# cggos/ptam_cg

Hardware: AMD Instinct MI355X
Metric: BA LM iterations/s (50 KF x 5k pts) [+ tracked frames/s @640x480 in 'tracking'] (higher is better)
Workload: dtype f64

## Files before the change

### __graft_entry__.py

```python
import os
import subprocess
import sys

ROOT = os.path.dirname(os.path.abspath(__file__))
if ROOT not in sys.path:
    sys.path.insert(0, ROOT)


def build():
    env = dict(os.environ)
    env.setdefault("PATH", "")
    env["PATH"] = "/opt/rocm/bin:" + env["PATH"]
    subprocess.check_call(["make", "-C", os.path.join(ROOT, "ptam_cg_amd", "csrc"), "-j4"], env=env)
    subprocess.check_call(["make", "-C", os.path.join(ROOT, "oracle")], env=env)
    import ptam_cg_amd
    from ptam_cg_amd import _abi
    import ctypes
    lib = ctypes.CDLL(os.path.join(ROOT, "ptam_cg_amd", "csrc", "libptam_hip.so"))
    missing = [n for n in _abi.DECLARED if not hasattr(lib, "ptam_" + n)]
    if missing:
        raise RuntimeError(f"libptam_hip.so lacks {missing}")


def smoke():
    import numpy as np
    from ptam_cg_amd import host, synth
    from ptam_cg_amd._lib import load
    from tests.oracle_lib import load_oracle
    from tests import util
    hip, oracle = load(), load_oracle()
    a, b = synth.make_frame_pair()
    util.assert_levels_equal(util.keyframe_levels(hip, a), util.keyframe_levels(oracle, a))
    res = []
    for lib in (hip, oracle):
        ctx = host.Context(lib=lib)
        kfa = host.KeyFrame(ctx).MakeKeyFrame_Lite(a)
        kfb = host.KeyFrame(ctx).MakeKeyFrame_Lite(b)
        q, t = synth.make_patch_queries([kfa.level(l) for l in range(4)], n=200)
        res.append(host.PatchFinder(ctx).FindPatchCoarse(kfb, q, t))
    for f in ("found", "best_ssd", "best_x", "best_y"):
        assert np.array_equal(res[0][f], res[1][f]), f
    pc = synth.make_pose_case(n=300)
    ph = host.Context(lib=hip).pose_gn(pc["world"], pc["found"], pc["sqrt_inv_noise"], pc["init_pose"])[0]
    po = host.Context(lib=oracle).pose_gn(pc["world"], pc["found"], pc["sqrt_inv_noise"], pc["init_pose"])[0]
    assert np.allclose(ph, po, atol=1e-10)
    prob = synth.make_ba_problem(8, 100, 1)
    util.assert_ba_equal(util.run_ba(hip, prob), util.run_ba(oracle, prob))
    print("smoke ok: keyframe / patch search bit-exact, pose GN and bundle within tolerance")


if __name__ == "__main__":
    build()
    if len(sys.argv) > 1 and sys.argv[1] == "smoke":
        smoke()
```

### include/ptam_hip_bench.h

```cpp
#ifndef PTAM_HIP_BENCH_H
#define PTAM_HIP_BENCH_H
#include "ptam_hip.h"
#ifdef __cplusplus
extern "C" {
#endif

int ptam_bench_track_frames(int n, ptam_tracker* const* trackers, ptam_kf* const* current, const uint8_t* const* d_frames,
                            const double pose_in[12], const ptam_trackmap_opts* opts, const int32_t* shuffle_levels,
                            const int32_t* shuffle_fine, int frames_each, double* seconds_out);
int ptam_bench_track_batch(int nb, ptam_tracker* const* trackers, ptam_kf* const* current, const uint8_t* const* d_frames,
                           const double pose_in[12], const ptam_trackmap_opts* opts, const int32_t* shuffle_levels,
                           const int32_t* shuffle_fine, int rounds, int groups, double* seconds_out);
int ptam_bench_track_sequence(ptam_tracker* t, ptam_kf* current, int n_frames, const uint8_t* const* d_frames,
                              ptam_motion_model* m, const ptam_trackmap_opts* opts, const int32_t* shuffle_levels,
                              const int32_t* shuffle_fine, int passes, const double* poses_true, double* seconds_out,
                              double* stats_out);

enum {
    PTAM_TS_PYR_PVS = 0,
    PTAM_TS_DETECT = 1,
    PTAM_TS_COMPACT_SELECT = 2,
    PTAM_TS_SEARCH_COARSE = 3,
    PTAM_TS_GATHER_COARSE = 4,
    PTAM_TS_POSE_COARSE = 5,
    PTAM_TS_SEARCH_FINE = 6,
    PTAM_TS_GATHER_FINE = 7,
    PTAM_TS_POSE_FINE = 8,
    PTAM_TS_COUNT = 9
};
int ptam_tracker_set_profiling(ptam_tracker* t, int on);
int ptam_tracker_stage_time(const ptam_tracker* t, int stage, double* total_ms, int* frames);

int ptam_ba_bench_jacobian(ptam_ba* ba, int reps, double* avg_ms, double* algorithmic_bytes);
int ptam_ba_bench_jacobian_rotating(ptam_ba** bas, int n, int reps, double* avg_ms);
int ptam_ba_schur_index_map(int variant, uint16_t* out, int cap);
enum {
    PTAM_BL_COUNTS = 0,
    PTAM_BL_ROWPTR = 1,
    PTAM_BL_M_CAM = 2,
    PTAM_BL_M_PT = 3,
    PTAM_BL_M_ORIG = 4,
    PTAM_BL_M_FIDX = 5,
    PTAM_BL_M_FOUND = 6,
    PTAM_BL_M_S = 7,
    PTAM_BL_PT_ORIG = 8,
    PTAM_BL_POINTS = 9,
    PTAM_BL_CHUNKS = 10,
    PTAM_BL_S_ENTRIES = 11,
    PTAM_BL_S_SEGS = 12,
    PTAM_BL_S_WG_SEG = 13,
    PTAM_BL_S_PAIR_BEGIN = 14,
    PTAM_BL_S_WG_HEAD = 15,
    PTAM_BL_CAM_PTR = 16,
    PTAM_BL_CAM_MEAS = 17
};
int ptam_ba_debug_lists(ptam_ba* ba, int which, void* out, size_t cap_bytes);

#ifdef __cplusplus
}
#endif
#endif
```

### ptam_cg_amd/csrc/ba_debug_host.inc

```
struct BaHostTimes {
    double t0 = 0, first = 0, loop = 0;
};
#ifdef K7_TIMING
static double ba_dbg_now_us() { return std::chrono::duration<double, std::micro>(std::chrono::steady_clock::now().time_since_epoch()).count(); }
#endif

static inline void ba_dbg_begin(ptam_ba* ba, BaHostTimes& ht) {
#ifdef K7_TIMING
    ht.t0 = ba_dbg_now_us();
    (void)hipMemsetAsync(ba->d.dbg + TL_BASE, 0, 8, ba->ctx->stream);
#endif
}
static inline void ba_dbg_first_read(BaHostTimes& ht) {
#ifdef K7_TIMING
    if (ht.first == 0) ht.first = ba_dbg_now_us();
#endif
}
static inline int ba_dbg_loop_end(ptam_ba* ba, BaHostTimes& ht) {
#ifdef K7_TIMING
    ht.loop = ba_dbg_now_us();
    const BaDev& d = ba->d;
    long long h[16];
    HIP_TRY(hipMemcpy(h, d.dbg, sizeof h, hipMemcpyDeviceToHost));
    std::printf("LDLT step2 wg0: loop %lld tail %lld | last wg (role %lld): loop %lld tail %lld\n", h[1] - h[0], h[2] - h[1], h[7],
                h[5] - h[4], h[6] - h[5]);
    long long q[8];
    HIP_TRY(hipMemcpy(q, d.dbg + 32, sizeof q, hipMemcpyDeviceToHost));
    std::printf("LDLT step2 wg0 iteration 3 (cycles): micro factor %lld | my rows %lld | next panel columns %lld | publish %lld | barrier %lld | "
                "operand reads issued %lld | off-chain updates %lld\n", q[1] - q[0], q[2] - q[1], q[3] - q[2], q[4] - q[3], q[5] - q[4], q[6] - q[5], q[7] - q[6]);
#endif
    return PTAM_OK;
}
static inline int ba_dbg_dump(ptam_ba* ba, const BaHostTimes& ht) {
#if defined(K7_TIMING) || defined(SCHUR_STAMPS)
    const BaDev& d = ba->d;
#endif
#ifdef K7_TIMING
    std::printf("HOST Compute: first trial read at %.1f us, loop end %.1f us, total %.1f us (%zu trials)\n", ht.first - ht.t0, ht.loop - ht.t0,
                ba_dbg_now_us() - ht.t0, ba->trials.size());
    {
        long long c[4];
        HIP_TRY(hipMemcpy(c, d.dbg + 5000, sizeof c, hipMemcpyDeviceToHost));
        if (c[3] > c[1])
            std::printf("K7 INSIDE Compute() (its last launch, block 100): %lld shader cycles in %.2f us = %.2f GHz\n", c[2] - c[0], (c[3] - c[1]) * 0.01,
                        (double)(c[2] - c[0]) / ((c[3] - c[1]) * 10.0));
    }
    if (getenv("PTAM_TIMELINE")) {
        std::vector<long long> tl(2 + 2 * TL_MAX);
        HIP_TRY(hipMemcpy(tl.data(), d.dbg + TL_BASE, tl.size() * 8, hipMemcpyDeviceToHost));
        const long long n_tl = std::min<long long>(tl[0], TL_MAX);
        static const char* nm[] = {"?", "purge_pass1", "select_compact", "select_final", "K7", "reduce_vinv", "vinv", "schur_tile", "schur_reduce",
                                   "ldlt_step0", "backward", "point_update", "finalize", "project_e2", "pass1_trial", "purge", "reduce_partials", "publish"};
        for (long long i = 0; i < n_tl; i++)
            std::printf("TL %4lld %-16s start %9.2f us  (+%.2f)\n", i, nm[tl[2 + 2 * i] < 18 ? tl[2 + 2 * i] : 0], (tl[3 + 2 * i] - tl[3]) * 0.01,
                        i ? (tl[3 + 2 * i] - tl[1 + 2 * i]) * 0.01 : 0.0);
    }
#endif
#ifdef SCHUR_STAMPS
    {
        std::vector<long long> wt(1024);
        HIP_TRY(hipMemcpy(wt.data(), d.dbg + 3072, wt.size() * 8, hipMemcpyDeviceToHost));
        const int nw = std::min(512, d.n_schur_wg);
        const long long M40 = (1ll << 40) - 1, M56 = (1ll << 56) - 1;
        long long e0 = wt[0] & M40, x1 = 0;
        for (int i = 0; i < nw; i++) e0 = std::min(e0, wt[2 * i] & M40), x1 = std::max(x1, wt[2 * i + 1] & M56 & M40);
        std::printf("SCHUR workgroups %d: makespan %.2f us; per workgroup (entry, exit in us from the first entry, segments, hw id):\n", nw, (x1 - e0) * 0.01);
        for (int i = 0; i < nw; i++)
            std::printf("%s[%d %.1f %.1f %d %llx]", i % 8 ? " " : "\n  ", i, ((wt[2 * i] & M40) - e0) * 0.01, ((wt[2 * i + 1] & M40) - e0) * 0.01, (int)(wt[2 * i + 1] >> 56),
                        (unsigned long long)(wt[2 * i] >> 40));
        std::printf("\n");
        std::vector<int> wseg((size_t)d.n_schur_wg + 1);
        HIP_TRY(hipMemcpy(wseg.data(), d.s_wg_seg, wseg.size() * 4, hipMemcpyDeviceToHost));
        std::vector<SchurWG> segs((size_t)wseg.back());
        HIP_TRY(hipMemcpy(segs.data(), d.s_segs, segs.size() * sizeof(SchurWG), hipMemcpyDeviceToHost));
        std::vector<SchurEntry> ents((size_t)std::max(1, d.n_schur_entries));
        HIP_TRY(hipMemcpy(ents.data(), d.s_entries, (size_t)d.n_schur_entries * sizeof(SchurEntry), hipMemcpyDeviceToHost));
        std::printf("SCHUR schedule:");
        for (int i = 0; i < nw; i++) {
            std::printf("%s{%d", i % 8 ? " " : "\n  ", i);
            for (int sg = wseg[i]; sg < wseg[i + 1]; sg++) {
                long long cost = 0;
                for (int e = segs[sg].e_begin; e < segs[sg].e_end; e++) cost += ents[(size_t)e].pad & 0xffff;
                std::printf(" %d:%d:%lld", segs[sg].pair, (segs[sg].e_end - segs[sg].e_begin + 3) / 4, cost);
            }
            std::printf("}");
        }
        std::printf("\n");
    }
    {
        std::vector<long long> st(1024);
        HIP_TRY(hipMemcpy(st.data(), d.dbg + 2048, st.size() * 8, hipMemcpyDeviceToHost));
        for (int sel = 0; sel < 2; sel++) {
            const long long* b = st.data() + sel * 512;
            long long t0 = b[0];
            for (int w = 0; w < 4; w++) if (b[w * 64] && b[w * 64] < t0) t0 = b[w * 64];
            std::printf("SCHUR stamps wg %d (groups %lld): per wave, per group: top, loads issued, data there, MFMAs issued (cycles from the first top)\n", sel ? 150 : 0, b[260]);
            for (int w = 0; w < 4; w++) {
                std::printf("  w%d:", w);
                for (int i = 0; i < 16 && b[(w * 16 + i) * 4]; i++)
                    std::printf(" [%lld %lld %lld %lld]", b[(w * 16 + i) * 4] - t0, b[(w * 16 + i) * 4 + 1] - t0, b[(w * 16 + i) * 4 + 2] - t0, b[(w * 16 + i) * 4 + 3] - t0);
                std::printf(" end %lld\n", b[256 + w] - t0);
            }
            std::printf("  kernel entry %lld, exit %lld, segments %lld; last segment's epilogue (wave 0): loop end %lld, barrier 1 %lld, 2 %lld, 3 %lld, laid out %lld, stores issued %lld\n",
                        b[264] - t0, b[265] - t0, b[266], b[268] - t0, b[269] - t0, b[270] - t0, b[271] - t0, b[272] - t0, b[273] - t0);
        }
    }
#endif
    return PTAM_OK;
}
static inline int ba_dbg_k7_stamps(ptam_ba* ba, int reps) {
#ifdef K7_TIMING
    const BaDev& d = ba->d;
    long long h[16];
    HIP_TRY(hipMemcpy(h, d.dbg, sizeof h, hipMemcpyDeviceToHost));
    {
        long long c[4];
        HIP_TRY(hipMemcpy(c, d.dbg + 5000, sizeof c, hipMemcpyDeviceToHost));
        if (c[3] > c[1])
            std::printf("K7 BACK TO BACK (last of %d launches, block 100): %lld shader cycles in %.2f us = %.2f GHz\n", reps, c[2] - c[0], (c[3] - c[1]) * 0.01,
                        (double)(c[2] - c[0]) / ((c[3] - c[1]) * 10.0));
    }
    std::printf("K7 stamps (10 ns ticks since kernel-body start):");
    for (int i = 1; i < 10; i++) std::printf(" [%d] %lld", i, h[i] - h[0]);
    std::printf("\n");
    const int nb = std::min(ba->d.grid_acc, 2000);
    std::vector<long long> w(2 * nb);
    HIP_TRY(hipMemcpy(w.data(), d.dbg + 16, w.size() * 8, hipMemcpyDeviceToHost));
    long long t0 = w[0];
    for (int b = 0; b < nb; b++) t0 = std::min(t0, w[2 * b]);
    std::vector<long long> st(nb), en(nb), du(nb);
    for (int b = 0; b < nb; b++) st[b] = w[2 * b] - t0, en[b] = w[2 * b + 1] - t0, du[b] = en[b] - st[b];
    std::sort(st.begin(), st.end());
    std::sort(en.begin(), en.end());
    std::sort(du.begin(), du.end());
    std::printf("K7 block 7: body starts %lld ticks after the block's first instruction\n", h[0] - w[14]);
    std::printf("K7 wall (10 ns ticks, %d blocks): start p0/p50/p90/p100 %lld %lld %lld %lld | end %lld %lld %lld %lld | dur %lld %lld %lld %lld\n",
                nb, st[0], st[nb / 2], st[nb * 9 / 10], st[nb - 1], en[0], en[nb / 2], en[nb * 9 / 10], en[nb - 1], du[0], du[nb / 2],
                du[nb * 9 / 10], du[nb - 1]);
#endif
    return PTAM_OK;
}
```

### ptam_cg_amd/csrc/ba_jacobian.inc

```
#ifdef K7_NOW
#define K7_WSTORE(dst, v) { const double2 v_ = v; asm volatile("" ::"v"(v_.x), "v"(v_.y)); }
#else
typedef double k7_d2 __attribute__((ext_vector_type(2)));
#define K7_WSTORE(dst, v) { const double2 v_ = v; const k7_d2 w_ = {v_.x, v_.y}; asm volatile("global_store_dwordx4 %0, %1, off sc1\n\ts_nop 1" ::"v"(&(dst)), "v"(w_) : "memory"); }
#endif
template <int THREADS, bool COPY>
__device__ __forceinline__ void jac_flush(const BaDev& d, const double* Ul, double err, int nbad) {
    __shared__ double werr[THREADS / 64];
    __shared__ int wbad[THREADS / 64];
    const int tid = threadIdx.x;
    double* up = d.Upart + (size_t)blockIdx.x * d.F * 27;
#ifdef K7_FLUSH_SC1
    {
        const int n2 = (d.F * 27) >> 1;
        const bool al = ((((size_t)blockIdx.x * d.F * 27) & 1) == 0);
        if (al) {
            for (int k = tid; k < n2; k += THREADS) K7_WSTORE(((double2*)up)[k], make_double2(Ul[2 * k], Ul[2 * k + 1]));
            if (tid == 0 && ((d.F * 27) & 1)) up[d.F * 27 - 1] = Ul[d.F * 27 - 1];
        } else {
            if (tid == 0) up[0] = Ul[0];
            const int n2b = (d.F * 27 - 1) >> 1;
            for (int k = tid; k < n2b; k += THREADS) K7_WSTORE(*(double2*)(up + 1 + 2 * k), make_double2(Ul[1 + 2 * k], Ul[2 + 2 * k]));
            if (tid == 0 && (((d.F * 27) - 1) & 1)) up[d.F * 27 - 1] = Ul[d.F * 27 - 1];
        }
// ... 81 lines not shown
jac_accum_wave_kernel(DevCam cam, BaDev d, int cur, int est_arg, int per_wave, int extra) {
    TL_MARK(d, 4)
    const int4 gf = ba_guard_load(d);
    const int tid = threadIdx.x, lane = tid & 63;
    const int n_chunks64 = (d.M + 63) >> 6;
    const int wid = __builtin_amdgcn_readfirstlane(tid >> 6);
    if (ba_guard_blocks(d, gf)) return;
    if (ba_guard_stay(d, gf)) cur ^= 1;
    const int est = EST >= 0 ? EST : est_arg;
    extern __shared__ __attribute__((aligned(16))) double smem[];
    double* Ul = BIG ? d.Upart : smem;
    double* Ps = BIG ? d.pose[cur] : smem + (DET ? 0 : (((size_t)d.F * 27 + 1) & ~(size_t)1));
    double* Wt = (BIG ? smem : Ps + (size_t)d.C * 12 + 2) + (size_t)(tid >> 6) * K7_WT_DOUBLES;
    K7_WALL(0)
    const double* __restrict__ pt = d.pt[cur];
    const size_t wp = w_plane(d);
#if defined(K7_PRIO) && K7_PRIO == 1
    if (!LOOP) __builtin_amdgcn_s_setprio(0), __builtin_amdgcn_s_setprio(0);
    if (!LOOP) {
        const int pr_ = (wid >> 2) | (((blockIdx.x >> 8) & 1) << 1);
        if (pr_ == 1) __builtin_amdgcn_s_setprio(1);
        if (pr_ == 2) __builtin_amdgcn_s_setprio(2);
        if (pr_ == 3) __builtin_amdgcn_s_setprio(3);
    }
#elif defined(K7_PRIO) && K7_PRIO == 2
    if (!LOOP) {
        const int pr_ = wid & 3;
        if (pr_ == 1) __builtin_amdgcn_s_setprio(1);
        if (pr_ == 2) __builtin_amdgcn_s_setprio(2);
        if (pr_ == 3) __builtin_amdgcn_s_setprio(3);
    }
#elif defined(K7_PRIO) && K7_PRIO == 3
    if (!LOOP) {
        const int pr_ = (wid >> 1) & 3;
        if (pr_ == 1) __builtin_amdgcn_s_setprio(1);
        if (pr_ == 2) __builtin_amdgcn_s_setprio(2);
        if (pr_ == 3) __builtin_amdgcn_s_setprio(3);
    }
#endif
    int c_begin, c_end;
    {
        constexpr int WPB = THREADS / 64;
        const int blk = blockIdx.x, grid = gridDim.x;
        const int full = extra / grid, rem = extra - full * grid;
        const int before = blk * full + min(blk, rem) + min(wid, full) + ((wid > full && blk < rem) ? 1 : 0);
        const int mine = per_wave + ((wid < full || (wid == full && blk < rem)) ? 1 : 0);
        c_begin = (blk * WPB + wid) * per_wave + before;
        c_end = min(n_chunks64, c_begin + mine);
    }
    if (!BIG && !DET)
        for (int k = tid; k < d.F * 27; k += THREADS) Ul[k] = 0;
    const double* __restrict__ pose = d.pose[cur];
    const int n_pose = d.C * 12;
    double pv[2];
#pragma unroll
    for (int i = 0; i < 2; i++) {
        const int k = tid + i * THREADS;
        pv[i] = pose[min(k, n_pose - 1)];
    }
    K7In in;
    if (PREFETCH) k7_load(d, pt, min(c_begin, n_chunks64 - 1) << 6, lane, in);
    const double sigma_sq = d.sc->sigma_sq;
    if (!BIG) {
#pragma unroll
        for (int i = 0; i < 2; i++) {
            const int k = tid + i * THREADS;
            Ps[min(k, n_pose)] = pv[i];
        }
        for (int k = tid + 2 * THREADS; k < n_pose; k += THREADS) Ps[k] = pose[k];
    }
    __syncthreads();
    K7_STAMP(0)
    const double inv_sigma_sq = 1.0 / sigma_sq;
    double err = 0;
    int nbad = 0;
    K7_STAMP(1)
#pragma unroll 1
    for (int ci = c_begin; ci < c_end; ci++) {
        const int m0 = ci << 6;
        const int m = m0 + lane;
        const bool active = m < d.M;
        if (!PREFETCH) k7_load(d, pt, m0, lane, in);
        const K7In cu = in;
        K7_STAMP(2)
        if (PREFETCH && LOOP && ci + 1 < c_end) k7_load(d, pt, (ci + 1) << 6, lane, in);
        const int st = active ? cu.st : MS_DEAD, c = cu.c, p = cu.p, fidx = active ? cu.fidx : -1;
        const int src = p - cu.pt0;
        const double Xw = __shfl(cu.px, src, 64), Yw = __shfl(cu.py, src, 64), Zw = __shfl(cu.pz, src, 64);
        int pid = active ? p : (-1 - lane);
        double v[9];
#pragma unroll
        for (int i = 0; i < 9; i++) v[i] = 0;
        double A0[6] = {0, 0, 0, 0, 0, 0}, A1[6] = {0, 0, 0, 0, 0, 0}, B0[3] = {0, 0, 0}, B1[3] = {0, 0, 0};
        bool full = false;
        BaProj pr;
        double ex = 0, ey = 0, w = 0;
        const double* T = Ps + 12 * c;
        if (st == MS_BAD) {
            err += 1.0;
            nbad++;
        } else if (st == MS_ALIVE) {
            const double Xp[3] = {Xw, Yw, Zw};
            ba_project(cam, T, Xp, pr);
            ex = cu.sn * (cu.fo.x - pr.u);
            ey = cu.sn * (cu.fo.y - pr.v);
            const double e2 = ex * ex + ey * ey;
            w = ba_sqrt_weight(est, e2, sigma_sq, inv_sigma_sq);
            if (w == 0) {
                d.m_state[m] = MS_BAD;
                err += 1.0;
                nbad++;
            } else {
                err += ba_objective(est, e2, sigma_sq, inv_sigma_sq);
                full = true;
            }
        }
        K7_STAMP(3)
        if (full) {
            ex *= w;
            ey *= w;
            double D[4];
            ba_derivs(cam, pr, D);
            const double sw = cu.sn * w;
            const double D0 = sw * D[0], D1 = sw * D[1], D2 = sw * D[2], D3 = sw * D[3];
            const double X = pr.X, Y = pr.Y, Z = pr.Z;
            const double iz = rcp_nr(Z);
            __builtin_amdgcn_sched_barrier(0);
#pragma unroll
            for (int k = 0; k < 3; k++) {
                const double g0 = T[k], g1 = T[3 + k], g2 = T[6 + k];
                const double mx = (g0 - X * g2 * iz) * iz, my = (g1 - Y * g2 * iz) * iz;
                B0[k] = D0 * mx + D1 * my;
                B1[k] = D2 * mx + D3 * my;
            }
            __builtin_amdgcn_sched_barrier(0);
            if (fidx >= 0) {
                const double zx = -X * iz * iz, zy = -Y * iz * iz;
                {
                    const double mxs[6] = {iz, 0, zx, zx * Y, iz * Z - zx * X, -iz * Y};
                    const double mys[6] = {0, iz, zy, -iz * Z + zy * Y, -zy * X, iz * X};
#pragma unroll
                    for (int k = 0; k < 6; k++) {
                        A0[k] = D0 * mxs[k] + D1 * mys[k];
                        A1[k] = D2 * mxs[k] + D3 * mys[k];
                    }
                }
                __builtin_amdgcn_sched_barrier(0);
                K7_STAMP(4)
                if (!DET) {
                    double* Uc = Ul + fidx * 27;
                    int k = 0;
#pragma unroll
                    for (int a = 0; a < 6; a++)
#pragma unroll
                        for (int b = 0; b <= a; b++) K7_UADD(&Uc[k++], A0[a] * A0[b] + A1[a] * A1[b]);
#pragma unroll
                    for (int a = 0; a < 6; a++) K7_UADD(&Uc[21 + a], A0[a] * ex + A1[a] * ey);
                }
                __builtin_amdgcn_sched_barrier(0);
                K7_STAMP(5)
            }
        }
        {
            double* wg0 = d.W + (size_t)m0 * 6;
#pragma unroll
            for (int c = 0; c < 3; c++) {
                double2* wl = (double2*)(Wt + lane * 6);
#pragma unroll
                for (int h = 0; h < 3; h++)
                    wl[h] = make_double2(A0[2 * h] * B0[c] + A1[2 * h] * B1[c], A0[2 * h + 1] * B0[c] + A1[2 * h + 1] * B1[c]);
                double2 tq[3];
#pragma unroll
                for (int j = 0; j < 3; j++) tq[j] = ((const double2*)Wt)[64 * j + lane];
#pragma unroll
                for (int j = 0; j < 3; j++) {
                    const int u = 64 * j + lane;
                    if (m0 + u / 3 < d.M) K7_WSTORE(*(double2*)(wg0 + c * wp + 2 * u), tq[j]);
                }
            }
        }
        __builtin_amdgcn_sched_barrier(0);
        if (!full) ex = ey = 0;
        if (DET && active) {
            double* ad = d.Adet + m;
#pragma unroll
            for (int k = 0; k < 6; k++) ad[(size_t)k * d.M] = A0[k], ad[(size_t)(6 + k) * d.M] = A1[k];
            ad[(size_t)12 * d.M] = ex;
            ad[(size_t)13 * d.M] = ey;
        }
        v[0] = B0[0] * B0[0] + B1[0] * B1[0];
        v[1] = B0[1] * B0[0] + B1[1] * B1[0];
        v[2] = B0[1] * B0[1] + B1[1] * B1[1];
        v[3] = B0[2] * B0[0] + B1[2] * B1[0];
        v[4] = B0[2] * B0[1] + B1[2] * B1[1];
        v[5] = B0[2] * B0[2] + B1[2] * B1[2];
        v[6] = B0[0] * ex + B1[0] * ey;
        v[7] = B0[1] * ex + B1[1] * ey;
        v[8] = B0[2] * ex + B1[2] * ey;
        K7_STAMP(6)
        const int pid1 = pid + 1;
#define SEG_STEP(GETP, GETV)                                             \
    {                                                                    \
        const int po = GETP;                                             \
        double t[9];                                                     \
        _Pragma("unroll") for (int i = 0; i < 9; i++) t[i] = GETV;       \
        if (po == pid1) {                                                \
            _Pragma("unroll") for (int i = 0; i < 9; i++) v[i] += t[i];  \
        }                                                                \
    }
#ifndef K7_NOSCAN
        SEG_STEP(dpp_row_shr0_i32<1>(pid1), dpp_row_shr_f64<1>(v[i]))
        SEG_STEP(dpp_row_shr0_i32<2>(pid1), dpp_row_shr_f64<2>(v[i]))
        SEG_STEP(dpp_row_shr0_i32<4>(pid1), dpp_row_shr_f64<4>(v[i]))
        SEG_STEP(dpp_row_shr0_i32<8>(pid1), dpp_row_shr_f64<8>(v[i]))
        SEG_STEP((dpp_bcastx_i32<0x142>(pid1) & -((lane >> 4) & 1)), dpp_bcastx_f64<0x142>(v[i]))
        SEG_STEP((dpp_bcastx_i32<0x143>(pid1) & -((lane >> 5) & 1)), dpp_bcastx_f64<0x143>(v[i]))
#endif
#undef SEG_STEP
        K7_STAMP(7)
        const int pn = __shfl_down(pid, 1, 64);
        if (active && (lane == 63 || pn != pid)) {
            const bool whole = pid != cu.p_prev && pid != cu.p_next;
            double* Vp = whole ? d.V + (size_t)pid * 6 : d.cut + (size_t)(2 * ci + (pid == cu.p_prev ? 0 : 1)) * 9;
            double* Ep = whole ? d.epsB + (size_t)pid * 3 : Vp + 6;
#pragma unroll
            for (int i = 0; i < 6; i++) Vp[i] = v[i];
            Ep[0] = v[6];
            Ep[1] = v[7];
            Ep[2] = v[8];
        }
        if (!LOOP) break;
    }
    K7_STAMP(8)
    __syncthreads();
    jac_flush<THREADS, !BIG && !DET>(d, Ul, err, nbad);
    K7_STAMP(9)
    K7_WALL(1)
}

static const void* k7_wave_fn(int threads, bool loop, int est, bool big = false, bool det = false) {
    const bool tukey = est == PTAM_EST_TUKEY;
    if (det) {
        if (big) return (const void*)jac_accum_wave_kernel<256, false, true, -1, true, true>;
        if (!loop)
            return tukey ? (const void*)jac_accum_wave_kernel<1024, true, false, PTAM_EST_TUKEY, false, true>
                         : (const void*)jac_accum_wave_kernel<1024, true, false, -1, false, true>;
        return tukey ? (const void*)jac_accum_wave_kernel<256, true, true, PTAM_EST_TUKEY, false, true>
                     : (const void*)jac_accum_wave_kernel<256, false, true, -1, false, true>;
    }
    if (big) return (const void*)jac_accum_wave_kernel<256, false, true, -1, true>;
    if (!loop && threads == 1024)
        return tukey ? (const void*)jac_accum_wave_kernel<1024, true, false, PTAM_EST_TUKEY>
                     : (const void*)jac_accum_wave_kernel<1024, true, false, -1>;
    if (!loop)
        return tukey ? (const void*)jac_accum_wave_kernel<512, true, false, PTAM_EST_TUKEY>
                     : (const void*)jac_accum_wave_kernel<512, true, false, -1>;
    if (threads == 256)
        return tukey ? (const void*)jac_accum_wave_kernel<256, true, true, PTAM_EST_TUKEY>
                     : (const void*)jac_accum_wave_kernel<256, false, true, -1>;
    if (threads == 1024)
        return tukey ? (const void*)jac_accum_wave_kernel<1024, true, true, PTAM_EST_TUKEY>
                     : (const void*)jac_accum_wave_kernel<1024, false, true, -1>;
    return tukey ? (const void*)jac_accum_wave_kernel<512, true, true, PTAM_EST_TUKEY>
                 : (const void*)jac_accum_wave_kernel<512, false, true, -1>;
}

#define DET_TILE 1024
__global__ void __launch_bounds__(256) reduce_det_kernel(BaDev d) {
    if (ba_guard_blocks(d)) return;
    extern __shared__ __attribute__((aligned(16))) double det_lds[];
    constexpr int P = DET_TILE + 1;
    const int tile = blockIdx.x, tid = threadIdx.x;
    const int m0 = tile * DET_TILE, cnt = min(DET_TILE, d.M - m0);
    const size_t M = (size_t)d.M;
#pragma unroll
    for (int k = 0; k < 14; k++)
        for (int i = tid; i < cnt; i += 256) det_lds[k * P + i] = d.Adet[k * M + m0 + i];
    __syncthreads();
    const int* tptr = d.cam_ptr + (size_t)tile * (d.F + 1);
    for (int f = tid; f < d.F; f += 256) {
        double acc[27];
#pragma unroll
        for (int k = 0; k < 27; k++) acc[k] = 0;
        for (int i = tptr[f]; i < tptr[f + 1]; i++) {
            const double* ad = det_lds + (d.cam_meas[i] - m0);
            double A0[6], A1[6];
#pragma unroll
            for (int k = 0; k < 6; k++) A0[k] = ad[k * P], A1[k] = ad[(6 + k) * P];
            const double ex = ad[12 * P], ey = ad[13 * P];
            int k = 0;
#pragma unroll
            for (int a = 0; a < 6; a++)
#pragma unroll
                for (int b = 0; b <= a; b++) acc[k++] += A0[a] * A0[b] + A1[a] * A1[b];
#pragma unroll
            for (int a = 0; a < 6; a++) acc[21 + a] += A0[a] * ex + A1[a] * ey;
        }
        double* up = d.Upart + ((size_t)tile * d.F + f) * 27;
#pragma unroll
        for (int k = 0; k < 27; k++) up[k] = acc[k];
    }
}

#define RSPLIT 16
__device__ __forceinline__ void reduce_partials_body(const BaDev& d, int grid_acc, int bx, int by) {
    __shared__ double comb[4][64];
    __shared__ double werr[4];
    __shared__ int wbad[4];
    const int total = d.F * 27;
    const int lane = threadIdx.x & 63, wid = threadIdx.x >> 6;
    const int col = bx * 64 + lane;
    const int split = by;
    const int rows_per = (d.u_rows + RSPLIT - 1) / RSPLIT;
    const int r0 = split * rows_per, r1 = min(d.u_rows, r0 + rows_per);
    double s = 0;
    if (col < total && r0 + wid < r1) {
        for (int b = r0 + wid; b < r1; b += 32) {
            double q[8];
#pragma unroll
            for (int u = 0; u < 8; u++) q[u] = d.Upart[(size_t)min(b + 4 * u, r1 - 1) * total + col];
#pragma unroll
            for (int u = 0; u < 8; u++) s += b + 4 * u < r1 ? q[u] : 0.0;
        }
    }
    comb[wid][lane] = s;
    __syncthreads();
    if (wid == 0 && col < total) d.Usplit[(size_t)split * total + col] = ((comb[0][lane] + comb[1][lane]) + comb[2][lane]) + comb[3][lane];
    if (bx == 0 && by == 0) {
        double e = 0;
        int nb = 0;
        for (int b = threadIdx.x; b < grid_acc; b += 256) {
            e += d.err_part[2 * b];
            nb += d.bad_part[b];
        }
        e = wave_sum_f64(e);
        nb = wave_sum_i32(nb);
        if (lane == 0) {
            werr[wid] = e;
            wbad[wid] = nb;
        }
        __syncthreads();
        if (threadIdx.x == 0) {
            d.sc->cur_err = ((werr[0] + werr[1]) + werr[2]) + werr[3];
            d.sc->n_bad = wbad[0] + wbad[1] + wbad[2] + wbad[3];
        }
    }
}

__global__ void __launch_bounds__(256) reduce_partials_kernel(BaDev d, int grid_acc) {
    TL_MARK(d, 16)
    if (ba_guard_blocks(d)) return;
    reduce_partials_body(d, grid_acc, blockIdx.x, blockIdx.y);
}
```

### ptam_cg_amd/csrc/ba_schur.inc

```
__device__ __forceinline__ void vinv_body(const BaDev& d, double lambda, int bx) {
    const int p = bx * 256 + threadIdx.x;
    if (p >= d.P) return;
    double v[6];
    const int r0 = d.rowptr[p], r1 = d.rowptr[p + 1];
    const int c0 = r0 >> 6, c1 = (r1 - 1) >> 6;
    if (d.cut != nullptr && r1 > r0 && c0 != c1) {
        const double* q = d.cut + (size_t)(2 * c0 + 1) * 9;
        double e[3] = {q[6], q[7], q[8]};
#pragma unroll
        for (int i = 0; i < 6; i++) v[i] = q[i];
        for (int c = c0 + 1; c <= c1; c++) {
            q = d.cut + (size_t)(2 * c) * 9;
#pragma unroll
            for (int i = 0; i < 6; i++) v[i] += q[i];
#pragma unroll
            for (int i = 0; i < 3; i++) e[i] += q[6 + i];
        }
#pragma unroll
        for (int i = 0; i < 3; i++) d.epsB[(size_t)p * 3 + i] = e[i];
    } else {
#pragma unroll
        for (int i = 0; i < 6; i++) v[i] = d.V[(size_t)p * 6 + i];
    }
    double A[9] = {v[0], v[1], v[3], v[1], v[2], v[4], v[3], v[4], v[5]};
    double* out = d.Vinv + (size_t)p * 9;
    if (A[0] * A[4] * A[8] == 0) {
#pragma unroll
        for (int i = 0; i < 9; i++) out[i] = 0;
        return;
    }
    A[0] *= (1.0 + lambda);
    A[4] *= (1.0 + lambda);
    A[8] *= (1.0 + lambda);
    for (int col = 0; col < 3; col++) {
        double inv_diag = 1;
        for (int row = col; row < 3; row++) {
            double val = A[row * 3 + col];
            for (int c2 = 0; c2 < col; c2++) val -= A[c2 * 3 + col] * A[row * 3 + c2];
            if (row == col) {
                A[row * 3 + col] = val;
                inv_diag = 1 / val;
            } else {
                A[col * 3 + row] = val;
                A[row * 3 + col] = val * inv_diag;
            }
        }
    }
    for (int c = 0; c < 3; c++) {
        double y[3], x[3];
        for (int i = 0; i < 3; i++) {
            double val = (i == c) ? 1.0 : 0.0;
            for (int j = 0; j < i; j++) val -= A[i * 3 + j] * y[j];
            y[i] = val;
        }
        for (int i = 0; i < 3; i++) y[i] /= A[i * 3 + i];
        for (int i = 2; i >= 0; i--) {
            double val = y[i];
            for (int j = i + 1; j < 3; j++) val -= A[j * 3 + i] * x[j];
            x[i] = val;
        }
        for (int r = 0; r < 3; r++) out[r * 3 + c] = x[r];
    }
}

__global__ void __launch_bounds__(256) vinv_kernel(BaDev d, double lambda) {
    TL_MARK(d, 6)
    if (ba_guard_blocks(d)) return;
    vinv_body(d, lambda, blockIdx.x);
}
__global__ void __launch_bounds__(256) reduce_vinv_kernel(BaDev d, int grid_acc, int nx, double lambda, double lambda_stay) {
    TL_MARK(d, 5)
    const int4 gf = ba_guard_load(d);
    if (ba_guard_blocks(d, gf)) return;
    if (ba_guard_stay(d, gf)) lambda = lambda_stay;
    const int b = blockIdx.x, nr = nx * RSPLIT;
    if (b < nr)
        reduce_partials_body(d, grid_acc, b % nx, b / nx);
    else
        vinv_body(d, lambda, b - nr);
}

#define SCHUR_TILE_ELEMS (SCHUR_TC * SCHUR_TC * 36 + SCHUR_TC * 6)
#ifndef SCHUR_RING
#define SCHUR_RING 2
#endif
#ifndef SCHUR_NW
#define SCHUR_NW 4
#endif
#define SCHUR_WG_PER_CU (8 / SCHUR_NW)
#define SCHUR_RED_BYTES ((SCHUR_NW / 2) * 40 * 64 * 8)
#define SCHUR_N_VARIANTS 6
#define SCHUR_MAP_WPT 8

struct SchurGrp {
    double wa[3][3];
    double wb[3][3];
    double vi[9];
    double eb[3];
    unsigned pm;
};
typedef double v4f64 __attribute__((ext_vector_type(4)));
typedef double schur_d2 __attribute__((ext_vector_type(2), aligned(8)));

template <int MODE>
__host__ __device__ __forceinline__ int schur_row(int t, int rid) {
    if (MODE == 1) return rid;
    if (t < 2) return 6 * (rid / 3) + 2 * (rid % 3) + t;
    const int q = 16 + (rid >> 1);
    return 6 * (q / 3) + 2 * (q % 3) + (rid & 1);
}
struct SchurLane {
    int hi4, sh4, hi2, sh2;
    unsigned o4, o2;
};
template <int MODE>
__device__ __forceinline__ SchurLane schur_lane(int l15) {
    SchurLane L;
    const int r0 = schur_row<MODE>(0, l15), r2 = MODE == 3 ? schur_row<3>(2, l15) : 0;
    const int s0 = r0 / 6, s2 = r2 / 6;
    L.hi4 = s0 >> 2, L.sh4 = 8 * (s0 & 3), L.o4 = 8u * (unsigned)(r0 - 6 * s0);
    L.hi2 = s2 >> 2, L.sh2 = 8 * (s2 & 3), L.o2 = 8u * (unsigned)(r2 - 6 * s2);
    return L;
}

__device__ __forceinline__ unsigned schur_slot_off(unsigned o0, unsigned o1, int first, int hi, int sh, int M, bool& present) {
    const unsigned o = ((hi ? o1 : o0) >> sh) & 0xffu;
    present = o != 0xffu;
    return (present ? (unsigned)first + o : (unsigned)M) * 48u;
}

template <int MODE>
__device__ __forceinline__ void schur_fetch_role(const char* __restrict__ W0, const char* __restrict__ W1, const char* __restrict__ W2,
                                                 unsigned o0, unsigned o1, int first, const SchurLane& L, int M, double w[3][3],
                                                 bool& pres01, bool& pres2) {
    pres2 = false;
    const unsigned off4 = schur_slot_off(o0, o1, first, L.hi4, L.sh4, M, pres01) + L.o4;
#ifdef SCHUR_NOLOAD
    for (int t = 0; t < 3; t++) w[t][0] = w[t][1] = w[t][2] = (double)off4;
    return;
#endif
    if (MODE == 1) {
        w[0][0] = *(const double*)(W0 + off4);
        w[0][1] = *(const double*)(W1 + off4);
        w[0][2] = *(const double*)(W2 + off4);
        return;
    }
    const double2 p0 = *(const double2*)(W0 + off4), p1 = *(const double2*)(W1 + off4), p2 = *(const double2*)(W2 + off4);
    w[0][0] = p0.x, w[1][0] = p0.y;
    w[0][1] = p1.x, w[1][1] = p1.y;
    w[0][2] = p2.x, w[1][2] = p2.y;
    if (MODE == 3) {
        const unsigned off2 = schur_slot_off(o0, o1, first, L.hi2, L.sh2, M, pres2) + L.o2;
#ifdef SCHUR_NOFRAG2
        w[2][0] = w[2][1] = w[2][2] = (double)off2;
        return;
#endif
        w[2][0] = *(const double*)(W0 + off2);
        w[2][1] = *(const double*)(W1 + off2);
        w[2][2] = *(const double*)(W2 + off2);
    }
}

template <bool DIAG, int MA, int MB>
__device__ __forceinline__ void schur_fetch(const BaDev& d, const char* __restrict__ W0, const char* __restrict__ W1,
                                            const char* __restrict__ W2, const SchurEntry& e, const SchurLane& La, const SchurLane& Lb,
                                            SchurGrp& g) {
    const double* __restrict__ vp = d.Vinv + (size_t)e.pt * 9;
#ifdef SCHUR_NOVINV
    for (int q = 0; q < 9; q++) g.vi[q] = (double)e.pt;
    if (false)
#endif
#pragma unroll
    for (int q = 0; q < 4; q++) {
        const schur_d2 t = *(const schur_d2*)(vp + 2 * q);
        g.vi[2 * q] = t.x;
        g.vi[2 * q + 1] = t.y;
    }
#ifndef SCHUR_NOVINV
    g.vi[8] = vp[8];
#endif
    if (DIAG) {
        const double* __restrict__ ep = d.epsB + (size_t)e.pt * 3;
#pragma unroll
        for (int q = 0; q < 3; q++) g.eb[q] = ep[q];
    }
    bool a01, a2, b01 = false, b2 = false;
    schur_fetch_role<MA>(W0, W1, W2, e.offa[0], e.offa[1], e.ma, La, d.M, g.wa, a01, a2);
    if (!DIAG) schur_fetch_role<MB>(W0, W1, W2, e.offb[0], e.offb[1], e.mb, Lb, d.M, g.wb, b01, b2);
    g.pm = (__ballot(a01) ? 1u : 0u) | (__ballot(a2) ? 2u : 0u) | (__ballot(b01) ? 4u : 0u) | (__ballot(b2) ? 8u : 0u);
}

template <bool DIAG, int MA, int MB, int PM = -1>
__device__ __forceinline__ void schur_mult(const SchurGrp& g, v4f64 acc[3][3], double accE[3]
#ifdef SCHUR_DOUBLE_MFMA
                                           , v4f64 acc2[3][3]
#endif
) {
    const unsigned pm = PM >= 0 ? (unsigned)PM : g.pm;
    const bool A01 = pm & 1u, A2 = MA == 3 && (pm & 2u), B01 = DIAG ? A01 : (pm & 4u) != 0, B2 = DIAG ? A2 : (MB == 3 && (pm & 8u));
    double y[3][3];
#pragma unroll
    for (int t = 0; t < 3; t++)
#pragma unroll
        for (int c = 0; c < 3; c++) y[t][c] = 0.0;
    if (A01) {
#pragma unroll
        for (int t = 0; t < (MA < 2 ? MA : 2); t++)
#pragma unroll
            for (int c = 0; c < 3; c++) y[t][c] = g.wa[t][0] * g.vi[c] + g.wa[t][1] * g.vi[3 + c] + g.wa[t][2] * g.vi[6 + c];
    }
    if (A2) {
#pragma unroll
        for (int c = 0; c < 3; c++) y[2][c] = g.wa[2][0] * g.vi[c] + g.wa[2][1] * g.vi[3 + c] + g.wa[2][2] * g.vi[6 + c];
    }
#ifdef SCHUR_NOMFMA
#define SCH_MFMA(ti, tj, c) asm volatile("" ::"v"(y[ti][c]), "v"(DIAG ? g.wa[tj][c] : g.wb[tj][c]));
#elif defined(SCHUR_DOUBLE_MFMA)
#define SCH_MFMA(ti, tj, c)                                                                                                          \
    {                                                                                                                                \
        acc[ti][tj] = __builtin_amdgcn_mfma_f64_16x16x4f64(y[ti][c], DIAG ? g.wa[tj][c] : g.wb[tj][c], acc[ti][tj], 0, 0, 0);   \
        acc2[ti][tj] = __builtin_amdgcn_mfma_f64_16x16x4f64(y[ti][c], DIAG ? g.wa[tj][c] : g.wb[tj][c], acc2[ti][tj], 0, 0, 0); \
    }
#else
#define SCH_MFMA(ti, tj, c) acc[ti][tj] = __builtin_amdgcn_mfma_f64_16x16x4f64(y[ti][c], DIAG ? g.wa[tj][c] : g.wb[tj][c], acc[ti][tj], 0, 0, 0);
#endif
    if (A01 && B01) {
#pragma unroll
        for (int c = 0; c < 3; c++)
#pragma unroll
            for (int ti = 0; ti < (MA < 2 ? MA : 2); ti++)
#pragma unroll
                for (int tj = 0; tj < (MB < 2 ? MB : 2); tj++) SCH_MFMA(ti, tj, c)
    }
    if (!DIAG && A01 && B2) {
#pragma unroll
        for (int c = 0; c < 3; c++)
#pragma unroll
            for (int ti = 0; ti < (MA < 2 ? MA : 2); ti++) SCH_MFMA(ti, 2, c)
    }
    if (A2 && B01) {
#pragma unroll
        for (int c = 0; c < 3; c++)
#pragma unroll
            for (int tj = 0; tj < (MB < 2 ? MB : 2); tj++) SCH_MFMA(2, tj, c)
    }
    if (A2 && B2) {
#pragma unroll
        for (int c = 0; c < 3; c++) SCH_MFMA(2, 2, c)
    }
#undef SCH_MFMA
    if (DIAG) {
#pragma unroll
        for (int c = 0; c < 3; c++)
#pragma unroll
            for (int t = 0; t < MA; t++) accE[t] = fma(y[t][c], g.eb[c], accE[t]);
    }
}

template <bool DIAG, int MA, int MB>
__device__ __forceinline__ void schur_tile_body(const BaDev& d, const SchurWG wg, double* red) {
    const int tid = threadIdx.x, wid = tid >> 6;
    int lane = tid & 63;
    asm volatile("" : "+v"(lane));
    const int l15 = lane & 15, l4 = lane >> 4;
    const SchurLane La = schur_lane<MA>(l15), Lb = schur_lane<MB>(l15);
    const size_t wp8 = w_plane(d) * 8;
    const char* __restrict__ W0 = (const char*)d.W;
    const char* __restrict__ W1 = W0 + wp8;
    const char* __restrict__ W2 = W1 + wp8;
    v4f64 acc[3][3];
    double accE[3] = {0, 0, 0};
#pragma unroll
    for (int i = 0; i < 3; i++)
#pragma unroll
        for (int j = 0; j < 3; j++) acc[i][j] = (v4f64){0, 0, 0, 0};
#ifdef SCHUR_DOUBLE_MFMA
    v4f64 acc2[3][3];
#pragma unroll
    for (int i = 0; i < 3; i++)
#pragma unroll
        for (int j = 0; j < 3; j++) acc2[i][j] = (v4f64){0, 0, 0, 0};
#endif
    const int n_ent = wg.e_end - wg.e_begin;
    const int n_grp = (n_ent + 3) >> 2;
    auto entry_at = [&](int gi) {
        const int e = wg.e_begin + 4 * gi + l4;
        const bool have = gi < n_grp && e < wg.e_end;
        SchurEntry en = d.s_entries[have ? e : wg.e_begin];
        if (!have) en.offa[0] = en.offa[1] = en.offb[0] = en.offb[1] = 0xffffffffu;
        return en;
    };
    constexpr int R = SCHUR_RING;
    SchurGrp g[R];
    constexpr int NW = SCHUR_NW;
#pragma unroll
    for (int u = 0; u < R - 1; u++) schur_fetch<DIAG, MA, MB>(d, W0, W1, W2, entry_at(wid + NW * u), La, Lb, g[u]);
    SchurEntry ent_next = entry_at(wid + NW * (R - 1));
#ifdef SCHUR_STAMPS
    __shared__ long long stp[SCHUR_NW][16][4];
    int st_n = 0;
    if (lane == 0) stp[wid][0][0] = -1;
#define SCH_ST(k) if (st_n < 16 && lane == 0) stp[wid][st_n][k] = (long long)__builtin_amdgcn_s_memtime();
#else
#define SCH_ST(k)
#endif
    for (int gi = wid; gi < n_grp; gi += NW * R) {
#pragma unroll
        for (int u = 0; u < R; u++) {
            if (gi + NW * u >= n_grp) break;
            SCH_ST(0)
#ifndef SCHUR_NO_INTERLEAVE
            {
                bool done = false;
                auto step = [&](auto pm_c) {
                    constexpr int PM = decltype(pm_c)::value;
                    constexpr int pa = PM & 3, pb = PM >> 2;
                    if constexpr (pa != 0 && (MA == 3 || pa == 1) && (DIAG ? pb == 0 : (pb != 0 && (MB == 3 || pb == 1)))) {
                        const SchurEntry ent_after = entry_at(gi + NW * (u + R));
                        schur_fetch<DIAG, MA, MB>(d, W0, W1, W2, ent_next, La, Lb, g[(u + R - 1) % R]);
                        ent_next = ent_after;
                        schur_mult<DIAG, MA, MB, PM>(g[u], acc, accE);
                        __builtin_amdgcn_sched_group_barrier(0x020, 2, 0);
#pragma unroll
                        for (int q = 0; q < 20; q++) {
                            __builtin_amdgcn_sched_group_barrier(0x008, 1, 0);
                            __builtin_amdgcn_sched_group_barrier(0x020, 1, 0);
                        }
                        done = true;
#ifdef SCHUR_STAMPS
                        SCH_ST(3)
                        if (st_n < 16 && lane == 0) stp[wid][st_n][1] = stp[wid][st_n][2] = stp[wid][st_n][0];
                        st_n++;
#endif
                    }
                };
                constexpr int full_pm = 1 | (MA == 3 ? 2 : 0) | (DIAG ? 0 : (4 | (MB == 3 ? 8 : 0)));
                if (g[u].pm == (unsigned)full_pm)
                    step(std::integral_constant<int, full_pm>{});
                else {
                    unsigned pmv = g[u].pm;
                    asm volatile("" : "+v"(pmv));
                    switch (pmv) {
#define SCH_CASE(k) case k: if constexpr (k != full_pm) step(std::integral_constant<int, k>{}); break;
                        SCH_CASE(1) SCH_CASE(2) SCH_CASE(3) SCH_CASE(5) SCH_CASE(6) SCH_CASE(7) SCH_CASE(9) SCH_CASE(10) SCH_CASE(11)
                        SCH_CASE(13) SCH_CASE(14) SCH_CASE(15)
#undef SCH_CASE
                        default: break;
                    }
                }
                if (done) continue;
            }
#endif
            schur_fetch<DIAG, MA, MB>(d, W0, W1, W2, ent_next, La, Lb, g[(u + R - 1) % R]);
            ent_next = entry_at(gi + NW * (u + R));
            SCH_ST(1)
#ifdef SCHUR_STAMPS
            asm volatile("" ::"v"(g[u].wa[0][0]), "v"(g[u].wa[1][1]), "v"(g[u].wa[2][2]), "v"(g[u].vi[8]), "v"(g[u].vi[0]),
                         "v"(DIAG ? g[u].eb[2] : g[u].wb[2][2]), "v"(DIAG ? g[u].eb[0] : g[u].wb[0][0]));
#endif
            SCH_ST(2)
#ifdef SCHUR_DOUBLE_MFMA
            schur_mult<DIAG, MA, MB>(g[u], acc, accE, acc2);
#else
            schur_mult<DIAG, MA, MB>(g[u], acc, accE);
#endif
            SCH_ST(3)
#ifdef SCHUR_STAMPS
            st_n++;
#endif
        }
    }
#ifdef SCHUR_STAMPS
    {
        const long long t_end = (long long)__builtin_amdgcn_s_memtime();
        __syncthreads();
        const int sel = blockIdx.x == 0 ? 0 : (blockIdx.x == 150 ? 1 : -1);
        if (sel >= 0 && lane < 16 && wid < 4) {
            long long* o = d.dbg + 2048 + sel * 512 + (wid * 16 + lane) * 4;
            for (int k = 0; k < 4; k++) o[k] = lane < st_n ? stp[wid][lane][k] : 0;
            if (lane == 0) d.dbg[2048 + sel * 512 + 256 + wid] = t_end, d.dbg[2048 + sel * 512 + 260 + wid] = n_grp;
        }
        __syncthreads();
    }
#endif
#ifdef SCHUR_STAMPS
    const int st_sel = blockIdx.x == 0 ? 0 : (blockIdx.x == 150 ? 1 : -1);
#define SCH_EP(k) if (st_sel >= 0 && tid == 0) d.dbg[2048 + st_sel * 512 + 268 + (k)] = (long long)__builtin_amdgcn_s_memtime();
#else
#define SCH_EP(k)
#endif
    SCH_EP(0)
#pragma unroll
    for (int t = 0; t < 3; t++) {
        accE[t] += __shfl_xor(accE[t], 16, 64);
        accE[t] += __shfl_xor(accE[t], 32, 64);
    }
    double flat[39];
#pragma unroll
    for (int ti = 0; ti < 3; ti++)
#pragma unroll
        for (int tj = 0; tj < 3; tj++)
#pragma unroll
            for (int v = 0; v < 4; v++) flat[(ti * 3 + tj) * 4 + v] = acc[ti][tj][v]
#ifdef SCHUR_DOUBLE_MFMA
                                                                      + 0.0 * acc2[ti][tj][v]
#endif
                ;
#pragma unroll
    for (int t = 0; t < 3; t++) flat[36 + t] = DIAG ? accE[t] : 0.0;
    constexpr int H = NW / 2;
    if (wid >= H) {
        double* rw = red + (wid - H) * (40 * 64);
#pragma unroll
        for (int i = 0; i < 39; i++) rw[i * 64 + lane] = flat[i];
    }
    __syncthreads();
    SCH_EP(1)
    if (wid < H) {
        double* rw = red + wid * (40 * 64);
#pragma unroll
        for (int i = 0; i < 39; i++) rw[i * 64 + lane] += flat[i];
    }
    __syncthreads();
    SCH_EP(2)
    {
        static_assert(NW == 4 && SCHUR_MAP_WPT == 8 && (SCHUR_TILE_ELEMS / 2 + 255) / 256 <= 5, "five words per thread of a 256-thread workgroup");
        constexpr int variant = DIAG ? 3 - MA : 6 - MA;
        const unsigned* __restrict__ mp = d.s_map + ((size_t)variant * 64 * NW + tid) * SCHUR_MAP_WPT;
        const uint4 m4 = *(const uint4*)mp;
        const unsigned m5 = mp[4];
        const unsigned mw[5] = {m4.x, m4.y, m4.z, m4.w, m5};
        double2* out2 = (double2*)(d.s_part + (size_t)wg.slot * SCHUR_TILE_ELEMS);
        auto at = [&](unsigned m) {
            if (m == 0xffffu) return 0.0;
            if (H == 4) return (red[m] + red[2 * 2560 + m]) + (red[2560 + m] + red[3 * 2560 + m]);
            if (H == 2) return red[m] + red[2560 + m];
            return red[m];
        };
#pragma unroll
        for (int i = 0; i < 5; i++)
            if (mw[i] != 0xffffffffu) out2[tid + 64 * NW * i] = make_double2(at(mw[i] & 0xffffu), at(mw[i] >> 16));
    }
    SCH_EP(5)
}

static std::vector<unsigned short> schur_index_map() {
    std::vector<unsigned short> map((size_t)SCHUR_N_VARIANTS * SCHUR_TILE_ELEMS, 0xffffu);
    auto inv = [](int mode, int row, int& t, int& rid) {
        for (t = 0; t < mode; t++)
            for (rid = 0; rid < 16; rid++) {
                const int r = mode == 1 ? schur_row<1>(t, rid) : (mode == 2 ? schur_row<2>(t, rid) : schur_row<3>(t, rid));
                if (r == row) return true;
            }
        return false;
    };
    for (int variant = 0; variant < SCHUR_N_VARIANTS; variant++) {
        const bool diag = variant < 3;
        const int ma = diag ? 3 - variant : 6 - variant, mb = diag ? ma : 3;
        unsigned short* m = map.data() + (size_t)variant * SCHUR_TILE_ELEMS;
        for (int e = 0; e < SCHUR_TC * SCHUR_TC * 36; e++) {
            const int jk = e / 36, rc = e - jk * 36, j = jk / SCHUR_TC, k = jk - j * SCHUR_TC, r = rc / 6, c = rc - r * 6;
            int ti, rr, tj, rcol;
            if (!inv(ma, 6 * j + r, ti, rr) || !inv(mb, 6 * k + c, tj, rcol)) continue;
            m[e] = (unsigned short)(((ti * 3 + tj) * 4 + (rr >> 2)) * 64 + rcol + 16 * (rr & 3));
        }
        if (diag)
            for (int row = 0; row < SCHUR_TC * 6; row++) {
                int t, rid;
                if (inv(ma, row, t, rid)) m[SCHUR_TC * SCHUR_TC * 36 + row] = (unsigned short)((36 + t) * 64 + rid);
            }
    }
    return map;
}

static std::vector<unsigned> schur_index_map_device() {
    const std::vector<unsigned short> m = schur_index_map();
    constexpr int NT = 64 * SCHUR_NW, NE2 = SCHUR_TILE_ELEMS / 2;
    std::vector<unsigned> dev((size_t)SCHUR_N_VARIANTS * NT * SCHUR_MAP_WPT, 0xffffffffu);
    for (int v = 0; v < SCHUR_N_VARIANTS; v++)
        for (int t = 0; t < NT; t++)
            for (int i = 0; i < SCHUR_MAP_WPT && t + NT * i < NE2; i++) {
                const int e = t + NT * i;
                dev[((size_t)v * NT + t) * SCHUR_MAP_WPT + i] = (unsigned)m[(size_t)v * SCHUR_TILE_ELEMS + 2 * e] | ((unsigned)m[(size_t)v * SCHUR_TILE_ELEMS + 2 * e + 1] << 16);
            }
    return dev;
}

__global__ void __launch_bounds__(64 * SCHUR_NW) __attribute__((amdgpu_waves_per_eu(2, 2))) schur_tile_mfma_kernel(BaDev d) {
    TL_MARK(d, 7)
    extern __shared__ __attribute__((aligned(16))) double red[];
#ifdef SCHUR_STAMPS
    const long long t_entry = (long long)__builtin_amdgcn_s_memtime();
    if (threadIdx.x == 0 && blockIdx.x < 512) {
        unsigned hw, xcc;
        asm volatile("s_getreg_b32 %0, hwreg(HW_REG_HW_ID)" : "=s"(hw));
        asm volatile("s_getreg_b32 %0, hwreg(HW_REG_XCC_ID)" : "=s"(xcc));
        d.dbg[3072 + 2 * blockIdx.x] = ((long long)__builtin_amdgcn_s_memrealtime() & ((1ll << 40) - 1)) | ((long long)((xcc & 0xf) << 16 | (hw & 0xffff)) << 40);
    }
#endif
#ifdef SCHUR_NO_HEAD
    const int sg0 = d.s_wg_seg[blockIdx.x], sg1 = d.s_wg_seg[blockIdx.x + 1];
#else
    const int4 h0 = ((const int4*)d.s_wg_head)[2 * blockIdx.x], h1 = ((const int4*)d.s_wg_head)[2 * blockIdx.x + 1];
    const int sg0 = h0.x, sg1 = h0.y;
#endif
    for (int sg = sg0; sg < sg1; sg++) {
#ifdef SCHUR_NO_HEAD
        const SchurWG wg = d.s_segs[sg];
#else
        const SchurWG wg = sg == sg0 ? SchurWG{h0.z, h0.w, h1.x, h1.y} : d.s_segs[sg];
#endif
        int a = (int)((sqrt(8.0 * wg.pair + 1.0) - 1.0) * 0.5);
        while ((a + 1) * (a + 2) / 2 <= wg.pair) a++;
        while (a * (a + 1) / 2 > wg.pair) a--;
        const int b = wg.pair - a * (a + 1) / 2;
        const int ncam = min(SCHUR_TC, d.F - a * SCHUR_TC);
        const int ma = ncam <= 2 ? 1 : (ncam <= 5 ? 2 : 3);
        if (a == b) {
            if (ma == 3) schur_tile_body<true, 3, 3>(d, wg, red);
            else if (ma == 2) schur_tile_body<true, 2, 2>(d, wg, red);
            else schur_tile_body<true, 1, 1>(d, wg, red);
        } else {
            if (ma == 3) schur_tile_body<false, 3, 3>(d, wg, red);
            else if (ma == 2) schur_tile_body<false, 2, 3>(d, wg, red);
            else schur_tile_body<false, 1, 3>(d, wg, red);
        }
        __syncthreads();
    }
#ifdef SCHUR_STAMPS
    if (threadIdx.x == 0 && blockIdx.x < 512) d.dbg[3072 + 2 * blockIdx.x + 1] = (long long)__builtin_amdgcn_s_memrealtime() | ((long long)(sg1 - sg0) << 56);
    if ((blockIdx.x == 0 || blockIdx.x == 150) && threadIdx.x == 0) {
        long long* o = d.dbg + 2048 + (blockIdx.x ? 512 : 0) + 264;
        o[0] = t_entry, o[1] = (long long)__builtin_amdgcn_s_memtime(), o[2] = sg1 - sg0;
    }
#endif
}

#define SRED_SLICES 10
__device__ __forceinline__ double schur_sum_partials(const double* __restrict__ elem, int w0, int w1) {
#ifdef SRED_NOLOAD
    return (double)(w1 - w0);
#endif
    double s0 = 0, s1 = 0, s2 = 0, s3 = 0;
    for (int w = w0; w < w1; w += 32) {
        double q[32];
#pragma unroll
        for (int i = 0; i < 32; i++) {
            const double v = elem[(size_t)min(w + i, w1 - 1) * SCHUR_TILE_ELEMS];
            q[i] = w + i < w1 ? v : 0.0;
        }
#pragma unroll
        for (int i = 0; i < 32; i += 4) {
            s0 += q[i];
            s1 += q[i + 1];
            s2 += q[i + 2];
            s3 += q[i + 3];
        }
    }
    return (s0 + s1) + (s2 + s3);
}
__global__ void __launch_bounds__(256) schur_reduce_kernel(BaDev d, double lambda, int pad_identity) {
    TL_MARK(d, 8)
    const int pair = blockIdx.x, slice = blockIdx.y;
    int a = (int)((sqrt(8.0 * pair + 1.0) - 1.0) * 0.5);
    while ((a + 1) * (a + 2) / 2 <= pair) a++;
    while (a * (a + 1) / 2 > pair) a--;
    const int b = pair - a * (a + 1) / 2;
    const int wg0 = d.s_pair_wg_begin[pair], wg1 = d.s_pair_wg_begin[pair + 1];
    double* S = d.SE;
    double* E = se_E(d);
    const int band = se_band(d);
    const size_t FS = (size_t)d.F * 27;
    if (slice < 9) {
        const int idx = slice * 256 + threadIdx.x;
        const int jk = idx / 36, rc = idx - jk * 36;
        const int j = jk >> 3, k = jk & 7, r = rc / 6, c = rc - r * 6;
        const int fa = a * SCHUR_TC + j, fb = b * SCHUR_TC + k;
        if (fa >= d.F || fb >= d.F) return;
        if (a == b && j < k) return;
        const int Rr = 6 * fa + r, Cc = 6 * fb + c, Rb = Rr / SOLVE_NB, Cb = Cc / SOLVE_NB;
        if (Cb > Rb || Rb - Cb > band) return;
        const bool dg = a == b && j == k;
        const int rr = r >= c ? r : c, cc = r >= c ? c : r;
        double uq[RSPLIT];
#pragma unroll
        for (int sp = 0; sp < RSPLIT; sp++) uq[sp] = dg ? d.Usplit[sp * FS + fa * 27 + rr * (rr + 1) / 2 + cc] : 0.0;
        const double tsum = schur_sum_partials(d.s_part + idx, wg0, wg1);
        double val = -tsum;
        if (dg) {
            double u = 0;
#pragma unroll
            for (int sp = 0; sp < RSPLIT; sp++) u += uq[sp];
            if (r == c) u *= (1.0 + lambda);
            val += u;
        }
        S[se_blk(Rb, Cb, band) + (size_t)(Rr % SOLVE_NB) * SOLVE_NB + (Cc % SOLVE_NB)] = val;
        return;
    }
    if (a == b && threadIdx.x < SCHUR_TC * 6) {
        const int idx = threadIdx.x;
        const int j = idx / 6, r = idx - j * 6;
        const int fa = a * SCHUR_TC + j;
        if (fa < d.F) {
            const double s = schur_sum_partials(d.s_part + SCHUR_TC * SCHUR_TC * 36 + idx, wg0, wg1);
            double ea = 0;
#pragma unroll
            for (int sp = 0; sp < RSPLIT; sp++) ea += d.Usplit[sp * FS + fa * 27 + 21 + r];
            E[6 * fa + r] = ea - s;
        }
    }
    {
        const int np = d.npad - d.n, total = np * d.npad;
        for (int idx = pair * 256 + threadIdx.x; idx < total; idx += 256 * (int)gridDim.x) {
            const int q = idx / d.npad;
            const int r = d.n + q, c = idx - q * d.npad;
            const int Rb = r / SOLVE_NB, Cb = c / SOLVE_NB;
            if (c <= r && Rb - Cb <= band)
                S[se_blk(Rb, Cb, band) + (size_t)(r % SOLVE_NB) * SOLVE_NB + (c % SOLVE_NB)] = (r == c && pad_identity) ? 1.0 : 0.0;
        }
    }
    if (pair == 0) {
        const int np = d.npad - d.n;
        for (int idx = threadIdx.x; idx < np; idx += 256) E[d.n + idx] = 0.0;
    }
}
```

### ptam_cg_amd/csrc/bundle.h

```cpp
#pragma once
#include <cstddef>

#include "common.h"

enum { MS_ALIVE = 0, MS_BAD = 1, MS_DEAD = 2 };

#define BA_CHUNK 256
#define SCHUR_TC 8
#define SOLVE_NB 32
#define HIST_BINS 4096

struct BaChunk {
    int pt_begin, pt_end, m_begin, m_end;
};

struct SchurEntry {
    int pt;
    int ma;
    int mb;
    int pad;
    unsigned offa[2];
    unsigned offb[2];
};
struct SchurWG {
    int pair;
    int e_begin, e_end;
    int slot;
};

struct BaScalars {
    double sigma_sq;
    double cur_err;
    double new_err;
    double sumsq_cam;
    double sumsq_pt;
    double median;
    long long n_valid;
    int n_bad;
    int n_outliers;
    int sel_bin;
    int sel_k;
    int n_cand;
    int sel_bin2;
    int sel_k2;
    int select_overflow;
    int n_outliers_pub;
    int pad_;
    int end_step;
    int spec_go;
    int spec_stay;
    int spec_seq;
    int abort_any;
    int solve_fault;
};
static_assert(offsetof(BaScalars, end_step) % 16 == 0 && sizeof(BaScalars) % 8 == 0, "BaScalars: the decision words are read as one 16-byte load");

struct BaDev {
    int C, F, P, M;
    int guard;
    int guard_seq;
    int n, npad;
    int band;
    int n_chunks, grid_acc;
    int u_rows;
    int n_wchunks;
    int n_tiles, n_pairs, n_schur_wg, n_schur_entries;
    double* pose[2];
    int* cam_free;
    double* pt[2];
    double* V;
    double* epsB;
    double* Vinv;
    double* cut;
    int* rowptr;
    int* m_cam;
    int* m_pt;
    double2* m_found;
    double* m_s;
    int* m_orig;
    int* m_fidx;
    uint8_t* m_state;
    double* m_e2;
    double* m_e2t;
    uint8_t* m_zbad_t;
    double* W;
    double* Usplit;
    double* Upart;
    double* Adet;
    int* cam_ptr;
    int* cam_meas;
    double* err_part;
    int* bad_part;
    BaChunk* chunks;
    BaChunk* wchunks;
    unsigned* hist;
    double* cand;
    SchurEntry* s_entries;
    SchurWG* s_segs;
    int* s_wg_seg;
    int* s_pair_wg_begin;
    int* s_wg_head;
    double* s_part;
    unsigned* s_map;
    double* SE;
    double* L;
    double* Dg;
    double* y;
    double* da;
    double *SE2, *L2, *Dg2, *y2;
    unsigned* sflags2;
    unsigned* sflags;
    unsigned solve_seq;
    int chain_off;
    int chain_xcd;
    int spin_limit;
    double* bw_scratch;
    double* sumsq2;
    int* outliers;
    BaScalars* sc;
    long long* dbg;
};

__host__ __device__ __forceinline__ size_t w_plane(const BaDev& d) { return (size_t)(d.M + 1) * 6; }

__host__ __device__ __forceinline__ size_t se_blocks_before_row(int bi, int band) {
    return bi <= band ? (size_t)bi * (bi + 1) / 2 : (size_t)(band + 1) * (band + 2) / 2 + (size_t)(bi - band - 1) * (band + 1);
}
__host__ __device__ __forceinline__ size_t se_blk(int bi, int bj, int band) {
    const int j0 = bi - band > 0 ? bi - band : 0;
    return (se_blocks_before_row(bi, band) + (size_t)(bj - j0)) * (SOLVE_NB * SOLVE_NB);
}
__host__ __device__ __forceinline__ size_t se_size(int nblk, int band) { return se_blocks_before_row(nblk, band) * (SOLVE_NB * SOLVE_NB); }
__host__ __device__ __forceinline__ int se_band(const BaDev& d) {
    const int nblk = d.npad / SOLVE_NB;
    return d.band < nblk - 1 ? d.band : (nblk > 0 ? nblk - 1 : 0);
}
__host__ __device__ __forceinline__ double* se_E(const BaDev& d) { return d.SE + se_size(d.npad / SOLVE_NB, se_band(d)); }

#define MS_LOG 15
#define MS_CH (1 << MS_LOG)
#define MS_CH_BYTES ((size_t)MS_CH * 32)
template <class B>
__host__ __device__ __forceinline__ B* ms_chunk(B* base, size_t i) { return base + (i >> MS_LOG) * MS_CH_BYTES; }
__host__ __device__ __forceinline__ const int& ms_cam(const char* base, size_t i) { return ((const int*)ms_chunk(base, i))[i & (MS_CH - 1)]; }
__host__ __device__ __forceinline__ const int& ms_pt(const char* base, size_t i) { return ((const int*)(ms_chunk(base, i) + (size_t)MS_CH * 4))[i & (MS_CH - 1)]; }
__host__ __device__ __forceinline__ const double2& ms_found(const char* base, size_t i) { return ((const double2*)(ms_chunk(base, i) + (size_t)MS_CH * 8))[i & (MS_CH - 1)]; }
__host__ __device__ __forceinline__ const double& ms_sig(const char* base, size_t i) { return ((const double*)(ms_chunk(base, i) + (size_t)MS_CH * 24))[i & (MS_CH - 1)]; }

struct Carver {
    size_t off = 0;
    size_t take(size_t bytes) {
        const size_t o = off;
        off += (bytes + 255) & ~(size_t)255;
        return o;
    }
};

int ba_dev_meas_chunks(ptam_ba* ba, size_t n_max, char** d_chunks);
int ba_dev_ingest(ptam_ba* ba, int C, const double* poses12, const uint8_t* fixed, int P, const double* d_pts, int M);
struct BaDevResult {
    const double* pose;
    const double* pt;
    const int* pt_orig;
    int C, P_live;
    const int* outliers;
    int n_out;
    const int* step_end;
    int n_steps;
};
int ba_dev_result(const ptam_ba* ba, BaDevResult* r);

int ba_solve(ptam_ctx* ctx, BaDev& d, int cur);
#define CH_SPIN_DEFAULT (1 << 18)
size_t ba_solve_flag_bytes(int nblk);
int ba_solve_init();

#ifdef K7_TIMING
#define TL_BASE 4096
#define TL_MAX 1900
#define TL_MARK(d, kid)                                                                                   \
    if (blockIdx.x == 0 && blockIdx.y == 0 && threadIdx.x == 0) {                                         \
        const unsigned long long q_ = atomicAdd((unsigned long long*)&(d).dbg[TL_BASE], 1ull);            \
        if (q_ < TL_MAX) {                                                                                \
            (d).dbg[TL_BASE + 2 + 2 * q_] = (kid);                                                        \
            (d).dbg[TL_BASE + 3 + 2 * q_] = (long long)__builtin_amdgcn_s_memrealtime();                  \
        }                                                                                                 \
    }
#else
#define TL_MARK(d, kid)
#endif
```

### ptam_cg_amd/csrc/bundle.hip

```cpp
#include <algorithm>
#include <array>
#include <chrono>
#include <climits>
#include <atomic>
#include <numeric>
#include <utility>

#include "bundle.h"
#include "../../include/ptam_hip_bench.h"

#include "ba_math.inc"
#include "ba_pass1.inc"
#include "ba_select.inc"
#include "ba_jacobian.inc"
#include "ba_schur.inc"
#include "ba_update.inc"
#include "ba_prepare.inc"

template <class T>
struct PinVec {
    ptam_ctx* ctx = nullptr;
    T* p = nullptr;
    size_t n = 0, cap = 0, cap_bytes = 0;
    size_t size() const { return n; }
// ... 707 lines not shown
            ba->sblock_cap = ba->sblock_bytes;
        }
        HIP_TRY(hipMemsetAsync(ba->sblock, 0, sclear, ctx->stream));
        char* sb = (char*)ba->sblock;
        d.s_entries = (SchurEntry*)(sb + o_sent);
        d.s_segs = (SchurWG*)(sb + o_swg);
        d.s_wg_seg = (int*)(sb + o_swgseg);
        d.s_pair_wg_begin = (int*)(sb + o_spw);
        d.s_wg_head = (int*)(sb + o_swghead);
        d.s_part = (double*)(sb + o_spart);
        q.cap_pl = cap_pl, q.cap_cut = cap_cut;
        q.cpx = (int*)(sb + o_cpx);
        q.run_cnt = (int*)(sb + o_runcnt);
        q.run_cost = (int*)(sb + o_runcost);
        q.pl_pair = (int*)(sb + o_plpair);
        q.pl_n = (int*)(sb + o_pln);
        q.pl_run0 = (int*)(sb + o_plrun0);
        q.pl_e0 = (int*)(sb + o_ple0);
        q.pl_e = (int*)(sb + o_ple);
        q.pl_h = (long long*)(sb + o_plh);
        q.cut_pair = (int*)(sb + o_cutpair);
        q.cut_e0 = (int*)(sb + o_cute0);
        q.cut_e1 = (int*)(sb + o_cute1);
        q.cut_wg = (int*)(sb + o_cutwg);
        q.wg_first = (int*)(sb + o_wgfirst);
        q.pair_first = (int*)(sb + o_pairfirst);
        q.wseg_tmp = (int*)(sb + o_wsegtmp);
        q.rec = with_rec ? (int4*)(sb + o_rec) : nullptr;
        hipLaunchKernelGGL(prep_split_kernel, dim3(8), dim3(512), 0, ctx->stream, q, cfg);
        hipLaunchKernelGGL(prep_entries_kernel, dim3(n_pairs, 8), dim3(256), 0, ctx->stream, q, d, cfg.cost_model);
        hipLaunchKernelGGL(prep_finish_kernel, dim3(1), dim3(1024), 0, ctx->stream, q, d, cfg.slots);
    } else if (F > 0) {
        Carver sv;
        const size_t o_spw = sv.take((size_t)(n_pairs + 1) * 4), o_spart = sv.take(SCHUR_TILE_ELEMS * 8), o_one = sv.take(256);
        ba->sblock_bytes = sv.off;
        if (!ctx_cache_take(ctx->dev_cache, CTX_NCACHE(ctx->dev_cache), ba->sblock_bytes, &ba->sblock, &ba->sblock_cap)) {
            HIP_TRY(hipMalloc(&ba->sblock, ba->sblock_bytes));
            ba->sblock_cap = ba->sblock_bytes;
        }
        HIP_TRY(hipMemsetAsync(ba->sblock, 0, ba->sblock_bytes, ctx->stream));
        char* sb = (char*)ba->sblock;
        d.s_pair_wg_begin = (int*)(sb + o_spw);
        d.s_part = (double*)(sb + o_spart);
        d.s_entries = (SchurEntry*)(sb + o_one);
        d.s_segs = (SchurWG*)(sb + o_one);
        d.s_wg_seg = (int*)(sb + o_one);
        d.s_wg_head = (int*)(sb + o_one);
    }
    if (ba->det) {
        int* tile_free = (int*)(base + o_tilefree);
        hipLaunchKernelGGL(prep_det_count_kernel, dim3(n_dtiles), dim3(256), 0, ctx->stream, d, tile_free);
        hipLaunchKernelGGL(prep_det_scan_kernel, dim3(1), dim3(1024), 0, ctx->stream, tile_free, n_dtiles);
        hipLaunchKernelGGL(prep_det_lists_kernel, dim3(n_dtiles), dim3(256), 0, ctx->stream, d, (const int*)tile_free);
    }
#undef UP
    seq = ++ctx->pose_seq;
    *stamp = 0;
    hipLaunchKernelGGL(prep_publish_kernel, dim3(1), dim3(64), 0, ctx->stream, q, (volatile unsigned long long*)dp, seq);
    HIP_TRY(hipGetLastError());
    lap("phase 2 enqueued");
    if (int rc = ba_wait_stamp(ctx, stamp, seq, "the second phase of the bundle's prepare")) return rc;
    lap("phase 2 wait");
    ps = *ps_host;
    if (ps.bad) {
        ptam_set_error("bundle prepare: a Schur work list outgrew its bound (%d; workgroups per list %d %d %d %d %d %d %d %d, budgets %lld %lld, segments %d %d)", ps.bad,
                       ps.n_wgs[0], ps.n_wgs[1], ps.n_wgs[2], ps.n_wgs[3], ps.n_wgs[4], ps.n_wgs[5], ps.n_wgs[6], ps.n_wgs[7], ps.t_cut[0], ps.t_cut[1],
                       ps.n_cuts[0], ps.n_cuts[1]);
        return PTAM_E_STATE;
    }
    d.n_schur_wg = ps.n_schur_wg;
    ba->n_schur_segs = ps.n_segs;
#ifdef PREP_STAMPS
    for (int x = 0; x < 8; x++) {
        std::fprintf(stderr, "[ptam] split kernel, list %d (us from its start): lists built %.1f | in LDS %.1f | round 1 done %.1f | search done %.1f | cut written %.1f\n", x,
                     (ps.stamp[x][1] - ps.stamp[x][0]) * 0.01, (ps.stamp[x][2] - ps.stamp[x][0]) * 0.01, (ps.stamp[x][3] - ps.stamp[x][0]) * 0.01,
                     (ps.stamp[x][4] - ps.stamp[x][0]) * 0.01, (ps.stamp[x][5] - ps.stamp[x][0]) * 0.01);
        std::fprintf(stderr, "[ptam]    the search: %lld shader cycles in %.1f us = %.2f GHz\n", ps.stamp[x][7] - ps.stamp[x][6], (ps.stamp[x][4] - ps.stamp[x][2]) * 0.01,
                     (double)(ps.stamp[x][7] - ps.stamp[x][6]) / ((ps.stamp[x][4] - ps.stamp[x][2]) * 10.0));
    }
#endif
    if (getenv("PTAM_DEBUG_SCHUR")) {
        std::fprintf(stderr, "[ptam] schur: %d segments, %d workgroups; %lld entries in %d (XCD, pair) lists, budgets", ps.n_segs, ps.n_schur_wg,
                     ps.n_entries, ps.n_xp);
        for (int x = 0; x < 8; x++) std::fprintf(stderr, " %lld", ps.t_cut[x]);
        std::fprintf(stderr, "; workgroups per XCD");
        for (int x = 0; x < 8; x++) std::fprintf(stderr, " %d", ps.n_wgs[x]);
        std::fprintf(stderr, "\n");
    }
    {
        const int rc_s = ba_solve_init();
        if (rc_s) return rc_s;
    }
    ba->cur = 0;
    ba->prepared = true;
    return PTAM_OK;
}

static void prof_begin(ptam_ba* ba, int k) {
    if (!ba->prof) return;
    hipEventRecord(ba->ev[k][0], ba->ctx->stream);
}
static void prof_end(ptam_ba* ba, int k) {
    if (!ba->prof) return;
    hipEventRecord(ba->ev[k][1], ba->ctx->stream);
    ba->ev_used[k] = true;
}
static void prof_collect(ptam_ba* ba) {
    if (!ba->prof) return;
    for (int k = 0; k < PTAM_K_COUNT; k++)
        if (ba->ev_used[k]) {
            float ms = 0;
            if (hipEventElapsedTime(&ms, ba->ev[k][0], ba->ev[k][1]) == hipSuccess) {
                ba->k_ms[k] += ms;
                ba->k_n[k]++;
            }
            ba->ev_used[k] = false;
        }
}

static int ba_allreduce(ptam_ba* ba, double* dptr, size_t count) {
    if (!(ba->comm && ba->world > 1)) return PTAM_OK;
    const int rc = ba->comm(ba->comm_user, dptr, count, (void*)ba->ctx->stream);
    if (rc != 0) {
        ptam_set_error("all-reduce hook failed (%d)", rc);
        return PTAM_E_COMM;
    }
    return PTAM_OK;
}

static int ba_sel_blocks() {
    static const int n = [] {
        const char* e = ptam_ab_env("PTAM_SEL_BLOCKS");
        return e ? std::max(1, atoi(e)) : 256;
    }();
    return n;
}
static int ba_pass1_sigma(ptam_ba* ba) {
    ptam_ctx* ctx = ba->ctx;
    BaDev& d = ba->d;
    const bool sharded = ba->comm && ba->world > 1;
    const double min_s2 = ba->opts.min_sigma * ba->opts.min_sigma;
    const int build_hist = (sharded && ba->slow_select) ? 0 : 1;
    prof_begin(ba, PTAM_K_PROJECT);
    if (ba->trial_is_current && d.M > 0)
        hipLaunchKernelGGL(pass1_from_trial_kernel, dim3(std::max(1, std::min((d.M + 256 * P1_U - 1) / (256 * P1_U), 512))), dim3(256), 0, ctx->stream, d,
                           build_hist);
    else if (ba->e2_is_current && d.M > 0) {
        if (build_hist)
            hipLaunchKernelGGL(pass1_keep_kernel, dim3(std::max(1, std::min((d.M + 256 * P1_U - 1) / (256 * P1_U), 512))), dim3(256), 0, ctx->stream, d);
    } else if (d.n_chunks > 0)
        hipLaunchKernelGGL(project_e2_kernel, dim3(std::min(d.n_chunks, 512)), dim3(BA_CHUNK), 0, ctx->stream, ctx->cam, d,
                           ba->cur, build_hist);
    prof_end(ba, PTAM_K_PROJECT);
    prof_begin(ba, PTAM_K_SELECT);
    if (!sharded) {
        hipLaunchKernelGGL(select_compact_kernel, dim3(std::max(1, std::min((d.M + 1023) / 1024, ba_sel_blocks()))), dim3(256), 0,
                           ctx->stream, d, (const double*)d.m_e2, (long long)d.M, (const uint8_t*)d.m_state, 0);
    } else if (!ba->slow_select) {
        if (!ba->d_sel) {
            if (const char* e = ptam_ab_env("PTAM_XCAND_CAP")) ba->xcand_cap = std::max(1, std::min(atoi(e), 1 << 20));
            HIP_TRY(hipMalloc((void**)&ba->d_sel, (HIST_BINS + (size_t)ba->world * (1 + 2 * (size_t)ba->xcand_cap)) * sizeof(double)));
        }
        double* hx = ba->d_sel;
        double* xc = ba->d_sel + HIST_BINS;
        const int cap = ba->xcand_cap;
        double* list = xc + (size_t)ba->world * (1 + (size_t)cap);
        const size_t n_xc = (size_t)ba->world * (1 + (size_t)cap);
        auto reduce_hist = [&](unsigned* h) -> int {
            hipLaunchKernelGGL(hist_to_f64_kernel, dim3(HIST_BINS / 256), dim3(256), 0, ctx->stream, (const unsigned*)h, hx, HIST_BINS);
            const int rc = ba_allreduce(ba, hx, HIST_BINS);
            if (rc) return rc;
            hipLaunchKernelGGL(f64_to_hist_kernel, dim3(HIST_BINS / 256), dim3(256), 0, ctx->stream, (const double*)hx, h, HIST_BINS);
            return PTAM_OK;
        };
        int rc = reduce_hist(d.hist);
        if (rc) return rc;
        hipLaunchKernelGGL(select_compact_kernel, dim3(std::max(1, std::min((d.M + 1023) / 1024, ba_sel_blocks()))), dim3(256), 0,
                           ctx->stream, d, (const double*)d.m_e2, (long long)d.M, (const uint8_t*)d.m_state, 1);
        rc = reduce_hist(d.hist + HIST_BINS);
        if (rc) return rc;
        HIP_TRY(hipMemsetAsync(xc, 0, n_xc * sizeof(double), ctx->stream));
        hipLaunchKernelGGL(select_stage_kernel, dim3(1), dim3(1024), 0, ctx->stream, d, xc, ba->rank, ba->world, cap);
        rc = ba_allreduce(ba, xc, n_xc);
        if (rc) return rc;
        hipLaunchKernelGGL(select_finish_kernel, dim3(1), dim3(1024), 0, ctx->stream, d, (const double*)xc, list, ba->world, cap,
                           ba->opts.estimator, min_s2);
        prof_end(ba, PTAM_K_SELECT);
        HIP_TRY(hipGetLastError());
        return PTAM_OK;
    } else {
        int* d_cnt = (int*)(ba->d_xchg + 256);
        HIP_TRY(hipMemsetAsync(d_cnt, 0, 4, ctx->stream));
        hipLaunchKernelGGL(compact_valid_kernel, dim3(std::max(1, std::min((d.M + 255) / 256, 1024))), dim3(256), 0,
                           ctx->stream, d, d.cand, d_cnt);
        int n_local = 0;
        HIP_TRY(hipMemcpyAsync(&n_local, d_cnt, 4, hipMemcpyDeviceToHost, ctx->stream));
        HIP_TRY(ptam_stream_wait(ctx->stream));
        std::vector<double> counts(ba->world, 0.0);
        counts[ba->rank] = n_local;
        HIP_TRY(hipMemcpyAsync(ba->d_xchg, counts.data(), ba->world * 8, hipMemcpyHostToDevice, ctx->stream));
        int rc = ba_allreduce(ba, ba->d_xchg, ba->world);
        if (rc) return rc;
        HIP_TRY(hipMemcpyAsync(counts.data(), ba->d_xchg, ba->world * 8, hipMemcpyDeviceToHost, ctx->stream));
        HIP_TRY(ptam_stream_wait(ctx->stream));
        long long total = 0, off = 0;
        for (int r = 0; r < ba->world; r++) {
            if (r == ba->rank) off = total;
            total += (long long)(counts[r] + 0.5);
        }
        if ((size_t)total > ba->gather_cap) {
            if (ba->d_gather) HIP_TRY(hipFree(ba->d_gather));
            ba->gather_cap = (size_t)total + (size_t)total / 8 + 1024;
            HIP_TRY(hipMalloc((void**)&ba->d_gather, ba->gather_cap * 16));
        }
        HIP_TRY(hipMemsetAsync(ba->d_gather, 0, (size_t)total * 8, ctx->stream));
        if (n_local > 0)
            hipLaunchKernelGGL(place_keys_kernel, dim3((n_local + 255) / 256), dim3(256), 0, ctx->stream,
                               (const double*)d.cand, n_local, ba->d_gather + off);
        rc = ba_allreduce(ba, ba->d_gather, (size_t)total);
        if (rc) return rc;
        BaDev dg = d;
        dg.cand = ba->d_gather + ba->gather_cap;
        if (total > 0)
            hipLaunchKernelGGL(hist_keys_kernel, dim3((int)std::max<long long>(1, std::min<long long>((total + 255) / 256, 1024))),
                               dim3(256), 0, ctx->stream, (const double*)ba->d_gather, total, d.hist);
        hipLaunchKernelGGL(select_compact_kernel, dim3((int)std::max<long long>(1, std::min<long long>((total + 1023) / 1024, 256))),
                           dim3(256), 0, ctx->stream, dg, (const double*)ba->d_gather, total, (const uint8_t*)nullptr, 0);
        hipLaunchKernelGGL(select_final_kernel, dim3(1), dim3(1024), 0, ctx->stream, dg, ba->opts.estimator, min_s2);
        prof_end(ba, PTAM_K_SELECT);
        HIP_TRY(hipGetLastError());
        return PTAM_OK;
    }
    hipLaunchKernelGGL(select_final_kernel, dim3(1), dim3(1024), 0, ctx->stream, d, ba->opts.estimator, min_s2);
    prof_end(ba, PTAM_K_SELECT);
    HIP_TRY(hipGetLastError());
    return PTAM_OK;
}

static void launch_k7(ptam_ba* ba, int guard = 0) {
    ptam_ctx* ctx = ba->ctx;
    BaDev d = ba->d;
    d.guard = guard;
    d.guard_seq = (int)ba->mbox_seq;
    int cur = guard ? (ba->cur ^ 1) : ba->cur;
    if ((ba->k7_big && !ba->det) || !ba->use_wave)
        (void)hipMemsetAsync(d.Upart, 0, std::max<size_t>(1, (size_t)d.F * 27) * sizeof(double), ctx->stream);
    if (!ba->use_wave) {
        (void)hipMemsetAsync(d.err_part, 0, 16, ctx->stream);
        (void)hipMemsetAsync(d.bad_part, 0, 4, ctx->stream);
        return;
    }
    int est = ba->opts.estimator;
    void* args[] = {&ctx->cam, &d, &cur, &est, &ba->per_wave, &ba->extra_waves};
    (void)hipLaunchKernel(k7_wave_fn(ba->k7_threads, ba->k7_loop, est, ba->k7_big, ba->det), dim3(d.grid_acc), dim3(ba->k7_threads), args,
                          ba->smem_acc, ctx->stream);
    if (ba->det && d.F > 0)
        hipLaunchKernelGGL(reduce_det_kernel, dim3(d.u_rows), dim3(256), (size_t)14 * (DET_TILE + 1) * sizeof(double), ctx->stream, d);
}

static int ba_pass2(ptam_ba* ba) {
    ptam_ctx* ctx = ba->ctx;
    BaDev& d = ba->d;
    prof_begin(ba, PTAM_K_JACOBIAN);
    launch_k7(ba);
    prof_end(ba, PTAM_K_JACOBIAN);
    hipLaunchKernelGGL(reduce_partials_kernel, dim3(std::max(1, (d.F * 27 + 63) / 64), RSPLIT), dim3(256), 0, ctx->stream,
                       d, d.grid_acc);
    HIP_TRY(hipGetLastError());
    if (ba->comm && ba->world > 1) {
        if (d.F > 0) {
            hipLaunchKernelGGL(pack2_kernel, dim3(1), dim3(1), 0, ctx->stream, (const BaScalars*)d.sc, se_E(d) + d.npad, 0, 0);
            ba->cur_pending = true;
        } else {
            hipLaunchKernelGGL(pack2_kernel, dim3(1), dim3(1), 0, ctx->stream, (const BaScalars*)d.sc, ba->d_xchg, 0, 0);
            int rc = ba_allreduce(ba, ba->d_xchg, 2);
            if (rc) return rc;
            hipLaunchKernelGGL(unpack2_kernel, dim3(1), dim3(1), 0, ctx->stream, d.sc, (const double*)ba->d_xchg, 0);
        }
    }
    return PTAM_OK;
}

static int ba_ensure_mailbox(ptam_ba* ba) {
    if (ba->mbox) return PTAM_OK;
    void* h = nullptr;
    size_t cap = 0;
    if (!ctx_cache_take(ba->ctx->host_cache, CTX_NCACHE(ba->ctx->host_cache), sizeof(ptam_ba::Mailbox), &h, &cap))
        HIP_TRY(hipHostMalloc(&h, sizeof(ptam_ba::Mailbox), hipHostMallocMapped | hipHostMallocCoherent));
    std::memset(h, 0, sizeof(ptam_ba::Mailbox));
    void* dv = nullptr;
    HIP_TRY(hipHostGetDevicePointer(&dv, h, 0));
    ba->mbox = (ptam_ba::Mailbox*)h;
    ba->mbox_dev = (ptam_ba::Mailbox*)dv;
    return PTAM_OK;
}

static int ba_trial(ptam_ba* ba, double lambda, bool skip_vinv, int last_allowed, int abort_local, bool decide_in_prologue = false) {
    ptam_ctx* ctx = ba->ctx;
    BaDev& d = ba->d;
    prof_begin(ba, PTAM_K_VINV);
    if (d.P > 0 && !skip_vinv) hipLaunchKernelGGL(vinv_kernel, dim3((d.P + 255) / 256), dim3(256), 0, ctx->stream, d, lambda);
    prof_end(ba, PTAM_K_VINV);
    if (d.F > 0) {
        prof_begin(ba, PTAM_K_SCHUR);
        if (d.n_schur_wg > 0)
            hipLaunchKernelGGL(schur_tile_mfma_kernel, dim3(d.n_schur_wg), dim3(64 * SCHUR_NW), SCHUR_RED_BYTES, ctx->stream, d);
        hipLaunchKernelGGL(schur_reduce_kernel, dim3(d.n_pairs, SRED_SLICES), dim3(256), 0, ctx->stream, d, lambda,
                           (ba->world > 1 && ba->rank != 0) ? 0 : 1);
        prof_end(ba, PTAM_K_SCHUR);
        HIP_TRY(hipGetLastError());
        const size_t n_se = se_size(d.npad / SOLVE_NB, se_band(d)) + d.npad;
        const bool sharded = ba->comm && ba->world > 1;
        if (sharded) prof_begin(ba, PTAM_K_EXCHANGE);
        int rc = ba_allreduce(ba, d.SE, n_se + (ba->cur_pending ? 2 : 0));
        if (sharded) prof_end(ba, PTAM_K_EXCHANGE);
        if (rc) return rc;
        if (ba->cur_pending) {
            hipLaunchKernelGGL(unpack2_kernel, dim3(1), dim3(1), 0, ctx->stream, d.sc, (const double*)(d.SE + n_se), 0);
            ba->cur_pending = false;
        }
        prof_begin(ba, PTAM_K_SOLVE);
        rc = ba_solve(ctx, d, ba->cur);
        prof_end(ba, PTAM_K_SOLVE);
        if (rc) return rc;
    }
    prof_begin(ba, PTAM_K_UPDATE);
    if (d.F == 0)
        hipLaunchKernelGGL(pose_update_kernel, dim3(std::max(1, (d.C + 63) / 64)), dim3(64), 0, ctx->stream, d, ba->cur);
    if (d.n_chunks > 0)
        hipLaunchKernelGGL(point_update_kernel, dim3(d.n_chunks), dim3(BA_CHUNK), 0, ctx->stream, ctx->cam, d, ba->cur,
                           ba->opts.estimator);
    {
        const bool fuse = !(ba->comm && ba->world > 1) && !ba->prof;
        ulonglong2* slots = nullptr;
        unsigned long long seq = 0;
        if (fuse) {
            const int rcm = ba_ensure_mailbox(ba);
            if (rcm) return rcm;
            slots = (ulonglong2*)ba->mbox_dev;
            seq = ++ba->mbox_seq;
            ba->published_by_finalize = true;
        }
        ba->decide_pending = decide_in_prologue;
        ba->decide_last_allowed = last_allowed;
        if (!decide_in_prologue)
            hipLaunchKernelGGL(finalize_new_kernel, dim3(1), dim3(256), 0, ctx->stream, d, ba->opts.update_sq_conv_limit, last_allowed,
                               slots, seq);
    }
    prof_end(ba, PTAM_K_UPDATE);
    HIP_TRY(hipGetLastError());
    if (ba->comm && ba->world > 1) {
        hipLaunchKernelGGL(pack2_kernel, dim3(1), dim3(1), 0, ctx->stream, (const BaScalars*)d.sc, ba->d_xchg, 1, abort_local);
        int rc = ba_allreduce(ba, ba->d_xchg, 4);
        if (rc) return rc;
        hipLaunchKernelGGL(unpack2_kernel, dim3(1), dim3(1), 0, ctx->stream, d.sc, (const double*)ba->d_xchg, 1);
    }
    return PTAM_OK;
}

static int ba_p1_blocks() {
    static const int n = [] {
        const char* e = ptam_ab_env("PTAM_P1_BLOCKS");
        return e ? std::max(1, atoi(e)) : 512;
    }();
    return n;
}
static int ba_enqueue_speculative(ptam_ba* ba, double lambda_next, double lambda_stay) {
    ptam_ctx* ctx = ba->ctx;
    BaDev d = ba->d;
    const double min_s2 = ba->opts.min_sigma * ba->opts.min_sigma;
    d.guard = 1;
    d.guard_seq = (int)ba->mbox_seq;
    const dim3 g_p1(std::max(1, std::min((d.M + 256 * P1_U - 1) / (256 * P1_U), ba_p1_blocks())));
    if (ba->decide_pending) {
        hipLaunchKernelGGL(purge_pass1_decide_kernel, g_p1, dim3(256), 0, ctx->stream, d, ba->opts.update_sq_conv_limit, ba->decide_last_allowed,
                           (ulonglong2*)ba->mbox_dev, ba->mbox_seq);
        ba->decide_pending = false;
    } else
        hipLaunchKernelGGL(purge_pass1_kernel, g_p1, dim3(256), 0, ctx->stream, d);
    hipLaunchKernelGGL(select_compact_kernel, dim3(std::max(1, std::min((d.M + 1023) / 1024, ba_sel_blocks()))), dim3(256), 0, ctx->stream, d,
                       (const double*)d.m_e2, (long long)d.M, (const uint8_t*)d.m_state, 0);
    hipLaunchKernelGGL(select_final_kernel, dim3(1), dim3(1024), 0, ctx->stream, d, ba->opts.estimator, min_s2);
    launch_k7(ba, 1);
    {
        const int nx = std::max(1, (d.F * 27 + 63) / 64);
        hipLaunchKernelGGL(reduce_vinv_kernel, dim3(nx * RSPLIT + (d.P + 255) / 256), dim3(256), 0, ctx->stream, d, d.grid_acc, nx,
                           lambda_next, lambda_stay);
    }
    HIP_TRY(hipGetLastError());
    return PTAM_OK;
}

static int ba_publish_scalars(ptam_ba* ba) {
    ptam_ctx* ctx = ba->ctx;
    int rc = ba_ensure_mailbox(ba);
    if (rc) return rc;
    if (ba->published_by_finalize) {
        ba->published_by_finalize = false;
        return PTAM_OK;
    }
    const unsigned long long seq = ++ba->mbox_seq;
    hipLaunchKernelGGL(publish_scalars_kernel, dim3(1), dim3(64), 0, ctx->stream, (const BaScalars*)ba->d.sc,
                       (ulonglong2*)ba->mbox_dev, seq);
    HIP_TRY(hipGetLastError());
    return PTAM_OK;
}

static int ba_wait_scalars(ptam_ba* ba, BaScalars* out) {
    ptam_ctx* ctx = ba->ctx;
    const unsigned long long seq = ba->mbox_seq;
    constexpr unsigned NW = sizeof(BaScalars) / 8;
    auto arrived = [&]() {
        for (unsigned i = 0; i < NW; i++)
            if (ba->mbox->slot[i].seq != seq) return false;
        return true;
    };
    if (ba->prof) {
        HIP_TRY(ptam_stream_wait(ctx->stream));
    } else {
        const int rc = ba_wait_mapped(ctx, "a trial's scalars", arrived, [&](bool drained) {
            std::fprintf(stderr, "[ptam] waiting for seq %llu: stream %s, slots", seq, drained ? "drained" : "busy");
            for (unsigned i = 0; i < NW; i++) std::fprintf(stderr, " %llu", (unsigned long long)ba->mbox->slot[i].seq);
            std::fprintf(stderr, "\n");
        });
        if (rc) return rc;
    }
    unsigned long long words[NW];
    for (;;) {
        std::atomic_thread_fence(std::memory_order_acquire);
        for (unsigned i = 0; i < NW; i++) words[i] = ba->mbox->slot[i].v;
        std::atomic_thread_fence(std::memory_order_acquire);
        if (arrived()) break;
    }
    std::memcpy(out, words, sizeof(BaScalars));
    prof_collect(ba);
    return PTAM_OK;
}

static int ba_read_scalars(ptam_ba* ba, BaScalars* out) {
    const int rc = ba_publish_scalars(ba);
    return rc ? rc : ba_wait_scalars(ba, out);
}

int ba_dev_meas_chunks(ptam_ba* ba, size_t n_max, char** d_chunks) {
    if (int rc = ba->ms.reserve_dev((n_max + MS_CH - 1) >> MS_LOG)) return rc;
    *d_chunks = ba->ms.d;
    return PTAM_OK;
}
int ba_dev_ingest(ptam_ba* ba, int C, const double* poses12, const uint8_t* fixed, int P, const double* d_pts, int M) {
    ba->cam_pose.assign(poses12, poses12 + (size_t)12 * C);
    ba->cam_fixed.assign(fixed, fixed + C);
    ba->pts.n = 0;
    if (int rc = ba->pts.reserve((size_t)3 * P)) return rc;
    ba->pts.n = (size_t)3 * P;
    ba->pts_dev = d_pts;
    ba->ms.n = (size_t)M;
    ba->ms.up_chunks = ((size_t)M + MS_CH - 1) >> MS_LOG;
    ba->m_dead.assign((size_t)M, 0);
    ba->n_dead = 0;
    ba->prepared = false;
    return PTAM_OK;
}
int ba_dev_result(const ptam_ba* ba, BaDevResult* r) {
    if (!ba->prepared && ba->raw_out.empty()) return PTAM_E_STATE;
    const BaDev& d = ba->d;
    r->pose = d.pose[ba->cur];
    r->pt = d.pt[ba->cur];
    r->pt_orig = ba->d_pt_orig;
    r->C = d.C;
    r->P_live = d.P;
    r->outliers = d.outliers;
    r->n_out = (int)ba->raw_out.size();
    r->step_end = ba->raw_out_ends.data();
    r->n_steps = (int)ba->raw_out_ends.size();
    return PTAM_OK;
}

struct ChainTurn {
    static std::atomic<int>& busy(int dev) {
        static std::atomic<int> b[64];
        return b[dev & 63];
    }
    BaDev& d;
    int dev, was;
    bool forced;
    ChainTurn(BaDev& d_, int dev_) : d(d_), dev(dev_), was(d_.chain_off), forced(false) {
        if (busy(dev).fetch_add(1) > 0 && !d.chain_off) {
            d.chain_off = 1;
            forced = true;
        }
    }
    ~ChainTurn() {
        busy(dev).fetch_sub(1);
        if (forced && d.chain_off == 1) d.chain_off = was;
    }
};

static int ba_sharded_handshake(ptam_ba* ba, int rc_prepare, bool abort_local, bool* abort_all, ChainTurn& chain_turn) {
    ptam_ctx* ctx = ba->ctx;
    BaDev& d = ba->d;
    int n_free = 0;
    for (uint8_t x : ba->cam_fixed) n_free += x ? 0 : 1;
    const int nblk_x = (6 * n_free + SOLVE_NB - 1) / SOLVE_NB;
    constexpr int XF = 5;
    const bool band_fits = nblk_x + XF <= 512;
    std::vector<double> mine(band_fits ? XF + nblk_x : XF, 0.0), all(mine.size(), 0.0);
    mine[0] = (!rc_prepare && d.M == 0) ? 1.0 : 0.0;
    mine[1] = (double)d.M;
    mine[2] = rc_prepare ? 1.0 : 0.0;
    mine[3] = abort_local ? 1.0 : 0.0;
    mine[4] = d.chain_off ? 1.0 : 0.0;
    if (!rc_prepare && band_fits && nblk_x > 0) mine[XF + std::min(ba->band_local, nblk_x - 1)] = 1.0;
    if (!ba->d_xchg) {
        HIP_TRY(hipMalloc((void**)&ba->d_xchg, 4096));
        ba->xchg_owned = true;
    }
    HIP_TRY(hipMemcpyAsync(ba->d_xchg, mine.data(), mine.size() * 8, hipMemcpyHostToDevice, ctx->stream));
    const int rc = ba_allreduce(ba, ba->d_xchg, mine.size());
    if (rc) return rc_prepare ? rc_prepare : rc;
    HIP_TRY(hipMemcpyAsync(all.data(), ba->d_xchg, all.size() * 8, hipMemcpyDeviceToHost, ctx->stream));
    HIP_TRY(ptam_stream_wait(ctx->stream));
    if (all[2] > 0.5) {
        if (rc_prepare) return rc_prepare;
        ptam_set_error("sharded bundle: %d of %d ranks could not prepare their shard; nothing was computed on any rank",
                       (int)(all[2] + 0.5), ba->world);
        return PTAM_E_STATE;
    }
    *abort_all = all[3] > 0.5;
    if (all[4] > 0.5 && !d.chain_off) {
        d.chain_off = 1;
        chain_turn.forced = true;
    }
    ba->d.band = std::max(0, nblk_x - 1);
    if (band_fits)
        for (int b = nblk_x - 1; b >= 0; b--)
            if (all[XF + b] > 0.5) {
                ba->d.band = b;
                break;
            }
    if (all[0] > 0.5) {
        ptam_set_error("sharded bundle: %d of %d ranks hold no measurement (shard the points so that every rank gets some)",
                       (int)(all[0] + 0.5), ba->world);
        return PTAM_E_STATE;
    }
    return PTAM_OK;
}

static double ba_stall_ms(std::chrono::steady_clock::time_point t0, int trial, const char* did, const char* what) {
    const double ms = std::chrono::duration<double, std::milli>(std::chrono::steady_clock::now() - t0).count();
    if (ms > 3.0 && ba_debug().stall) std::fprintf(stderr, "[ptam] stall: trial %d %s %.2f ms %s\n", trial, did, ms, what);
    return ms;
}

static int ba_solve_fallback(ptam_ba* ba, int trial) {
    ptam_ctx* ctx = ba->ctx;
    BaDev& d = ba->d;
    if (d.chain_off) {
        ptam_set_error("bundle adjustment: the camera solve reports a fault in its launch-per-block form");
        return PTAM_E_HIP;
    }
    d.chain_off = 2;
    ba->solve_fallbacks++;
    HIP_TRY(hipMemsetAsync(&d.sc->solve_fault, 0, sizeof(int), ctx->stream));
    if (d.sflags) HIP_TRY(hipMemsetAsync(d.sflags, 0, sizeof(unsigned), ctx->stream));
    if (ba_debug().solve) std::fprintf(stderr, "[ptam] rank %d: persistent camera solve timed out at trial %d; repeating it with the launch-per-column form\n", ba->rank, trial);
    return PTAM_OK;
}

static void ba_report_trial_times(const ptam_ba* ba, const std::vector<double>& trial_read_us) {
    if (trial_read_us.empty()) return;
    std::fprintf(stderr, "[ptam] trial times (us):");
    for (size_t i = 0; i < trial_read_us.size() && i < ba->trials.size(); i++) {
        const ptam_ba_trial& t = ba->trials[i];
        std::fprintf(stderr, " %c%.1f", t.accepted ? 'a' : (t.err_new > t.err_old ? 'r' : 's'), trial_read_us[i] - (i ? trial_read_us[i - 1] : 0.0));
    }
    std::fprintf(stderr, "\n");
}

static int ba_readback(ptam_ba* ba, int n_out, std::vector<int>& out_idx) {
    ptam_ctx* ctx = ba->ctx;
    const BaDev& d = ba->d;
    const size_t b_pose = (size_t)d.C * 96, b_pts = (size_t)d.P * 24, b_out = (size_t)n_out * 4;
    void* pin = nullptr;
    int rc = ctx_pinned(ctx, 64 + b_pose + b_pts + b_out + 64, &pin);
    if (rc) return rc;
    char* hp = (char*)pin + 64;
    char* dp = (char*)ctx->d_pinned + 64;
    volatile unsigned long long* slot = (volatile unsigned long long*)pin;
    const unsigned long long seq = ++ctx->pose_seq;
    *slot = 0;
    const size_t n_all = (size_t)d.C * 12 + (size_t)d.P * 3 + (size_t)n_out;
    hipLaunchKernelGGL(readback_kernel, dim3((unsigned)std::max<size_t>(1, std::min<size_t>((n_all + 255) / 256, 1024))), dim3(256), 0,
                       ctx->stream, (const double*)d.pose[ba->cur], (size_t)d.C * 12, (const double*)d.pt[ba->cur], (size_t)d.P * 3,
                       (const int*)d.outliers, (size_t)n_out, (double*)dp, (double*)(dp + b_pose), (int*)(dp + b_pose + b_pts));
    hipLaunchKernelGGL(stamp_kernel, dim3(1), dim3(1), 0, ctx->stream, (volatile unsigned long long*)ctx->d_pinned, seq);
    HIP_TRY(hipGetLastError());
    rc = ba_wait_stamp(ctx, slot, seq, "the bundle's results");
    if (rc) return rc;
    std::memcpy(ba->cam_pose.data(), hp, b_pose);
    for (int q = 0; q < d.P; q++)
        std::memcpy(&ba->pts[(size_t)3 * ba->pt_orig[(size_t)q]], hp + b_pose + (size_t)q * 24, 24);
    if (n_out > 0) std::memcpy(out_idx.data(), hp + b_pose + b_pts, b_out);
    return PTAM_OK;
}

extern "C" {

void ptam_ba_opts_default(ptam_ba_opts* o) {
    if (!o) return;
    o->max_iterations = 20;
    o->update_sq_conv_limit = 1e-6;
    o->min_sigma = 0.4;
    o->estimator = PTAM_EST_TUKEY;
    o->verbose = 0;
    o->deterministic = 0;
    o->pad_ = 0;
}

int ptam_ba_create(ptam_ctx* ctx, const ptam_ba_opts* opts, ptam_ba** out) {
    ARG_TRY(ctx && out);
    ptam_ba* ba = new ptam_ba();
    ba->ctx = ctx;
    ba->pts.ctx = ba->ms.ctx = ctx;
    if (opts)
        ba->opts = *opts;
// ... 120 lines not shown
    HIP_TRY(hipSetDevice(ba->ctx->device));
    if (on && !ba->ev_ok) {
        for (int k = 0; k < PTAM_K_COUNT; k++) {
            HIP_TRY(hipEventCreate(&ba->ev[k][0]));
            HIP_TRY(hipEventCreate(&ba->ev[k][1]));
        }
        ba->ev_ok = true;
    }
    ba->prof = on != 0;
    return PTAM_OK;
}

int ptam_ba_kernel_time(const ptam_ba* ba, int kernel, double* total_ms, int* launches) {
    ARG_TRY(ba && kernel >= 0 && kernel < PTAM_K_COUNT);
    if (total_ms) *total_ms = ba->k_ms[kernel];
    if (launches) *launches = ba->k_n[kernel];
    return PTAM_OK;
}

int ptam_ba_set_comm(ptam_ba* ba, int rank, int world, ptam_allreduce_f64_fn fn, void* user) {
    ARG_TRY(ba && world >= 1 && rank >= 0 && rank < world);
    ARG_TRY(world == 1 || fn);
    ARG_TRY(world <= 32);
    if (ba->d_sel && world != ba->world) {
        HIP_TRY(hipSetDevice(ba->ctx->device));
        HIP_TRY(ptam_stream_wait(ba->ctx->stream));
        HIP_TRY(hipFree(ba->d_sel));
        ba->d_sel = nullptr;
    }
    ba->rank = rank;
    ba->world = world;
    ba->comm = fn;
    ba->comm_user = user;
    return PTAM_OK;
}

#define BA_DBG(...) do { if (dbg.wait) { std::fprintf(stderr, "[ptam] " __VA_ARGS__); std::fprintf(stderr, "\n"); } } while (0)
int ptam_ba_compute(ptam_ba* ba, const volatile unsigned char* abort_flag, int* accepted_out) {
    ARG_TRY(ba);
    ptam_ctx* ctx = ba->ctx;
    const BaDebug& dbg = ba_debug();
    HIP_TRY(hipSetDevice(ctx->device));
    BA_DBG("compute: prepare");
    const bool sharded = ba->comm && ba->world > 1;
    int rc = ptam_ba_prepare(ba);
    if (rc && !sharded) return rc;
    const int rc_prepare = rc;
    BA_DBG("compute: prepared M=%d P=%d F=%d chunks=%d wchunks=%d grid_acc=%d schur_wg=%d", ba->d.M, ba->d.P, ba->d.F, ba->d.n_chunks,
           ba->d.n_wchunks, ba->d.grid_acc, ba->d.n_schur_wg);
    BaDev& d = ba->d;
    ChainTurn chain_turn(d, ctx->device);
    double lambda = 0.0001, lambda_factor = 2.0;
    ba->converged = ba->published_by_finalize = ba->cur_pending = ba->slow_select = false;
    ba->trial_is_current = ba->e2_is_current = false;
    bool hit_max = false;
    int counter = 0;
    ba->accepted = 0;
    ba->trials.clear();
    std::vector<int> step_outlier_end;
    int n_steps = 0;
    bool prev_end_pending = false;
    bool abort_all = false;
    auto abort_local = [&]() { return abort_flag && *abort_flag; };
    auto aborted = [&]() { return sharded ? abort_all : abort_local(); };
    BaScalars sc;
    std::memset(&sc, 0, sizeof sc);
    double dbg_enq_ms = 0, dbg_wait_ms = 0;
    std::vector<double> trial_read_us;
    const auto dbg_t0 = std::chrono::steady_clock::now();
    BaHostTimes ht;
    ba_dbg_begin(ba, ht);
    if (sharded && (rc = ba_sharded_handshake(ba, rc_prepare, abort_local(), &abort_all, chain_turn))) return rc;
    const bool empty = d.M == 0;
    const bool spec = !sharded && !ba->prof && d.n_chunks > 0 && !ptam_ab_env("PTAM_NO_SPECULATION");
    bool spec_ready = false;
    const bool fused_decision = !ptam_ab_env("PTAM_SEPARATE_FINALIZE");
    while (!empty && !ba->converged && !hit_max && !aborted()) {
        bool skip_vinv = false;
        if (spec_ready) {
            spec_ready = false;
            skip_vinv = true;
        } else {
            if ((rc = ba_pass1_sigma(ba))) return rc;
            if ((rc = ba_pass2(ba))) return rc;
        }
        bool have_cur = false;
        double cur_err = 0, new_err = 0;
        bool ran_any = false, redo_step = false, nan_stop = false;
        for (;;) {
            if (have_cur && !(new_err > cur_err)) break;
            if (ba->converged || hit_max || aborted()) break;
            BA_DBG("trial %d lambda %g", counter, lambda);
            const auto q0 = std::chrono::steady_clock::now();
            rc = ba_trial(ba, lambda, skip_vinv, counter + 1 >= ba->opts.max_iterations ? 1 : 0, abort_local() ? 1 : 0, spec && fused_decision);
            dbg_enq_ms += ba_stall_ms(q0, counter, "took", "to enqueue");
            skip_vinv = false;
            if (rc) return rc;
            if ((rc = ba_publish_scalars(ba))) return rc;
            if (spec) {
                if ((rc = ba_enqueue_speculative(ba, lambda * 0.3, lambda))) return rc;
            }
            BA_DBG("trial %d enqueued, waiting", counter);
            const auto w0 = std::chrono::steady_clock::now();
            rc = ba_wait_scalars(ba, &sc);
            dbg_wait_ms += ba_stall_ms(w0, counter, "waited", "for its scalars");
            if (rc) return rc;
            BA_DBG("trial %d read: cur %g new %g sigma2 %g median %g n_valid %lld n_bad %d sumsq %g %g", counter, sc.cur_err, sc.new_err,
                   sc.sigma_sq, sc.median, sc.n_valid, sc.n_bad, sc.sumsq_cam, sc.sumsq_pt);
            ba_dbg_first_read(ht);
            if (!have_cur) {
                if (prev_end_pending) step_outlier_end.push_back(spec && fused_decision ? sc.n_outliers_pub : sc.n_outliers);
                prev_end_pending = false;
                if (sc.select_overflow && !ba->slow_select) {
                    ba->slow_select = true;
                    if (dbg.select) std::fprintf(stderr, "[ptam] rank %d: select overflow, repeating the step on the gather path\n", ba->rank);
                    redo_step = true;
                    break;
                }
                have_cur = true;
                cur_err = sc.cur_err;
                new_err = cur_err + 9999;
                if (!(new_err > cur_err)) {
                    nan_stop = true;
                    break;
                }
            }
            if (sc.solve_fault) {
                if ((rc = ba_solve_fallback(ba, counter))) return rc;
                continue;
            }
            ran_any = true;
            if (dbg.trial_times) trial_read_us.push_back(std::chrono::duration<double, std::micro>(std::chrono::steady_clock::now() - dbg_t0).count());
            if (sharded) abort_all = abort_all || sc.abort_any != 0;
            new_err = sc.new_err;
            const double sumsq = sc.sumsq_cam + sc.sumsq_pt;
            if (sumsq < ba->opts.update_sq_conv_limit) ba->converged = true;
            ptam_ba_trial t;
            t.lambda = lambda;
            t.sigma_sq = sc.sigma_sq;
            t.err_old = cur_err;
            t.err_new = new_err;
            t.sum_sq_update = sumsq;
            t.n_bad = sc.n_bad;
            t.accepted = 0;
            if (ba->opts.verbose)
                std::printf("L%.1e\tOld %.6f  New %.6f  Diff %.6f\n", lambda, cur_err, new_err, cur_err - new_err);
            if (new_err > cur_err) {
                lambda = lambda * lambda_factor;
                lambda_factor = lambda_factor * 2;
            }
            counter++;
            if (counter >= ba->opts.max_iterations) hit_max = true;
            ba->trials.push_back(t);
        }
        if (redo_step) continue;
        if (nan_stop) hit_max = true;
        ba->trial_is_current = false;
        ba->e2_is_current = ran_any && !(new_err < cur_err);
        if (ran_any && new_err < cur_err) {
            lambda_factor = 2.0;
            lambda *= 0.3;
            ba->cur ^= 1;
            ba->accepted++;
            ba->trials.back().accepted = 1;
            ba->trial_is_current = true;
        }
        if (prev_end_pending) {
            if ((rc = ba_read_scalars(ba, &sc))) return rc;
            step_outlier_end.push_back(sc.n_outliers);
        }
        const bool stayed = spec && ran_any && !(new_err < cur_err) && !(new_err > cur_err) && !ba->converged && !hit_max;
        spec_ready = (spec && ran_any && new_err < cur_err && !ba->converged && !hit_max) || stayed;
        if (!spec_ready && d.M > 0)
            hipLaunchKernelGGL(purge_kernel, dim3((d.M + 255) / 256), dim3(256), 0, ctx->stream, d);
        prev_end_pending = true;
        HIP_TRY(hipGetLastError());
        n_steps++;
    }
    BA_DBG("loop done, steps %d", n_steps);
    ba_report_trial_times(ba, trial_read_us);
    if (dbg.stall)
        std::fprintf(stderr, "[ptam] compute loop: %zu trials in %.3f ms; host enqueueing trials %.3f ms, waiting for scalars %.3f ms\n",
                     ba->trials.size(), std::chrono::duration<double, std::milli>(std::chrono::steady_clock::now() - dbg_t0).count(),
                     dbg_enq_ms, dbg_wait_ms);
    if (n_steps > 0) {
        if ((rc = ba_read_scalars(ba, &sc))) return rc;
        step_outlier_end.push_back(sc.n_outliers);
    }
    if ((rc = ba_dbg_loop_end(ba, ht))) return rc;
    const int n_out = step_outlier_end.empty() ? 0 : step_outlier_end.back();
    std::vector<int> out_idx(std::max(n_out, 1));
    if ((rc = ba_readback(ba, n_out, out_idx))) return rc;
    ba->raw_out.insert(ba->raw_out.end(), out_idx.begin(), out_idx.begin() + n_out);
    for (int end : step_outlier_end) ba->raw_out_ends.push_back(ba->raw_out_base + end);
    ba->raw_out_base += n_out;
    if (n_out > 0) ba->prepared = false;
    if ((rc = ba_dbg_dump(ba, ht))) return rc;
    if (dbg.stall)
        std::fprintf(stderr, "[ptam] compute total %.3f ms\n",
                     std::chrono::duration<double, std::milli>(std::chrono::steady_clock::now() - dbg_t0).count());
    if (accepted_out) *accepted_out = ba->accepted;
    return PTAM_OK;
}

int ptam_ba_converged(const ptam_ba* ba) { return ba && ba->converged ? 1 : 0; }

int ptam_ba_get_point(const ptam_ba* ba, int n, double pos[3]) {
    ARG_TRY(ba && pos && n >= 0 && n < (int)(ba->pts.size() / 3));
    std::memcpy(pos, &ba->pts[3 * (size_t)n], 24);
    return PTAM_OK;
}
int ptam_ba_get_camera(const ptam_ba* ba, int n, double pose[12]) {
    ARG_TRY(ba && pose && n >= 0 && n < (int)ba->cam_fixed.size());
    std::memcpy(pose, &ba->cam_pose[12 * (size_t)n], 96);
    return PTAM_OK;
}
int ptam_ba_get_all(const ptam_ba* ba, double* poses12, double* points3) {
    ARG_TRY(ba);
    if (poses12) std::memcpy(poses12, ba->cam_pose.data(), ba->cam_pose.size() * 8);
    if (points3) std::memcpy(points3, ba->pts.data(), ba->pts.size() * 8);
    return PTAM_OK;
}
int ptam_ba_get_outliers(const ptam_ba* ba, int32_t* pairs, int cap) {
    if (!ba) return PTAM_E_ARG;
    ba_finish_outliers(const_cast<ptam_ba*>(ba));
    const int n = (int)ba->outliers.size();
    for (int i = 0; i < n && i < cap && pairs; i++) {
        pairs[2 * i] = ba->outliers[i].first;
        pairs[2 * i + 1] = ba->outliers[i].second;
    }
    return n;
}
int ptam_ba_get_trials(const ptam_ba* ba, ptam_ba_trial* out, int cap) {
    if (!ba) return PTAM_E_ARG;
    const int n = (int)ba->trials.size();
    for (int i = 0; i < n && i < cap && out; i++) out[i] = ba->trials[i];
    return n;
}
int ptam_ba_solve_fallbacks(const ptam_ba* ba) {
    ARG_TRY(ba);
    return ba->solve_fallbacks;
}
int ptam_ba_duplicates_refused(const ptam_ba* ba) {
    ARG_TRY(ba);
    return ba->dups_refused;
}
int ptam_ba_counts(const ptam_ba* ba, int* n_cams, int* n_free, int* n_points, int* n_meas) {
    ARG_TRY(ba);
    int f = 0;
    for (uint8_t x : ba->cam_fixed) f += x ? 0 : 1;
    ba_finish_outliers(const_cast<ptam_ba*>(ba));
    const int live = (int)ba->m_dead.size() - ba->n_dead;
    if (n_cams) *n_cams = (int)ba->cam_fixed.size();
    if (n_free) *n_free = f;
    if (n_points) *n_points = (int)(ba->pts.size() / 3);
    if (n_meas) *n_meas = live;
    return PTAM_OK;
}

int ptam_ba_bench_jacobian(ptam_ba* ba, int reps, double* avg_ms, double* algorithmic_bytes) {
    ARG_TRY(ba && reps > 0);
    ptam_ctx* ctx = ba->ctx;
    HIP_TRY(hipSetDevice(ctx->device));
    int rc = ptam_ba_prepare(ba);
    if (rc) return rc;
    BaDev& d = ba->d;
    ARG_TRY(d.M > 0);
    const bool prof = ba->prof;
    ba->prof = false;
    rc = ba_pass1_sigma(ba);
    if (rc) return rc;
    hipEvent_t e0, e1;
    HIP_TRY(hipEventCreate(&e0));
    HIP_TRY(hipEventCreate(&e1));
    for (int i = 0; i < 3; i++)
        launch_k7(ba);
    HIP_TRY(ptam_stream_wait(ctx->stream));
    HIP_TRY(hipEventRecord(e0, ctx->stream));
    for (int i = 0; i < reps; i++) launch_k7(ba);
    HIP_TRY(hipEventRecord(e1, ctx->stream));
    HIP_TRY(hipEventSynchronize(e1));
    float ms_total = 0;
    HIP_TRY(hipEventElapsedTime(&ms_total, e0, e1));
    const double total = ms_total;
    hipEventDestroy(e0);
    hipEventDestroy(e1);
    ba->prof = prof;
    if ((rc = ba_dbg_k7_stamps(ba, reps))) return rc;
    if (avg_ms) *avg_ms = total / reps;
    if (algorithmic_bytes)
        *algorithmic_bytes = (double)d.M * (8 + 24 + 1 + 144) + (double)d.C * 96 + (double)d.P * (24 + 72) + (double)d.F * 216;
    return PTAM_OK;
}

int ptam_ba_schur_index_map(int variant, uint16_t* out, int cap) {
    ARG_TRY(out && variant >= 0 && variant < SCHUR_N_VARIANTS && cap >= SCHUR_TILE_ELEMS);
    const std::vector<unsigned short> m = schur_index_map();
    std::memcpy(out, m.data() + (size_t)variant * SCHUR_TILE_ELEMS, (size_t)SCHUR_TILE_ELEMS * 2);
    return SCHUR_TILE_ELEMS;
}

int ptam_ba_debug_lists(ptam_ba* ba, int which, void* out, size_t cap_bytes) {
    ARG_TRY(ba);
    if (!ba->prepared) {
        ptam_set_error("ptam_ba_debug_lists: the bundle is not prepared");
        return PTAM_E_STATE;
    }
    ptam_ctx* ctx = ba->ctx;
    HIP_TRY(hipSetDevice(ctx->device));
    const BaDev& d = ba->d;
    int counts[16] = {d.C, d.F, d.P, d.M, d.band, d.n_chunks, d.n_tiles, d.n_pairs, d.n_schur_wg, d.n_schur_entries, ba->n_schur_segs, d.grid_acc, 0, 0, 0, 0};
    const void* src = nullptr;
    size_t bytes = 0;
    bool host_src = false;
    int n_free_meas = 0;
    switch (which) {
        case PTAM_BL_COUNTS: src = counts, bytes = sizeof counts, host_src = true; break;
        case PTAM_BL_ROWPTR: src = d.rowptr, bytes = ((size_t)d.P + 1) * 4; break;
        case PTAM_BL_M_CAM: src = d.m_cam, bytes = (size_t)d.M * 4; break;
        case PTAM_BL_M_PT: src = d.m_pt, bytes = (size_t)d.M * 4; break;
        case PTAM_BL_M_ORIG: src = d.m_orig, bytes = (size_t)d.M * 4; break;
        case PTAM_BL_M_FIDX: src = d.m_fidx, bytes = (size_t)d.M * 4; break;
        case PTAM_BL_M_FOUND: src = d.m_found, bytes = (size_t)d.M * 16; break;
        case PTAM_BL_M_S: src = d.m_s, bytes = (size_t)d.M * 8; break;
        case PTAM_BL_PT_ORIG: src = ba->pt_orig.data(), bytes = (size_t)d.P * 4, host_src = true; break;
        case PTAM_BL_POINTS: src = d.pt[ba->cur], bytes = (size_t)d.P * 24; break;
        case PTAM_BL_CHUNKS: src = d.chunks, bytes = (size_t)d.n_chunks * sizeof(BaChunk); break;
        case PTAM_BL_S_ENTRIES: src = d.s_entries, bytes = (size_t)d.n_schur_entries * sizeof(SchurEntry); break;
        case PTAM_BL_S_SEGS: src = d.s_segs, bytes = (size_t)ba->n_schur_segs * sizeof(SchurWG); break;
        case PTAM_BL_S_WG_SEG: src = d.s_wg_seg, bytes = d.n_schur_wg > 0 ? ((size_t)d.n_schur_wg + 1) * 4 : 0; break;
        case PTAM_BL_S_PAIR_BEGIN: src = d.s_pair_wg_begin, bytes = d.F > 0 ? ((size_t)d.n_pairs + 1) * 4 : 0; break;
        case PTAM_BL_S_WG_HEAD: src = d.s_wg_head, bytes = (size_t)d.n_schur_wg * 32; break;
        case PTAM_BL_CAM_PTR: src = d.cam_ptr, bytes = ba->det ? (size_t)((d.M + DET_TILE - 1) / DET_TILE) * ((size_t)d.F + 1) * 4 : 0; break;
        case PTAM_BL_CAM_MEAS:
            if (ba->det && d.M > 0) {
                const size_t last = (size_t)((d.M + DET_TILE - 1) / DET_TILE) * ((size_t)d.F + 1) - 1;
                HIP_TRY(hipMemcpyAsync(&n_free_meas, d.cam_ptr + last, 4, hipMemcpyDeviceToHost, ctx->stream));
                HIP_TRY(ptam_stream_wait(ctx->stream));
            }
            src = d.cam_meas, bytes = (size_t)n_free_meas * 4;
            break;
        default: ARG_TRY(!"which"); 
    }
    if (out && bytes > 0) {
        ARG_TRY(cap_bytes >= bytes);
        if (host_src)
            std::memcpy(out, src, bytes);
        else {
            HIP_TRY(hipMemcpyAsync(out, src, bytes, hipMemcpyDeviceToHost, ctx->stream));
            HIP_TRY(ptam_stream_wait(ctx->stream));
        }
    }
    if (bytes > (size_t)INT_MAX) return PTAM_E_LIMIT;
    return (int)bytes;
}

int ptam_ba_bench_jacobian_rotating(ptam_ba** bas, int n, int reps, double* avg_ms) {
    ARG_TRY(bas && n > 0 && reps > 0 && avg_ms);
    ptam_ctx* ctx = bas[0]->ctx;
    HIP_TRY(hipSetDevice(ctx->device));
    for (int i = 0; i < n; i++) {
        ARG_TRY(bas[i] && bas[i]->ctx == ctx);
        int rc = ptam_ba_prepare(bas[i]);
        if (rc) return rc;
        ARG_TRY(bas[i]->d.M > 0);
        rc = ba_pass1_sigma(bas[i]);
        if (rc) return rc;
    }
    for (int r = 0; r < 2; r++)
        for (int i = 0; i < n; i++) launch_k7(bas[i]);
    HIP_TRY(ptam_stream_wait(ctx->stream));
    hipEvent_t e0, e1;
    HIP_TRY(hipEventCreate(&e0));
    HIP_TRY(hipEventCreate(&e1));
    HIP_TRY(hipEventRecord(e0, ctx->stream));
    for (int r = 0; r < reps; r++)
        for (int i = 0; i < n; i++) launch_k7(bas[i]);
    HIP_TRY(hipEventRecord(e1, ctx->stream));
    HIP_TRY(hipEventSynchronize(e1));
    float ms_total = 0;
    HIP_TRY(hipEventElapsedTime(&ms_total, e0, e1));
    hipEventDestroy(e0);
    hipEventDestroy(e1);
    *avg_ms = (double)ms_total / ((double)reps * n);
    return PTAM_OK;
}

}

int ba_preload_kernels() {
    ptam_preload((const void*)project_e2_kernel);
    ptam_preload((const void*)pass1_from_trial_kernel);
    ptam_preload((const void*)pass1_keep_kernel);
    ptam_preload((const void*)purge_pass1_kernel);
    ptam_preload((const void*)purge_pass1_decide_kernel);
    ptam_preload((const void*)hist_keys_kernel);
    ptam_preload((const void*)select_compact_kernel);
    ptam_preload((const void*)select_final_kernel);
    ptam_preload((const void*)hist_to_f64_kernel);
    ptam_preload((const void*)f64_to_hist_kernel);
    ptam_preload((const void*)select_stage_kernel);
    ptam_preload((const void*)select_finish_kernel);
    ptam_preload((const void*)compact_valid_kernel);
    ptam_preload(k7_wave_fn(256, true, -1, true));
    for (int est : {(int)PTAM_EST_TUKEY, (int)PTAM_EST_CAUCHY})
        for (int lp = 0; lp < 2; lp++) ptam_preload(k7_wave_fn(lp ? 256 : 1024, lp != 0, est, false, true));
    ptam_preload(k7_wave_fn(256, true, -1, true, true));
    ptam_preload((const void*)reduce_det_kernel);
    ptam_preload((const void*)reduce_partials_kernel);
    ptam_preload((const void*)vinv_kernel);
    ptam_preload((const void*)reduce_vinv_kernel);
    ptam_preload((const void*)schur_tile_mfma_kernel);
    ptam_preload((const void*)schur_reduce_kernel);
    ptam_preload((const void*)pose_update_kernel);
    ptam_preload((const void*)point_update_kernel);
    ptam_preload((const void*)finalize_new_kernel);
    ptam_preload((const void*)purge_kernel);
    ptam_preload((const void*)readback_kernel);
    ptam_preload((const void*)stamp_kernel);
    ptam_preload((const void*)publish_scalars_kernel);
    ptam_preload((const void*)set_scalars_kernel);
    ptam_preload((const void*)set_new_kernel);
    ptam_preload((const void*)pack2_kernel);
    ptam_preload((const void*)unpack2_kernel);
    ptam_preload((const void*)place_keys_kernel);
    for (int est = 0; est < 2; est++) {
        ptam_preload(k7_wave_fn(512, false, est ? PTAM_EST_CAUCHY : PTAM_EST_TUKEY));
        ptam_preload(k7_wave_fn(1024, false, est ? PTAM_EST_CAUCHY : PTAM_EST_TUKEY));
        ptam_preload(k7_wave_fn(256, true, est ? PTAM_EST_CAUCHY : PTAM_EST_TUKEY));
        ptam_preload(k7_wave_fn(512, true, est ? PTAM_EST_CAUCHY : PTAM_EST_TUKEY));
        ptam_preload(k7_wave_fn(1024, true, est ? PTAM_EST_CAUCHY : PTAM_EST_TUKEY));
    }
    HIP_TRY(hipFuncSetAttribute((const void*)reduce_det_kernel, hipFuncAttributeMaxDynamicSharedMemorySize, (int)((size_t)14 * (DET_TILE + 1) * sizeof(double))));
    HIP_TRY(hipFuncSetAttribute((const void*)schur_tile_mfma_kernel, hipFuncAttributeMaxDynamicSharedMemorySize, SCHUR_RED_BYTES));
    return PTAM_OK;
}
```

### ptam_cg_amd/csrc/ldlt_chain.inc

```
struct ChainLds {
    double PF[2][2][NB][6];
    double T0[NB * LDP];
    double T1[NB * LDP];
    double T2[NB * LDP];
    double T3[NB * LDP];
    double T4[NB * LDP];
    double iD[NB], Dv[NB], z[NB];
    double zp[8][NB];
    int one_xcd;
    int staged[2];
};
#define CH_TS (NB * LDP)
#define CH_MAX_NB 28
#define CH_LDS_MAX (160 * 1024)
__host__ __device__ __forceinline__ size_t ch_lds_bytes(int band) { return sizeof(ChainLds) + 8 + (size_t)(band + 1) * CH_TS * sizeof(double); }
#define CH_BW_SL 12
__host__ __device__ __forceinline__ size_t ch_lds_bytes_bw(int band, int nblk) {
    const size_t rhs = (size_t)(2 + CH_BW_SL) * nblk * NB + NB, tiles = (size_t)(band + 1) * CH_TS;
    return sizeof(ChainLds) + 8 + (rhs > tiles ? rhs : tiles) * sizeof(double);
}
#define CH_BW_MAXT 9

__device__ __forceinline__ double ch_ld(const double* p) {
    return __longlong_as_double(__hip_atomic_load((const long long*)p, __ATOMIC_RELAXED, __HIP_MEMORY_SCOPE_AGENT));
}
__device__ __forceinline__ void ch_st(double* p, double v, bool one_xcd) {
    if (one_xcd)
        *p = v;
    else
        __hip_atomic_store((long long*)p, __double_as_longlong(v), __ATOMIC_RELAXED, __HIP_MEMORY_SCOPE_AGENT);
}
__device__ __forceinline__ void ch_ld2_issue(double2& v, const double2* p) { asm volatile("global_load_dwordx4 %0, %1, off sc1" : "=v"(v) : "v"(p) : "memory"); }
__device__ __forceinline__ void ch_ld2_wait() { asm volatile("s_waitcnt vmcnt(0)" ::: "memory"); }
__device__ __forceinline__ void ch_raise(unsigned* f, unsigned seq, bool one_xcd) {
    const unsigned v = (seq << 1) | (one_xcd ? 1u : 0u);
    if (one_xcd)
        asm volatile("global_store_dword %0, %1, off" ::"v"(f), "v"(v) : "memory");
    else
        __hip_atomic_store(f, v, __ATOMIC_RELAXED, __HIP_MEMORY_SCOPE_AGENT);
}
__device__ __forceinline__ unsigned ch_flag(const unsigned* f) { return __hip_atomic_load(f, __ATOMIC_RELAXED, __HIP_MEMORY_SCOPE_AGENT); }
__device__ __forceinline__ unsigned ch_wait(const unsigned* f, unsigned seq, unsigned* err, int limit) {
    int spins = 0;
    unsigned v;
    while (((v = ch_flag(f)) >> 1) != seq) {
        __builtin_amdgcn_s_sleep(1);
        if (++spins > limit || ((spins & 255) == 0 && ch_flag(err) == seq)) {
            __hip_atomic_store(err, seq, __ATOMIC_RELAXED, __HIP_MEMORY_SCOPE_AGENT);
            break;
        }
    }
    return v;
}
__device__ __forceinline__ void ch_wait_lanes(const unsigned* f, bool active, unsigned seq, unsigned* err, int limit) {
    int spins = 0;
    for (;;) {
        const bool up = !active || (ch_flag(f) >> 1) == seq;
        if (__builtin_amdgcn_ballot_w64(!up) == 0) break;
        __builtin_amdgcn_s_sleep(1);
        if (++spins > limit || ((spins & 255) == 0 && ch_flag(err) == seq)) {
            __hip_atomic_store(err, seq, __ATOMIC_RELAXED, __HIP_MEMORY_SCOPE_AGENT);
            break;
        }
    }
}
__host__ __device__ __forceinline__ int ch_roles(int nblk) { return nblk > 2 ? nblk : 2; }
__host__ __device__ __forceinline__ size_t ch_flag_words(int nblk, int band) { return 2 + 3 * (size_t)nblk + (size_t)nblk * (band + 1); }

struct ChainArgs {
    double *S, *E, *L, *Dg, *y;
    unsigned* flags;
    int k0, k1, kr, n;
};
__global__ void __launch_bounds__(TPB, 2) ldlt_chain_kernel(BaDev d, ChainArgs a0, ChainArgs a1, int clubs, int cur, int do_bw) {
    const int club = ((int)(blockIdx.x & 7) - d.chain_xcd) & 7;
    if (club >= clubs) return;
    const ChainArgs& a = club == 0 ? a0 : a1;
    const int k0 = a.k0, k1 = a.k1, kr = a.kr;
    const int role = blockIdx.x >> 3;
    if (role == 0 && club == 0) { TL_MARK(d, 9) }
    extern __shared__ __attribute__((aligned(16))) double ch_lds[];
    ChainLds& s = *(ChainLds*)ch_lds;
    const int band = se_band(d), nblk = d.npad / NB;
    const int n_roles = ch_roles(kr - k0);
    if (role >= n_roles) return;
    const unsigned seq = d.solve_seq;
    unsigned* const err = d.sflags;
    unsigned* const F = a.flags + 1;
    unsigned* const RF = F + nblk;
    unsigned* const XCC = RF + nblk;
    unsigned* const XFb = XCC + nblk + 1;
    auto XF = [&](int r, int m) { return XFb + (size_t)r * (band + 1) + (m - max(0, r - band)); };
    double* __restrict__ S = a.S;
    double* __restrict__ E = a.E;
    double* __restrict__ Lf = a.L;
    const int tid = threadIdx.x;
    const int w = __builtin_amdgcn_readfirstlane(tid >> 6), lane = tid & 63;
    const int qi = w >> 1, qj = w & 1;
    const int i16 = lane & 15, m4 = lane >> 4;
    const int colq = 16 * qj + i16;
    const unsigned my_xcc = __builtin_amdgcn_s_getreg(20 | (0 << 6) | (3 << 11)) & 0xf;
    if (tid == 0) __hip_atomic_store(XCC + role, (seq << 4) | my_xcc, __ATOMIC_RELAXED, __HIP_MEMORY_SCOPE_AGENT);
    auto mma_t = [&](const double* A, const double (&bt)[NB / 4]) {
        v4f64 acc = {0, 0, 0, 0};
        const double* pa = A + (16 * qi + i16) * LDP + m4;
        double a8[NB / 4];
#pragma unroll
        for (int kk = 0; kk < NB / 4; kk++) a8[kk] = pa[4 * kk];
#pragma unroll
        for (int kk = 0; kk < NB / 4; kk++) acc = __builtin_amdgcn_mfma_f64_16x16x4f64(a8[kk], bt[kk], acc, 0, 0, 0);
        return acc;
    };
#ifdef K7_TIMING
    int nst_ = 0;
#define CH_STAMP() if (role == 0 && threadIdx.x == 192 && nst_ < 200) d.dbg[32 + nst_++] = (long long)__builtin_readcyclecounter();
#define CH_SEEN(t_) if (lane == 0) d.dbg[440 + k] = d.dbg[456 + k] = 100 + (t_);
#define CH_RT(slot) d.dbg[600 + (slot)] = (long long)__builtin_amdgcn_s_memrealtime();
#else
#define CH_STAMP()
#define CH_SEEN(t_)
#define CH_RT(slot)
#endif
    if (role == 0) {
        const double e0 = m4 == 0 ? 1.0 : 0.0, e1 = m4 == 1 ? 1.0 : 0.0, e2 = m4 == 2 ? 1.0 : 0.0, e3 = m4 == 3 ? 1.0 : 0.0;
        v4f64 accK;
#pragma unroll
        for (int v = 0; v < 4; v++) {
            const int row = 16 * qi + m4 + 4 * v;
            accK[v] = S[se_blk(k0, k0, band) + max(row, colq) * NB + min(row, colq)];
        }
        bool one_xcd = false;
        for (int k = k0; k < k1; k++) {
            v4f64 accI;
            const int niter = (min(NB, a.n - k * NB) + 3) / 4;
            if (tid < NB) {
                s.iD[tid] = 1.0;
                s.Dv[tid] = 1.0;
            }
            const int r = k + 1;
            const bool have_row = r < kr;
            const size_t o_rk = have_row ? se_blk(r, k, band) : 0, o_rr = have_row ? se_blk(r, r, band) : 0;
            if (tid < 2) s.staged[tid] = 0;
            int stage_state = have_row ? 0 : 2;
            double stg[2][NB * NB / 64];
            CH_STAMP()
            if (tid == 0) { CH_RT(4 * k + 3) }
#ifdef FL_NO_STAGE
#define FL_STAGE_ON false
#else
#define FL_STAGE_ON true
#endif
#define FACTOR_IDLE_HOOK(t_)                                                                                         \
    if (FL_STAGE_ON && stage_state < 2) {                                                                            \
        if (stage_state == 0 && (r < k0 + 2 || (ch_flag(RF + r) >> 1) == seq)) {                                     \
            _Pragma("unroll") for (int u = 0; u < NB * NB / 64; u++) stg[0][u] = ch_ld(S + o_rk + lane + 64 * u);    \
            _Pragma("unroll") for (int u = 0; u < NB * NB / 64; u++) stg[1][u] = ch_ld(S + o_rr + lane + 64 * u);    \
            stage_state = (t_) + 1 < niter ? 1 : 3;                                                                  \
            CH_SEEN(t_)                                                                                              \
        } else if (stage_state == 1)                                                                                 \
            stage_state = 3;                                                                                         \
        if (stage_state == 3) {                                                                                      \
            _Pragma("unroll") for (int u = 0; u < NB * NB / 64; u++) {                                               \
                const int e_ = lane + 64 * u;                                                                        \
                s.T3[(e_ / NB) * LDP + e_ % NB] = stg[0][u];                                                         \
                s.T4[(e_ / NB) * LDP + e_ % NB] = stg[1][u];                                                         \
            }                                                                                                        \
            if (lane == 0) s.staged[0] = s.staged[1] = 1;                                                            \
            stage_state = 2;                                                                                         \
        }                                                                                                            \
    }
#include "ldlt_factor2.inc"
#undef FACTOR_IDLE_HOOK
            CH_STAMP()
            if (k == k0) {
                if (w == 0) {
                    bool same = true;
                    for (int i = lane; i < n_roles; i += 64) same = same && ch_flag(XCC + i) == ((seq << 4) | my_xcc);
                    const bool all_same = __builtin_amdgcn_ballot_w64(!same) == 0;
                    if (lane == 0) s.one_xcd = all_same;
                }
                __syncthreads();
                one_xcd = s.one_xcd != 0;
            }
            const size_t o_kk = se_blk(k, k, band);
#pragma unroll
            for (int v = 0; v < 4; v++)
                s.T0[(16 * qi + m4 + 4 * v) * LDP + fl_colI] = accI[v];
            auto store_diag = [&]() {
#pragma unroll
                for (int v = 0; v < 4; v++) ch_st(Lf + o_kk + (16 * qi + m4 + 4 * v) * NB + fl_colI, accI[v], one_xcd);
                if (tid < NB) ch_st(a.Dg + k * NB + tid, s.Dv[tid], one_xcd);
            };
            if (!have_row) {
                store_diag();
                asm volatile("s_waitcnt vmcnt(0)" ::: "memory");
                __syncthreads();
                if (tid == 0) ch_raise(F + k, seq, one_xcd);
                break;
            }
            double aop[NB / 4];
            v4f64 accN;
            if (!(s.staged[0] && s.staged[1])) {
                if (r >= k0 + 2 && lane == 0) ch_wait(RF + r, seq, err, d.spin_limit);
                double t3[NB * NB / TPB], t4[NB * NB / TPB];
#pragma unroll
                for (int u = 0; u < NB * NB / TPB; u++) t3[u] = ch_ld(S + o_rk + tid + u * TPB);
#pragma unroll
                for (int u = 0; u < NB * NB / TPB; u++) t4[u] = ch_ld(S + o_rr + tid + u * TPB);
#pragma unroll
                for (int u = 0; u < NB * NB / TPB; u++) {
                    const int e = tid + u * TPB;
                    s.T3[(e / NB) * LDP + e % NB] = t3[u];
                    s.T4[(e / NB) * LDP + e % NB] = t4[u];
                }
                __syncthreads();
            }
#pragma unroll
            for (int kk = 0; kk < NB / 4; kk++) aop[kk] = s.T3[(16 * qi + i16) * LDP + 4 * kk + m4];
#pragma unroll
            for (int v = 0; v < 4; v++) {
                const int row = 16 * qi + m4 + 4 * v;
                accN[v] = s.T4[max(row, colq) * LDP + min(row, colq)];
            }
            CH_STAMP()
            __syncthreads();
            v4f64 x = {0, 0, 0, 0};
            {
                const double* pb = s.T0 + m4 * LDP + colq;
                double b8[NB / 4];
#pragma unroll
                for (int kk = 0; kk < NB / 4; kk++) b8[kk] = pb[4 * kk * LDP];
#pragma unroll
                for (int kk = 0; kk < NB / 4; kk++) x = __builtin_amdgcn_mfma_f64_16x16x4f64(aop[kk], b8[kk], x, 0, 0, 0);
            }
            const double idc = s.iD[colq];
            __builtin_amdgcn_sched_barrier(0);
            store_diag();
            __builtin_amdgcn_sched_barrier(0);
            double lv[4];
#pragma unroll
            for (int v = 0; v < 4; v++) {
                const int e = (16 * qi + m4 + 4 * v);
                lv[v] = x[v] * idc;
                s.T1[e * LDP + colq] = x[v];
                s.T2[e * LDP + colq] = lv[v];
            }
            __syncthreads();
            double bt[NB / 4];
#pragma unroll
            for (int kk = 0; kk < NB / 4; kk++) bt[kk] = s.T2[(16 * qj + i16) * LDP + 4 * kk + m4];
            const v4f64 upd = mma_t(s.T1, bt);
            __builtin_amdgcn_sched_barrier(0);
#pragma unroll
            for (int v = 0; v < 4; v++) ch_st(Lf + o_rk + (16 * qi + m4 + 4 * v) * NB + colq, lv[v], one_xcd);
            __builtin_amdgcn_sched_barrier(0);
#pragma unroll
            for (int v = 0; v < 4; v++) accK[v] = accN[v] - upd[v];
            asm volatile("s_waitcnt vmcnt(0)" ::: "memory");
            __syncthreads();
            if (tid == 0) {
                ch_raise(F + k, seq, one_xcd);
                ch_raise(XF(r, k), seq, one_xcd);
                CH_RT(4 * k)
            }
            if (r == k1) {
                if (w != 1) {
#pragma unroll
                    for (int v = 0; v < 4; v++) S[o_rr + (16 * qi + m4 + 4 * v) * NB + colq] = accK[v];
                }
                break;
            }
            CH_STAMP()
        }
        return;
    }
    if (role == n_roles - 1) {
        double* const bb = ch_lds + (sizeof(ChainLds) + 7) / 8;
        const int b0 = k0 * NB;
        for (int i = k0 * NB + tid; i < kr * NB; i += TPB) bb[i - b0] = E[i];
        __syncthreads();
        const int q = tid & (NB - 1), part = tid >> 5;
        const int row = tid >> 3, g = tid & 7;
        for (int m = k0; m < k1; m++) {
            if (lane == 0) (void)ch_wait(F + m, seq, err, d.spin_limit);
            const size_t o_mm = se_blk(m, m, band);
            double t4[NB / 8];
#pragma unroll
            for (int j = 0; j < NB / 8; j++) t4[j] = ch_ld(Lf + o_mm + (part + 8 * j) * NB + q);
            double p = 0;
#pragma unroll
            for (int j = 0; j < NB / 8; j++) p += t4[j] * bb[m * NB - b0 + part + 8 * j];
            s.zp[part][q] = p;
            __syncthreads();
            if (tid < NB) {
                const double z = ((s.zp[0][tid] + s.zp[1][tid]) + (s.zp[2][tid] + s.zp[3][tid])) +
                                 ((s.zp[4][tid] + s.zp[5][tid]) + (s.zp[6][tid] + s.zp[7][tid]));
                s.z[tid] = z;
                a.y[m * NB + tid] = z;
                if (do_bw) bb[m * NB - b0 + tid] = z / ch_ld(a.Dg + m * NB + tid);
            }
            __syncthreads();
            double zr[NB / 8];
#pragma unroll
            for (int jj = 0; jj < NB / 8; jj++) zr[jj] = s.z[g + 8 * jj];
            const int jhi = min(kr - 1, m + band);
            {
                const int jw = m + 1 + lane;
                ch_wait_lanes(XF(min(jw, jhi), m), jw <= jhi && jhi > m, seq, err, d.spin_limit);
            }
            for (int jb = m + 1; jb <= jhi; jb += 4) {
                const int nj = min(4, jhi - jb + 1);
                double lv[4][NB / 8];
#pragma unroll
                for (int u = 0; u < 4; u++)
                    if (u < nj) {
                        const double* Lj = Lf + se_blk(jb + u, m, band) + row * NB + g;
#pragma unroll
                        for (int jj = 0; jj < NB / 8; jj++) lv[u][jj] = ch_ld(Lj + 8 * jj);
                    }
#pragma unroll
                for (int u = 0; u < 4; u++)
                    if (u < nj) {
                        double sum = 0;
#pragma unroll
                        for (int jj = 0; jj < NB / 8; jj++) sum += lv[u][jj] * zr[jj];
                        sum += dpp_row_shr_f64<1>(sum);
                        sum += dpp_row_shr_f64<2>(sum);
                        sum += dpp_row_shr_f64<4>(sum);
                        if (g == 7) bb[(jb + u) * NB - b0 + row] -= sum;
                    }
            }
            __syncthreads();
        }
        for (int i = k1 * NB + tid; i < kr * NB; i += TPB) E[i] = bb[i - b0];
        if (!do_bw) return;
        {
            const int nrow = kr * NB;
            double* const xs = bb + nrow;
            double* const pend = xs + nrow;
            for (int i = tid; i < CH_BW_SL * nrow; i += TPB) pend[i] = 0.0;
            const int hh = lane >> 5, c32 = lane & (NB - 1);
            const int g4 = lane >> 4, cp = lane & 15;
            constexpr int TW = 3;
            static_assert(3 * TW >= CH_BW_MAXT, "three tile waves cover a block row");
            static_assert(CH_BW_SL == 12, "a slice per tile wave and lane group");
            const int tw = w - 1;
            double* const dstage0 = s.T1;
            static_assert(4 * NB * LDP >= 2 * NB * 34, "the diagonal tiles' staging areas");
            auto stage_diag = [&](int k) {
                const double2* dk = (const double2*)(Lf + se_blk(k, k, band)) + lane;
                double2 dq[3];
#pragma unroll
                for (int i = 0; i < 3; i++)
                    if (tw + 3 * i < NB / 4) ch_ld2_issue(dq[i], dk + 64 * (tw + 3 * i));
                ch_ld2_wait();
                double* const ds = dstage0 + (k & 1) * (NB * 34);
#pragma unroll
                for (int i = 0; i < 3; i++)
                    if (tw + 3 * i < NB / 4) *(double2*)(ds + (4 * (tw + 3 * i) + g4) * 34 + 2 * cp) = dq[i];
            };
            if (w > 0) stage_diag(kr - 1);
            __syncthreads();
#ifdef K7_TIMING
#define BWI_STAMP(i_) if (lane == 0 && w < 2) d.dbg[1400 + 8 * k + 4 * w + (i_)] = (long long)__builtin_readcyclecounter();
            if (tid == 0) d.dbg[1399] = (long long)__builtin_readcyclecounter();
#else
#define BWI_STAMP(i_)
#endif
#pragma unroll 1
            for (int k = kr - 1; k >= 0; k--) {
                const int jb0 = max(0, k - band), nt = k - jb0;
                BWI_STAMP(0)
                double2 lt[TW][NB / 4];
                if (w == 0) {
                    const double* pk = pend + k * NB + c32;
                    const double v = bb[k * NB + c32] - ((((pk[0] + pk[nrow]) + (pk[2 * nrow] + pk[3 * nrow])) + ((pk[4 * nrow] + pk[5 * nrow]) + (pk[6 * nrow] + pk[7 * nrow]))) +
                                                         ((pk[8 * nrow] + pk[9 * nrow]) + (pk[10 * nrow] + pk[11 * nrow])));
                    if (hh == 0) s.z[c32] = v;
                    __builtin_amdgcn_fence(__ATOMIC_RELEASE, "wavefront");
                    __builtin_amdgcn_wave_barrier();
                    double tk[NB / 2], zk[NB / 2];
#pragma unroll
                    for (int u = 0; u < NB / 2; u++) tk[u] = dstage0[(k & 1) * (NB * 34) + c32 * 34 + 16 * hh + u], zk[u] = s.z[16 * hh + u];
                    double p4[4] = {0, 0, 0, 0};
#pragma unroll
                    for (int u = 0; u < NB / 2; u++) p4[u & 3] += (16 * hh + u >= c32) ? tk[u] * zk[u] : 0.0;
                    const double p = (p4[0] + p4[1]) + (p4[2] + p4[3]);
                    const unsigned long long pb_ = (unsigned long long)__double_as_longlong(p);
                    const auto lo_ = __builtin_amdgcn_permlane32_swap((unsigned)pb_, (unsigned)pb_, false, false);
                    const auto hi_ = __builtin_amdgcn_permlane32_swap((unsigned)(pb_ >> 32), (unsigned)(pb_ >> 32), false, false);
                    const double p_up = __longlong_as_double((long long)(((unsigned long long)hi_[1] << 32) | lo_[1]));
                    if (hh == 0) xs[k * NB + c32] = p + p_up;
                    BWI_STAMP(1)
                } else {
                    const double2* src = (const double2*)(Lf + se_blk(k, jb0, band)) + lane;
#pragma unroll
                    for (int i = 0; i < TW; i++)
                        if (tw + 3 * i < nt) {
#pragma unroll
                            for (int u = 0; u < NB / 4; u++) ch_ld2_issue(lt[i][u], src + (size_t)(tw + 3 * i) * (NB * NB / 2) + 64 * u);
                        }
                    if (k > 0)
                        stage_diag(k - 1);
                    else
                        ch_ld2_wait();
                }
                BWI_STAMP(2)
                __syncthreads();
                BWI_STAMP(3)
                if (w > 0) {
                    double xv[NB / 4];
#pragma unroll
                    for (int u = 0; u < NB / 4; u++) xv[u] = xs[k * NB + 4 * u + g4];
                    double* const pslot = pend + (4 * tw + g4) * nrow + jb0 * NB + 2 * cp;
#pragma unroll
                    for (int i = 0; i < TW; i++)
                        if (tw + 3 * i < nt) {
                            double a0 = 0, a1 = 0;
#pragma unroll
                            for (int u = 0; u < NB / 4; u++) a0 += lt[i][u].x * xv[u], a1 += lt[i][u].y * xv[u];
                            __hip_atomic_fetch_add(pslot + (tw + 3 * i) * NB, a0, __ATOMIC_RELAXED, __HIP_MEMORY_SCOPE_WORKGROUP);
                            __hip_atomic_fetch_add(pslot + (tw + 3 * i) * NB + 1, a1, __ATOMIC_RELAXED, __HIP_MEMORY_SCOPE_WORKGROUP);
                        }
                }
                __syncthreads();
            }
            __syncthreads();
            for (int i = tid; i < nrow; i += TPB) d.da[i] = xs[i];
            for (int c2 = tid; c2 < d.C; c2 += TPB) {
                const int f = d.cam_free[c2];
                const double* T = d.pose[cur] + 12 * c2;
                double* Tn = d.pose[cur ^ 1] + 12 * c2;
                double Tl[12], o[12];
#pragma unroll
                for (int i = 0; i < 12; i++) Tl[i] = T[i];
                if (f < 0) {
#pragma unroll
                    for (int i = 0; i < 12; i++) Tn[i] = Tl[i];
                } else {
                    double mu[6];
#pragma unroll
                    for (int i = 0; i < 6; i++) mu[i] = xs[6 * f + i];
                    se3_exp_mul(mu, Tl, o);
#pragma unroll
                    for (int i = 0; i < 12; i++) Tn[i] = o[i];
                }
            }
#ifdef K7_TIMING
            if (tid == 0) d.dbg[1398] = (long long)__builtin_readcyclecounter();
#endif
            if (tid < 64) {
                double sq = 0;
                for (int i = tid; i < min(nrow, d.n); i += 64) sq += xs[i] * xs[i];
                sq = wave_sum_f64(sq);
                if (tid == 0) {
                    d.sumsq2[0] = sq;
                    d.sumsq2[1] = 0.0;
                    if (ch_flag(err) != 0) {
                        d.sc->solve_fault = 1;
                        __hip_atomic_store(err, 0u, __ATOMIC_RELAXED, __HIP_MEMORY_SCOPE_AGENT);
                    }
                }
            }
        }
        return;
    }
    const int r = k0 + role + 1;
    if (r >= kr) return;
    const int j0 = max(k0, r - band), nt = r - j0 + 1;
    double* const tiles = ch_lds + (sizeof(ChainLds) + 7) / 8;
    for (int t = 0; t < nt; t++) {
        const size_t o = se_blk(r, j0 + t, band);
        double v4[NB * NB / TPB];
#pragma unroll
        for (int u = 0; u < NB * NB / TPB; u++) v4[u] = S[o + tid + u * TPB];
#pragma unroll
        for (int u = 0; u < NB * NB / TPB; u++) {
            const int e = tid + u * TPB;
            tiles[t * CH_TS + (e / NB) * LDP + e % NB] = v4[u];
        }
    }
    __syncthreads();
    bool one_xcd = false, stored_direct = false;
    const int m_last = min(r - 2, k1 - 1);
    for (int m = j0; m <= m_last; m++) {
        unsigned fv = 0;
        if (lane == 0) fv = ch_wait(F + m, seq, err, d.spin_limit);
        one_xcd = (__builtin_amdgcn_readfirstlane(fv) & 1u) != 0;
        if (tid == 0 && m == r - 2) { CH_RT(4 * m + 1) }
        if (tid == 0 && r == k1 - 1) { CH_RT(100 + 4 * m) }
        const size_t o_mm = se_blk(m, m, band), o_rm = se_blk(r, m, band);
        double lm[NB / 4], ln[NB * NB / TPB];
#pragma unroll
        for (int kk = 0; kk < NB / 4; kk++) lm[kk] = ch_ld(Lf + o_mm + (4 * kk + m4) * NB + colq);
        const double dgc = ch_ld(a.Dg + m * NB + colq);
        {
            const double* Lj = Lf + se_blk(m + 1, m, band) + tid;
#pragma unroll
            for (int i = 0; i < NB * NB / TPB; i++) ln[i] = ch_ld(Lj + TPB * i);
        }
        const double* tA = tiles + (m - j0) * CH_TS + (16 * qi + i16) * LDP + m4;
        double a8[NB / 4];
#pragma unroll
        for (int kk = 0; kk < NB / 4; kk++) a8[kk] = tA[4 * kk];
        v4f64 x = {0, 0, 0, 0};
#pragma unroll
        for (int kk = 0; kk < NB / 4; kk++) x = __builtin_amdgcn_mfma_f64_16x16x4f64(a8[kk], lm[kk], x, 0, 0, 0);
        const double idc = fast_rcp(dgc);
#pragma unroll
        for (int v = 0; v < 4; v++) {
            const int e = (16 * qi + m4 + 4 * v);
            const double l = x[v] * idc;
            ch_st(Lf + o_rm + e * NB + colq, l, one_xcd);
            s.T1[e * LDP + colq] = x[v];
            s.T2[e * LDP + colq] = l;
        }
#pragma unroll
        for (int i = 0; i < NB * NB / TPB; i++) {
            const int e = tid + TPB * i;
            s.T3[(e / NB) * LDP + e % NB] = ln[i];
        }
        const bool last_pivot = m == m_last;
        if (!last_pivot) asm volatile("s_waitcnt vmcnt(0)" ::: "memory");
        __syncthreads();
        if (tid == 0 && !last_pivot) ch_raise(XF(r, m), seq, one_xcd);
        if (tid == 0 && r == k1 - 1) { CH_RT(100 + 4 * m + 1) }
        const bool to_S = last_pivot && m == r - 2;
        auto update = [&](int j, const double (&bt)[NB / 4]) {
            const v4f64 upd = mma_t(s.T1, bt);
            double* tj = tiles + (j - j0) * CH_TS + (16 * qi + m4) * LDP + colq;
            double* gj = S + se_blk(r, j, band) + (16 * qi + m4) * NB + colq;
#pragma unroll
            for (int v = 0; v < 4; v++) {
                const double nv = tj[4 * v * LDP] - upd[v];
                tj[4 * v * LDP] = nv;
                if (to_S) ch_st(gj + 4 * v * NB, nv, one_xcd);
            }
        };
        stored_direct = to_S;
        {
            double bt1[NB / 4];
#pragma unroll
            for (int kk = 0; kk < NB / 4; kk++) bt1[kk] = s.T3[(16 * qj + i16) * LDP + 4 * kk + m4];
            update(m + 1, bt1);
        }
        {
            double btr[NB / 4];
#pragma unroll
            for (int kk = 0; kk < NB / 4; kk++) btr[kk] = s.T2[(16 * qj + i16) * LDP + 4 * kk + m4];
            update(r, btr);
        }
        if (tid == 0 && r == k1 - 1) { CH_RT(100 + 4 * m + 2) }
        {
            const int jw = m + 2 + lane;
            ch_wait_lanes(XF(min(jw, nblk - 1), m), jw < r, seq, err, d.spin_limit);
        }
        {
            constexpr int RT = 3;
            double* const stage[RT] = {s.T0, s.T3, s.T4};
            auto issue = [&](int jb, double (&pr)[RT][NB * NB / TPB]) {
#pragma unroll
                for (int u = 0; u < RT; u++)
                    if (jb + u < r) {
                        const double* src = Lf + se_blk(jb + u, m, band) + tid;
#pragma unroll
                        for (int i = 0; i < NB * NB / TPB; i++) pr[u][i] = ch_ld(src + TPB * i);
                    }
            };
            auto round = [&](int jb, const double (&cur)[RT][NB * NB / TPB], double (&nxt)[RT][NB * NB / TPB]) {
                if (jb + RT < r) issue(jb + RT, nxt);
#pragma unroll
                for (int u = 0; u < RT; u++)
                    if (jb + u < r) {
#pragma unroll
                        for (int i = 0; i < NB * NB / TPB; i++) {
                            const int e = tid + TPB * i;
                            stage[u][(e / NB) * LDP + e % NB] = cur[u][i];
                        }
                    }
                __syncthreads();
#pragma unroll
                for (int u = 0; u < RT; u++)
                    if (jb + u < r) {
                        double bt[NB / 4];
#pragma unroll
                        for (int kk = 0; kk < NB / 4; kk++) bt[kk] = stage[u][(16 * qj + i16) * LDP + 4 * kk + m4];
                        update(jb + u, bt);
                    }
                __syncthreads();
            };
            double pa[RT][NB * NB / TPB], pb[RT][NB * NB / TPB];
            if (m + 2 < r) {
                issue(m + 2, pa);
                __syncthreads();
            }
            for (int jb = m + 2; jb < r; jb += 2 * RT) {
                round(jb, pa, pb);
                if (jb + RT < r) round(jb + RT, pb, pa);
            }
        }
        __syncthreads();
        if (tid == 0 && r == k1 - 1) { CH_RT(100 + 4 * m + 3) }
    }
    {
        const int jf = max(j0, min(r - 1, k1));
        if (m_last < j0) one_xcd = false;
        for (int j = jf; j <= r && !stored_direct; j++) {
            const size_t o = se_blk(r, j, band);
            const double* tj = tiles + (j - j0) * CH_TS;
#pragma unroll
            for (int e = tid; e < NB * NB; e += TPB) ch_st(S + o + e, tj[(e / NB) * LDP + e % NB], one_xcd);
        }
        asm volatile("s_waitcnt vmcnt(0)" ::: "memory");
        __syncthreads();
        if (tid == 0) {
            if (m_last >= j0) ch_raise(XF(r, m_last), seq, one_xcd);
            ch_raise(RF + r, seq, one_xcd);
            CH_RT(4 * (r - 2) + 2)
        }
    }
}

__global__ void __launch_bounds__(TPB) ldlt_mirror_in_kernel(BaDev d, int kr) {
    const int band = se_band(d), nblk = d.npad / NB;
    const int bi = blockIdx.x / (band + 1), jo = blockIdx.x % (band + 1), bj = bi - band + jo;
    if (bi >= kr || bj < 0) return;
    const double* __restrict__ src = d.SE + se_blk(nblk - 1 - bj, nblk - 1 - bi, band);
    double* __restrict__ dst = d.SE2 + se_blk(bi, bj, band);
    double v[NB * NB / TPB];
#pragma unroll
    for (int i = 0; i < NB * NB / TPB; i++) v[i] = src[threadIdx.x + TPB * i];
#pragma unroll
    for (int i = 0; i < NB * NB / TPB; i++) {
        const int e = threadIdx.x + TPB * i;
        const int a = e / NB, b = e % NB;
        dst[(NB - 1 - b) * NB + (NB - 1 - a)] = v[i];
    }
    if (bi == bj && threadIdx.x < NB)
        d.SE2[se_size(nblk, band) + bi * NB + threadIdx.x] = se_E(d)[(nblk - 1 - bi) * NB + NB - 1 - threadIdx.x];
}
__global__ void __launch_bounds__(TPB) ldlt_mirror_out_kernel(BaDev d, int k1, int kr) {
    const int band = se_band(d), nblk = d.npad / NB;
    const int bi = blockIdx.x / (band + 1), jo = blockIdx.x % (band + 1), bj = bi - band + jo;
    if (bi >= kr || bj < 0) return;
    const int pi = nblk - 1 - bi, pj = nblk - 1 - bj;
    const int tid = threadIdx.x;
    if (bj < k1) {
        const double* __restrict__ src = d.L2 + se_blk(bi, bj, band);
        double v[NB * NB / TPB];
#pragma unroll
        for (int i = 0; i < NB * NB / TPB; i++) v[i] = src[tid + TPB * i];
        if (bi == bj) {
            double* __restrict__ dst = d.L + se_blk(pi, pi, band);
#pragma unroll
            for (int i = 0; i < NB * NB / TPB; i++) dst[tid + TPB * i] = v[i];
            if (tid < NB) {
                d.Dg[pi * NB + tid] = d.Dg2[bi * NB + tid];
                d.y[pi * NB + tid] = d.y2[bi * NB + tid];
            }
        } else {
            double* __restrict__ dst = d.L + se_blk(pj, pi, band);
#pragma unroll
            for (int i = 0; i < NB * NB / TPB; i++) {
                const int e = tid + TPB * i;
                const int r = e / NB, q = e % NB;
                dst[q * NB + (NB - 1 - r)] = v[i];
            }
        }
    } else {
        const double* __restrict__ src = d.SE2 + se_blk(bi, bj, band);
        double* __restrict__ dst = d.SE + se_blk(pj, pi, band);
        double v[NB * NB / TPB];
#pragma unroll
        for (int i = 0; i < NB * NB / TPB; i++) v[i] = src[tid + TPB * i];
#pragma unroll
        for (int i = 0; i < NB * NB / TPB; i++) {
            const int e = tid + TPB * i;
            const int r = e / NB, c = e % NB;
            dst[(NB - 1 - c) * NB + (NB - 1 - r)] = v[i];
        }
        if (bi == bj && tid < NB) se_E(d)[pi * NB + NB - 1 - tid] = d.SE2[se_size(nblk, band) + bi * NB + tid];
    }
}
```

### ptam_cg_amd/csrc/solve.hip

```cpp
#include "bundle.h"

#define NB SOLVE_NB
#define LDP (NB + 1)
#define STRIPS 8
#define CPT (NB / STRIPS)
#define TPB (NB * STRIPS)
#define NITER (NB / 4)
#define BW_LDS_MAX ((size_t)150 * 1024)
static_assert(NB == 32, "the strip decomposition below is written for 32x32 blocks");

__device__ __forceinline__ double fast_rcp(double d) {
    const double y = __builtin_amdgcn_rcp(d);
    const double e = fma(-d, y, 1.0);
    return fma(y, fma(e, e, e), y);
}

struct Micro {
    double l10, l20, l21, l30, l31, l32;
    double i0, i1, i2, i3;
    double d0, d1, d2, d3, u10, u20, u30, u21, u31, u32;
};
__device__ __forceinline__ Micro micro_factor(double m00, double m10, double m11, double m20, double m21, double m22,
                                              double m30, double m31, double m32, double m33) {
    Micro f;
    f.d0 = m00;
    f.u10 = m10;
    f.u20 = m20;
    f.u30 = m30;
    f.i0 = fast_rcp(m00);
    f.l10 = m10 * f.i0;
    f.l20 = m20 * f.i0;
    f.l30 = m30 * f.i0;
    f.d1 = m11 - f.l10 * m10;
    f.i1 = fast_rcp(f.d1);
    f.u21 = m21 - f.l20 * m10;
    f.u31 = m31 - f.l30 * m10;
    f.l21 = f.u21 * f.i1;
    f.l31 = f.u31 * f.i1;
    f.d2 = m22 - f.l20 * m20 - f.l21 * f.u21;
    f.i2 = fast_rcp(f.d2);
    f.u32 = m32 - f.l30 * m20 - f.l31 * f.u21;
    f.l32 = f.u32 * f.i2;
    f.d3 = m33 - f.l30 * m30 - f.l31 * f.u31 - f.l32 * f.u32;
    f.i3 = fast_rcp(f.d3);
    return f;
}
__device__ __forceinline__ void micro_subst(const Micro& f, const double a[4], double x[4]) {
    x[0] = a[0];
    x[1] = a[1] - x[0] * f.l10;
    x[2] = a[2] - x[0] * f.l20 - x[1] * f.l21;
    x[3] = a[3] - x[0] * f.l30 - x[1] * f.l31 - x[2] * f.l32;
}

typedef double v4f64 __attribute__((ext_vector_type(4)));
struct StepLds {
    double P[2][3][NB][4];
    double Pb[2][4];
    double Xi[NB * LDP];
    double Xj[NB * LDP];
    double iD[NB], Dv[NB], z[NB];
};

__global__ void __launch_bounds__(TPB) ldlt_step_kernel(BaDev d, int k, int row_limit) {
    if (k == 0) { TL_MARK(d, 9) }
    __shared__ StepLds s;
    constexpr bool mir = false;
    const int wg = blockIdx.x;
    const int rem = min(row_limit - k - 1, se_band(d));
#include "ldlt_step_body.inc"
}

__global__ void __launch_bounds__(TPB) ldlt_step_twin_kernel(BaDev d, int k_top, int k_bot, int nwg_top) {
    if (k_top == 0) { TL_MARK(d, 9) }
    __shared__ StepLds s;
    if ((int)blockIdx.x >= nwg_top) {
        constexpr bool mir = true;
        const int k = k_bot, wg = (int)blockIdx.x - nwg_top;
        const int rem = min(k, se_band(d));
#include "ldlt_step_body.inc"
    } else {
        constexpr bool mir = false;
        const int k = k_top, wg = blockIdx.x;
        const int rem = min(d.npad / NB - k - 1, se_band(d));
#include "ldlt_step_body.inc"
    }
}

#include "ldlt_small.inc"
#include "ldlt_chain.inc"

template <bool BIG>
__global__ void __launch_bounds__(1024) ldlt_backward_kernel(BaDev d, int cur, int b_start) {
    TL_MARK(d, 10)
    const int chain = blockIdx.x;
    extern __shared__ __attribute__((aligned(16))) double bw_lds[];
    const int npad = d.npad, nblk = npad / NB, band = se_band(d);
    double* xs = BIG ? d.bw_scratch + (size_t)chain * 6 * npad : bw_lds;
    double* pend = xs + npad;
    double* wv = pend + 4 * npad;
    const int tid = threadIdx.x;
    const int c = tid % NB, rr = tid / NB;
    if (tid == 0 && chain == 0 && d.sflags && d.sflags[0] != 0) {
        d.sc->solve_fault = 1;
        d.sflags[0] = 0;
    }
    for (int i = tid; i < npad; i += 1024) {
        pend[i] = pend[npad + i] = pend[2 * npad + i] = pend[3 * npad + i] = 0.0;
        wv[i] = d.y[i] / d.Dg[i];
    }
    const int t_end = nblk - b_start;
    const int k_stop = chain == 0 ? 0 : t_end;
    double wnext = d.L[se_blk(b_start - 1, b_start - 1, band) + rr * NB + c];
#ifdef K7_TIMING
#define BW_STAMP(i) if (tid == 0 && chain == 0) d.dbg[1000 + 8 * k + (i)] = (long long)__builtin_readcyclecounter();
#else
#define BW_STAMP(i)
#endif
    const int ucol = tid & (NB - 1), sl0 = (tid >> 5) & 3, ut0 = tid >> 7;
    auto fetch_l = [&](int k, double (&l)[8]) {
        const int jb0 = max(0, k - band);
        const double* src = d.L + se_blk(k, jb0, band) + (size_t)ut0 * (NB * NB) + (sl0 * 8) * NB + ucol;
        const bool on = ut0 < k - jb0;
#pragma unroll
        for (int q = 0; q < 8; q++) l[q] = on ? src[q * NB] : 0.0;
    };
    for (int k = b_start - 1; k >= k_stop; k--) {
        const double w = wnext;
        if (k > k_stop) wnext = d.L[se_blk(k - 1, k - 1, band) + rr * NB + c];
        double lreg[8];
        fetch_l(k, lreg);
        const int jb0 = max(0, k - band), nbk = k - jb0, jlo = jb0 * NB;
        const double* Lrow = d.L + se_blk(k, jb0, band);
        const bool upd = ut0 < nbk;
        const int j0 = jlo + ut0 * NB + ucol;
        BW_STAMP(0)
        __syncthreads();
        BW_STAMP(1)
        const int kc = k * NB + c;
        double p = (c >= rr) ? w * (wv[kc] - ((pend[kc] + pend[npad + kc]) + (pend[2 * npad + kc] + pend[3 * npad + kc]))) : 0.0;
        p += dpp_row_shr_f64<1>(p);
        p += dpp_row_shr_f64<2>(p);
        p += dpp_row_shr_f64<4>(p);
        p += dpp_row_shr_f64<8>(p);
        p += dpp_bcast_f64<0x142, 0xA>(p);
        if (c == NB - 1) xs[k * NB + rr] = p;
        BW_STAMP(2)
        __syncthreads();
        BW_STAMP(3)
        if (upd) {
            double a = 0;
#pragma unroll
            for (int q = 0; q < 8; q++) a += lreg[q] * xs[k * NB + sl0 * 8 + q];
            pend[sl0 * npad + j0] += a;
        }
        for (int ut = ut0 + 8; ut < nbk; ut += 8) {
            double a = 0;
#pragma unroll
            for (int q = 0; q < 8; q++) a += Lrow[(size_t)ut * (NB * NB) + (sl0 * 8 + q) * NB + ucol] * xs[k * NB + sl0 * 8 + q];
            pend[sl0 * npad + jlo + ut * NB + ucol] += a;
        }
        BW_STAMP(4)
    }
    __syncthreads();
    for (int k = b_start; k < nblk && chain == 1; k++) {
        const int jb = max(0, k - band), nj = k - jb;
        const double w = d.L[se_blk(k, k, band) + rr * NB + c];
        const double* Lrow = d.L + se_blk(k, jb, band) + rr * NB + c;
        double a = 0;
        for (int j = 0; j < nj; j++) a += Lrow[(size_t)j * (NB * NB)] * xs[(jb + j) * NB + c];
        a += dpp_row_shr_f64<1>(a);
        a += dpp_row_shr_f64<2>(a);
        a += dpp_row_shr_f64<4>(a);
        a += dpp_row_shr_f64<8>(a);
        a += dpp_bcast_f64<0x142, 0xA>(a);
        if (c == NB - 1) pend[k * NB + rr] = a;
        __syncthreads();
        const int kc = k * NB + c;
        double p = (c >= rr) ? w * (wv[kc] - pend[kc]) : 0.0;
        p += dpp_row_shr_f64<1>(p);
        p += dpp_row_shr_f64<2>(p);
        p += dpp_row_shr_f64<4>(p);
        p += dpp_row_shr_f64<8>(p);
        p += dpp_bcast_f64<0x142, 0xA>(p);
        if (c == NB - 1) xs[k * NB + (NB - 1 - rr)] = p;
        __syncthreads();
    }
    const bool two = t_end > 0;
    const int r_lo = chain == 0 ? 0 : b_start * NB, r_hi = (two && chain == 0) ? b_start * NB : npad;
    for (int i = r_lo + tid; i < r_hi; i += 1024) d.da[i] = xs[i];
    for (int c2 = tid; c2 < d.C; c2 += 1024) {
        const int f = d.cam_free[c2];
        const bool mine = (two && f >= 0 && 6 * f + 5 >= b_start * NB) ? chain == 1 : chain == 0;
        if (!mine) continue;
        const double* T = d.pose[cur] + 12 * c2;
        double* Tn = d.pose[cur ^ 1] + 12 * c2;
        double Tl[12], o[12];
#pragma unroll
        for (int i = 0; i < 12; i++) Tl[i] = T[i];
        if (f < 0) {
#pragma unroll
            for (int i = 0; i < 12; i++) Tn[i] = Tl[i];
        } else {
            double mu[6];
#pragma unroll
            for (int i = 0; i < 6; i++) mu[i] = xs[6 * f + i];
            se3_exp_mul(mu, Tl, o);
#pragma unroll
            for (int i = 0; i < 12; i++) Tn[i] = o[i];
        }
    }
    if (tid < 64) {
        double sq = 0;
        for (int i = r_lo + tid; i < min(r_hi, d.n); i += 64) sq += xs[i] * xs[i];
        sq = wave_sum_f64(sq);
        if (tid == 0) {
            d.sumsq2[chain] = sq;
            if (!two) d.sumsq2[1] = 0.0;
        }
    }
}

int ba_solve_init() {
    HIP_TRY(hipFuncSetAttribute((const void*)ldlt_backward_kernel<false>, hipFuncAttributeMaxDynamicSharedMemorySize, 160 * 1024));
    HIP_TRY(hipFuncSetAttribute((const void*)ldlt_small_kernel, hipFuncAttributeMaxDynamicSharedMemorySize, 160 * 1024));
    HIP_TRY(hipFuncSetAttribute((const void*)ldlt_chain_kernel, hipFuncAttributeMaxDynamicSharedMemorySize, 160 * 1024));
    return PTAM_OK;
}

static int ldlt_twist_len(int nblk, int band) {
    static const bool off = ptam_ab_env("PTAM_LDLT_ONE_ENDED") != nullptr;
    if (off || band < 1 || nblk < 2 * band + 8) return 0;
    return (nblk - 2 * band) / 2;
}

size_t ba_solve_flag_bytes(int nblk) { return ch_flag_words(nblk, nblk) * sizeof(unsigned); }

static ChainArgs chain_args_natural(const BaDev& d, int k0, int k1, int kr) {
    return ChainArgs{d.SE, se_E(d), d.L, d.Dg, d.y, d.sflags, k0, k1, kr, d.n};
}

int ba_solve(ptam_ctx* ctx, BaDev& d, int cur) {
    const int nblk = d.npad / NB, band = se_band(d);
    static const bool no_small = ptam_ab_env("PTAM_LDLT_NO_SMALL") != nullptr;
    if (!no_small && nblk <= SM_USE_NB) {
        hipLaunchKernelGGL(ldlt_small_kernel, dim3(1), dim3(TPB), sizeof(SmallLds), ctx->stream, d, cur);
        HIP_TRY(hipGetLastError());
        return PTAM_OK;
    }
    auto nwg_of = [](int rem) { return 1 + rem + rem * (rem + 1) / 2; };
    const int t_end = ldlt_twist_len(nblk, band), b_start = nblk - t_end;
    {
        static const bool no_chain = getenv("PTAM_LDLT_NO_CHAIN") != nullptr;
        static const bool sep_bw = getenv("PTAM_LDLT_SEPARATE_BACKWARD") != nullptr;
        const bool bw_in = !sep_bw && band <= CH_BW_MAXT && ch_lds_bytes_bw(band, nblk) <= CH_LDS_MAX;
        const size_t lds = bw_in ? ch_lds_bytes_bw(band, nblk) : ch_lds_bytes(band);
        if (t_end == 0 && !no_chain && !d.chain_off && d.sflags && nblk <= CH_MAX_NB && lds <= CH_LDS_MAX) {
            d.solve_seq++;
            if (d.solve_seq >= (1u << 27)) d.solve_seq = 1;
            {
                const ChainArgs a = chain_args_natural(d, 0, nblk, nblk);
                hipLaunchKernelGGL(ldlt_chain_kernel, dim3(8 * ch_roles(nblk)), dim3(TPB), lds, ctx->stream, d, a, a, 1, cur, bw_in ? 1 : 0);
            }
            if (!bw_in) {
                const size_t bw = (size_t)6 * d.npad * sizeof(double);
                hipLaunchKernelGGL(ldlt_backward_kernel<false>, dim3(1), dim3(1024), bw, ctx->stream, d, cur, nblk);
            }
            HIP_TRY(hipGetLastError());
            return PTAM_OK;
        }
    }
    static const bool no_chain2 = getenv("PTAM_LDLT_NO_CHAIN") != nullptr || ptam_ab_env("PTAM_LDLT_TWIN_LAUNCHES") != nullptr;
    const int kr2 = std::min(b_start, t_end + band);
    const bool two_persistent = t_end >= 2 && !no_chain2 && !d.chain_off && d.sflags && d.SE2 && kr2 <= CH_MAX_NB && ch_lds_bytes(band) <= CH_LDS_MAX;
    if (two_persistent) {
        d.solve_seq++;
        if (d.solve_seq >= (1u << 27)) d.solve_seq = 1;
        hipLaunchKernelGGL(ldlt_mirror_in_kernel, dim3(kr2 * (band + 1)), dim3(TPB), 0, ctx->stream, d, kr2);
        const ChainArgs a0 = chain_args_natural(d, 0, t_end, kr2);
        const ChainArgs a1{d.SE2, d.SE2 + se_size(nblk, band), d.L2, d.Dg2, d.y2, d.sflags2, 0, t_end, kr2, d.npad};
        hipLaunchKernelGGL(ldlt_chain_kernel, dim3(8 * ch_roles(kr2)), dim3(TPB), ch_lds_bytes(band), ctx->stream, d, a0, a1, 2, cur, 0);
        hipLaunchKernelGGL(ldlt_mirror_out_kernel, dim3(kr2 * (band + 1)), dim3(TPB), 0, ctx->stream, d, t_end, kr2);
    }
    for (int st = 0; st < (two_persistent ? 0 : t_end); st++) {
        const int kt = st, kb = nblk - 1 - st;
        const int nt = nwg_of(std::min(nblk - kt - 1, band)), nb = nwg_of(std::min(kb, band));
        hipLaunchKernelGGL(ldlt_step_twin_kernel, dim3(nt + nb), dim3(TPB), 0, ctx->stream, d, kt, kb, nt);
    }
    {
        static const bool no_chain = getenv("PTAM_LDLT_NO_CHAIN") != nullptr;
        const int n_mid = b_start - t_end;
        const size_t lds = ch_lds_bytes(band);
        if (t_end > 0 && !no_chain && !d.chain_off && d.sflags && n_mid >= 3 && n_mid <= CH_MAX_NB && lds <= CH_LDS_MAX) {
            d.solve_seq++;
            if (d.solve_seq >= (1u << 27)) d.solve_seq = 1;
            {
                const ChainArgs a = chain_args_natural(d, t_end, b_start, b_start);
                hipLaunchKernelGGL(ldlt_chain_kernel, dim3(8 * ch_roles(n_mid)), dim3(TPB), lds, ctx->stream, d, a, a, 1, cur, 0);
            }
        } else {
            for (int k = t_end; k < b_start; k++) {
                const int nwg = nwg_of(std::min(b_start - k - 1, band));
                hipLaunchKernelGGL(ldlt_step_kernel, dim3(nwg), dim3(TPB), 0, ctx->stream, d, k, b_start);
            }
        }
    }
    const size_t bw_bytes = (size_t)6 * d.npad * sizeof(double);
    if (bw_bytes > BW_LDS_MAX)
        hipLaunchKernelGGL(ldlt_backward_kernel<true>, dim3(t_end > 0 ? 2 : 1), dim3(1024), 0, ctx->stream, d, cur, b_start);
    else
        hipLaunchKernelGGL(ldlt_backward_kernel<false>, dim3(t_end > 0 ? 2 : 1), dim3(1024), bw_bytes, ctx->stream, d, cur, b_start);
    HIP_TRY(hipGetLastError());
    return PTAM_OK;
}

void solve_preload_kernels() {
    ptam_preload((const void*)ldlt_step_kernel);
    ptam_preload((const void*)ldlt_step_twin_kernel);
    ptam_preload((const void*)ldlt_backward_kernel<false>);
    ptam_preload((const void*)ldlt_backward_kernel<true>);
    ptam_preload((const void*)ldlt_small_kernel);
    ptam_preload((const void*)ldlt_chain_kernel);
    ptam_preload((const void*)ldlt_mirror_in_kernel);
    ptam_preload((const void*)ldlt_mirror_out_kernel);
}
```

Before: 6373.

## Fuse Schur partial reduction into the persistent LDLT chain kernel with per-row flags

The separate schur_reduce_kernel launch is folded into the persistent LDLT chain kernel. Extra reducer workgroups sum the Schur partial tiles and write them with agent-scope atomic stores, then publish per-block-row readiness flags. The factor, forward and backward roles wait on those flags, so factorisation of early rows can start while later rows are still being reduced, and one kernel launch disappears. The cost is extra flag words, spin-waiting, and a dependence on co-residency of the reducer and chain workgroups. It applies only to the single-chain, unsharded path.

```diff
diff --git a/__graft_entry__.py b/__graft_entry__.py
--- a/__graft_entry__.py
+++ b/__graft_entry__.py
@@ -12,6 +12,7 @@
     env.setdefault("PATH", "")
     env["PATH"] = "/opt/rocm/bin:" + env["PATH"]
     subprocess.check_call(["make", "-C", os.path.join(ROOT, "ptam_cg_amd", "csrc"), "-j4"], env=env)
+    subprocess.check_call(["make", "-C", os.path.join(ROOT, "ptam_cg_amd", "csrc"), "ab"], env=env)
     subprocess.check_call(["make", "-C", os.path.join(ROOT, "oracle")], env=env)
     import ptam_cg_amd
     from ptam_cg_amd import _abi
diff --git a/include/ptam_hip_bench.h b/include/ptam_hip_bench.h
--- a/include/ptam_hip_bench.h
+++ b/include/ptam_hip_bench.h
@@ -52,7 +52,8 @@
     PTAM_BL_S_PAIR_BEGIN = 14,
     PTAM_BL_S_WG_HEAD = 15,
     PTAM_BL_CAM_PTR = 16,
-    PTAM_BL_CAM_MEAS = 17
+    PTAM_BL_CAM_MEAS = 17,
+    PTAM_BL_SE_COPY = 18
 };
 int ptam_ba_debug_lists(ptam_ba* ba, int which, void* out, size_t cap_bytes);
 
diff --git a/ptam_cg_amd/csrc/ba_debug_host.inc b/ptam_cg_amd/csrc/ba_debug_host.inc
--- a/ptam_cg_amd/csrc/ba_debug_host.inc
+++ b/ptam_cg_amd/csrc/ba_debug_host.inc
@@ -44,6 +44,16 @@
         if (c[3] > c[1])
             std::printf("K7 INSIDE Compute() (its last launch, block 100): %lld shader cycles in %.2f us = %.2f GHz\n", c[2] - c[0], (c[3] - c[1]) * 0.01,
                         (double)(c[2] - c[0]) / ((c[3] - c[1]) * 10.0));
+    }
+    {
+        long long r[2 + 28];
+        HIP_TRY(hipMemcpy(r, d.dbg + 7950, sizeof r, hipMemcpyDeviceToHost));
+        const int nblk = std::min(28, d.npad / SOLVE_NB);
+        if (r[1] > 0 && r[2] > 0) {
+            std::printf("REDUCER role (us from the chain's entry): chain waited for row 0 until %.2f | rows published at", (r[1] - r[0]) * 0.01);
+            for (int i = 0; i < nblk; i++) std::printf(" %.2f", (r[2 + i] - r[0]) * 0.01);
+            std::printf("\n");
+        }
     }
     if (getenv("PTAM_TIMELINE")) {
         std::vector<long long> tl(2 + 2 * TL_MAX);
diff --git a/ptam_cg_amd/csrc/ba_jacobian.inc b/ptam_cg_amd/csrc/ba_jacobian.inc
--- a/ptam_cg_amd/csrc/ba_jacobian.inc
+++ b/ptam_cg_amd/csrc/ba_jacobian.inc
@@ -407,7 +407,6 @@
     }
 }
 
-#define RSPLIT 16
 __device__ __forceinline__ void reduce_partials_body(const BaDev& d, int grid_acc, int bx, int by) {
     __shared__ double comb[4][64];
     __shared__ double werr[4];
diff --git a/ptam_cg_amd/csrc/ba_schur.inc b/ptam_cg_amd/csrc/ba_schur.inc
--- a/ptam_cg_amd/csrc/ba_schur.inc
+++ b/ptam_cg_amd/csrc/ba_schur.inc
@@ -80,7 +80,6 @@
         vinv_body(d, lambda, b - nr);
 }
 
-#define SCHUR_TILE_ELEMS (SCHUR_TC * SCHUR_TC * 36 + SCHUR_TC * 6)
 #ifndef SCHUR_RING
 #define SCHUR_RING 2
 #endif
@@ -536,91 +535,8 @@
 #endif
 }
 
-#define SRED_SLICES 10
-__device__ __forceinline__ double schur_sum_partials(const double* __restrict__ elem, int w0, int w1) {
-#ifdef SRED_NOLOAD
-    return (double)(w1 - w0);
-#endif
-    double s0 = 0, s1 = 0, s2 = 0, s3 = 0;
-    for (int w = w0; w < w1; w += 32) {
-        double q[32];
-#pragma unroll
-        for (int i = 0; i < 32; i++) {
-            const double v = elem[(size_t)min(w + i, w1 - 1) * SCHUR_TILE_ELEMS];
-            q[i] = w + i < w1 ? v : 0.0;
-        }
-#pragma unroll
-        for (int i = 0; i < 32; i += 4) {
-            s0 += q[i];
-            s1 += q[i + 1];
-            s2 += q[i + 2];
-            s3 += q[i + 3];
-        }
-    }
-    return (s0 + s1) + (s2 + s3);
-}
-__global__ void __launch_bounds__(256) schur_reduce_kernel(BaDev d, double lambda, int pad_identity) {
+#include "ba_schur_reduce.inc"
+__global__ void __launch_bounds__(256) schur_reduce_kernel(BaDev d, double lambda, int pad_identity, double* copy) {
     TL_MARK(d, 8)
-    const int pair = blockIdx.x, slice = blockIdx.y;
-    int a = (int)((sqrt(8.0 * pair + 1.0) - 1.0) * 0.5);
-    while ((a + 1) * (a + 2) / 2 <= pair) a++;
-    while (a * (a + 1) / 2 > pair) a--;
-    const int b = pair - a * (a + 1) / 2;
-    const int wg0 = d.s_pair_wg_begin[pair], wg1 = d.s_pair_wg_begin[pair + 1];
-    double* S = d.SE;
-    double* E = se_E(d);
-    const int band = se_band(d);
-    const size_t FS = (size_t)d.F * 27;
-    if (slice < 9) {
-        const int idx = slice * 256 + threadIdx.x;
-        const int jk = idx / 36, rc = idx - jk * 36;
-        const int j = jk >> 3, k = jk & 7, r = rc / 6, c = rc - r * 6;
-        const int fa = a * SCHUR_TC + j, fb = b * SCHUR_TC + k;
-        if (fa >= d.F || fb >= d.F) return;
-        if (a == b && j < k) return;
-        const int Rr = 6 * fa + r, Cc = 6 * fb + c, Rb = Rr / SOLVE_NB, Cb = Cc / SOLVE_NB;
-        if (Cb > Rb || Rb - Cb > band) return;
-        const bool dg = a == b && j == k;
-        const int rr = r >= c ? r : c, cc = r >= c ? c : r;
-        double uq[RSPLIT];
-#pragma unroll
-        for (int sp = 0; sp < RSPLIT; sp++) uq[sp] = dg ? d.Usplit[sp * FS + fa * 27 + rr * (rr + 1) / 2 + cc] : 0.0;
-        const double tsum = schur_sum_partials(d.s_part + idx, wg0, wg1);
-        double val = -tsum;
-        if (dg) {
-            double u = 0;
-#pragma unroll
-            for (int sp = 0; sp < RSPLIT; sp++) u += uq[sp];
-            if (r == c) u *= (1.0 + lambda);
-            val += u;
-        }
-        S[se_blk(Rb, Cb, band) + (size_t)(Rr % SOLVE_NB) * SOLVE_NB + (Cc % SOLVE_NB)] = val;
-        return;
-    }
-    if (a == b && threadIdx.x < SCHUR_TC * 6) {
-        const int idx = threadIdx.x;
-        const int j = idx / 6, r = idx - j * 6;
-        const int fa = a * SCHUR_TC + j;
-        if (fa < d.F) {
-            const double s = schur_sum_partials(d.s_part + SCHUR_TC * SCHUR_TC * 36 + idx, wg0, wg1);
-            double ea = 0;
-#pragma unroll
-            for (int sp = 0; sp < RSPLIT; sp++) ea += d.Usplit[sp * FS + fa * 27 + 21 + r];
-            E[6 * fa + r] = ea - s;
-        }
-    }
-    {
-        const int np = d.npad - d.n, total = np * d.npad;
-        for (int idx = pair * 256 + threadIdx.x; idx < total; idx += 256 * (int)gridDim.x) {
-            const int q = idx / d.npad;
-            const int r = d.n + q, c = idx - q * d.npad;
-            const int Rb = r / SOLVE_NB, Cb = c / SOLVE_NB;
-            if (c <= r && Rb - Cb <= band)
-                S[se_blk(Rb, Cb, band) + (size_t)(r % SOLVE_NB) * SOLVE_NB + (c % SOLVE_NB)] = (r == c && pad_identity) ? 1.0 : 0.0;
-        }
-    }
-    if (pair == 0) {
-        const int np = d.npad - d.n;
-        for (int idx = threadIdx.x; idx < np; idx += 256) E[d.n + idx] = 0.0;
-    }
-}
+    schur_reduce_body<false>(d, lambda, pad_identity, blockIdx.x, blockIdx.y, gridDim.x, copy);
+}
diff --git a/ptam_cg_amd/csrc/ba_schur_reduce.inc b/ptam_cg_amd/csrc/ba_schur_reduce.inc
--- /dev/null
+++ b/ptam_cg_amd/csrc/ba_schur_reduce.inc
@@ -0,0 +1,111 @@
+#define SRED_SLICES 10
+__device__ __forceinline__ double schur_sum_partials(const double* __restrict__ elem, int w0, int w1) {
+#ifdef SRED_NOLOAD
+    return (double)(w1 - w0);
+#endif
+    double s0 = 0, s1 = 0, s2 = 0, s3 = 0;
+    for (int w = w0; w < w1; w += 32) {
+        double q[32];
+#pragma unroll
+        for (int i = 0; i < 32; i++) {
+            const double v = elem[(size_t)min(w + i, w1 - 1) * SCHUR_TILE_ELEMS];
+            q[i] = w + i < w1 ? v : 0.0;
+        }
+#pragma unroll
+        for (int i = 0; i < 32; i += 4) {
+            s0 += q[i];
+            s1 += q[i + 1];
+            s2 += q[i + 2];
+            s3 += q[i + 3];
+        }
+    }
+    return (s0 + s1) + (s2 + s3);
+}
+template <bool WT>
+__device__ __forceinline__ void sred_store(double* base, double* copy, size_t off, double v) {
+    if (WT)
+        __hip_atomic_store((long long*)(base + off), __double_as_longlong(v), __ATOMIC_RELAXED, __HIP_MEMORY_SCOPE_AGENT);
+    else
+        base[off] = v;
+    if (copy) copy[off] = v;
+}
+template <bool WT>
+__device__ __forceinline__ void schur_reduce_body(const BaDev& d, double lambda, int pad_identity, int pair, int slice, int n_pairs, double* copy) {
+    int a = (int)((sqrt(8.0 * pair + 1.0) - 1.0) * 0.5);
+    while ((a + 1) * (a + 2) / 2 <= pair) a++;
+    while (a * (a + 1) / 2 > pair) a--;
+    const int b = pair - a * (a + 1) / 2;
+    const int wg0 = d.s_pair_wg_begin[pair], wg1 = d.s_pair_wg_begin[pair + 1];
+    double* S = d.SE;
+    const int band = se_band(d);
+    const size_t oE = se_size(d.npad / SOLVE_NB, band);
+    const size_t FS = (size_t)d.F * 27;
+    if (slice < 9) {
+        const int idx = slice * 256 + threadIdx.x;
+        const int jk = idx / 36, rc = idx - jk * 36;
+        const int j = jk >> 3, k = jk & 7, r = rc / 6, c = rc - r * 6;
+        const int fa = a * SCHUR_TC + j, fb = b * SCHUR_TC + k;
+        if (fa >= d.F || fb >= d.F) return;
+        if (a == b && j < k) return;
+        const int Rr = 6 * fa + r, Cc = 6 * fb + c, Rb = Rr / SOLVE_NB, Cb = Cc / SOLVE_NB;
+        if (Cb > Rb || Rb - Cb > band) return;
+        const bool dg = a == b && j == k;
+        const int rr = r >= c ? r : c, cc = r >= c ? c : r;
+        double uq[RSPLIT];
+#pragma unroll
+        for (int sp = 0; sp < RSPLIT; sp++) uq[sp] = dg ? d.Usplit[sp * FS + fa * 27 + rr * (rr + 1) / 2 + cc] : 0.0;
+        const double tsum = schur_sum_partials(d.s_part + idx, wg0, wg1);
+        double val = -tsum;
+        if (dg) {
+            double u = 0;
+#pragma unroll
+            for (int sp = 0; sp < RSPLIT; sp++) u += uq[sp];
+            if (r == c) u *= (1.0 + lambda);
+            val += u;
+        }
+        sred_store<WT>(S, copy, se_blk(Rb, Cb, band) + (size_t)(Rr % SOLVE_NB) * SOLVE_NB + (Cc % SOLVE_NB), val);
+        return;
+    }
+    if (a == b && threadIdx.x < SCHUR_TC * 6) {
+        const int idx = threadIdx.x;
+        const int j = idx / 6, r = idx - j * 6;
+        const int fa = a * SCHUR_TC + j;
+        if (fa < d.F) {
+            const double s = schur_sum_partials(d.s_part + SCHUR_TC * SCHUR_TC * 36 + idx, wg0, wg1);
+            double ea = 0;
+#pragma unroll
+            for (int sp = 0; sp < RSPLIT; sp++) ea += d.Usplit[sp * FS + fa * 27 + 21 + r];
+            sred_store<WT>(S, copy, oE + 6 * fa + r, ea - s);
+        }
+    }
+    {
+        const int np = d.npad - d.n, total = np * d.npad;
+        for (int idx = pair * 256 + threadIdx.x; idx < total; idx += 256 * n_pairs) {
+            const int q = idx / d.npad;
+            const int r = d.n + q, c = idx - q * d.npad;
+            const int Rb = r / SOLVE_NB, Cb = c / SOLVE_NB;
+            if (c <= r && Rb - Cb <= band)
+                sred_store<WT>(S, copy, se_blk(Rb, Cb, band) + (size_t)(r % SOLVE_NB) * SOLVE_NB + (c % SOLVE_NB), (r == c && pad_identity) ? 1.0 : 0.0);
+        }
+    }
+    if (pair == 0) {
+        const int np = d.npad - d.n;
+        for (int idx = threadIdx.x; idx < np; idx += 256) sred_store<WT>(S, copy, oE + d.n + idx, 0.0);
+    }
+}
+
+__host__ __device__ __forceinline__ int sred_row_lo(int a) { return a * (SCHUR_TC * 6) / SOLVE_NB; }
+__host__ __device__ __forceinline__ int sred_row_hi(int a, int nblk) {
+    const int hi = (a * (SCHUR_TC * 6) + SCHUR_TC * 6 - 1) / SOLVE_NB;
+    return hi < nblk - 1 ? hi : nblk - 1;
+}
+__host__ __device__ __forceinline__ unsigned sred_row_items(int R, int n_tiles, int nblk) {
+    unsigned n = 0;
+    for (int a = 0; a < n_tiles; a++) {
+        if (sred_row_lo(a) <= R && R <= sred_row_hi(a, nblk))
+            n += (unsigned)(a + 1) * SRED_SLICES;
+        else if (R == nblk - 1)
+            n += (unsigned)(a + 1);
+    }
+    return n;
+}
diff --git a/ptam_cg_amd/csrc/bundle.h b/ptam_cg_amd/csrc/bundle.h
--- a/ptam_cg_amd/csrc/bundle.h
+++ b/ptam_cg_amd/csrc/bundle.h
@@ -7,6 +7,8 @@
 
 #define BA_CHUNK 256
 #define SCHUR_TC 8
+#define SCHUR_TILE_ELEMS (SCHUR_TC * SCHUR_TC * 36 + SCHUR_TC * 6)
+#define RSPLIT 16
 #define SOLVE_NB 32
 #define HIST_BINS 4096
 
@@ -170,7 +172,14 @@
 };
 int ba_dev_result(const ptam_ba* ba, BaDevResult* r);
 
-int ba_solve(ptam_ctx* ctx, BaDev& d, int cur);
+struct SolveReduce {
+    double lambda;
+    int pad_identity;
+    double* copy;
+};
+bool ba_solve_reduces(const BaDev& d, bool sharded);
+bool ba_solve_one_chain(const BaDev& d);
+int ba_solve(ptam_ctx* ctx, BaDev& d, int cur, const SolveReduce* red = nullptr);
 #define CH_SPIN_DEFAULT (1 << 18)
 size_t ba_solve_flag_bytes(int nblk);
 int ba_solve_init();
diff --git a/ptam_cg_amd/csrc/bundle.hip b/ptam_cg_amd/csrc/bundle.hip
--- a/ptam_cg_amd/csrc/bundle.hip
+++ b/ptam_cg_amd/csrc/bundle.hip
@@ -1033,15 +1033,18 @@
     if (d.P > 0 && !skip_vinv) hipLaunchKernelGGL(vinv_kernel, dim3((d.P + 255) / 256), dim3(256), 0, ctx->stream, d, lambda);
     prof_end(ba, PTAM_K_VINV);
     if (d.F > 0) {
+        const bool sharded = ba->comm && ba->world > 1;
+        const bool reduce_in_solve = ba_solve_reduces(d, sharded);
+        const SolveReduce red{lambda, (ba->world > 1 && ba->rank != 0) ? 0 : 1,
+                              ptam_ab_env("PTAM_DEBUG_SE_COPY") && !sharded && ba_solve_one_chain(d) ? d.SE2 : nullptr};
         prof_begin(ba, PTAM_K_SCHUR);
         if (d.n_schur_wg > 0)
             hipLaunchKernelGGL(schur_tile_mfma_kernel, dim3(d.n_schur_wg), dim3(64 * SCHUR_NW), SCHUR_RED_BYTES, ctx->stream, d);
-        hipLaunchKernelGGL(schur_reduce_kernel, dim3(d.n_pairs, SRED_SLICES), dim3(256), 0, ctx->stream, d, lambda,
-                           (ba->world > 1 && ba->rank != 0) ? 0 : 1);
+        if (!reduce_in_solve)
+            hipLaunchKernelGGL(schur_reduce_kernel, dim3(d.n_pairs, SRED_SLICES), dim3(256), 0, ctx->stream, d, red.lambda, red.pad_identity, red.copy);
         prof_end(ba, PTAM_K_SCHUR);
         HIP_TRY(hipGetLastError());
         const size_t n_se = se_size(d.npad / SOLVE_NB, se_band(d)) + d.npad;
-        const bool sharded = ba->comm && ba->world > 1;
         if (sharded) prof_begin(ba, PTAM_K_EXCHANGE);
         int rc = ba_allreduce(ba, d.SE, n_se + (ba->cur_pending ? 2 : 0));
         if (sharded) prof_end(ba, PTAM_K_EXCHANGE);
@@ -1051,7 +1054,7 @@
             ba->cur_pending = false;
         }
         prof_begin(ba, PTAM_K_SOLVE);
-        rc = ba_solve(ctx, d, ba->cur);
+        rc = ba_solve(ctx, d, ba->cur, reduce_in_solve ? &red : nullptr);
         prof_end(ba, PTAM_K_SOLVE);
         if (rc) return rc;
     }
@@ -1778,7 +1781,7 @@
 
 int ptam_ba_debug_lists(ptam_ba* ba, int which, void* out, size_t cap_bytes) {
     ARG_TRY(ba);
-    if (!ba->prepared) {
+    if (!ba->prepared && !(which == PTAM_BL_SE_COPY && ba->block)) {
         ptam_set_error("ptam_ba_debug_lists: the bundle is not prepared");
         return PTAM_E_STATE;
     }
@@ -1816,6 +1819,14 @@
             }
             src = d.cam_meas, bytes = (size_t)n_free_meas * 4;
             break;
+        case PTAM_BL_SE_COPY:
+#ifdef PTAM_AB_SWITCHES
+            src = d.SE2, bytes = (se_size(d.npad / SOLVE_NB, se_band(d)) + (size_t)d.npad) * 8;
+            break;
+#else
+            ptam_set_error("ptam_ba_debug_lists: PTAM_BL_SE_COPY exists in the A/B build only (make ab)");
+            return PTAM_E_STATE;
+#endif
         default: ARG_TRY(!"which"); 
     }
     if (out && bytes > 0) {
diff --git a/ptam_cg_amd/csrc/ldlt_chain.inc b/ptam_cg_amd/csrc/ldlt_chain.inc
--- a/ptam_cg_amd/csrc/ldlt_chain.inc
+++ b/ptam_cg_amd/csrc/ldlt_chain.inc
@@ -65,20 +65,62 @@
     }
 }
 __host__ __device__ __forceinline__ int ch_roles(int nblk) { return nblk > 2 ? nblk : 2; }
-__host__ __device__ __forceinline__ size_t ch_flag_words(int nblk, int band) { return 2 + 3 * (size_t)nblk + (size_t)nblk * (band + 1); }
+__host__ __device__ __forceinline__ size_t ch_flag_words(int nblk, int band) { return 2 + 5 * (size_t)nblk + (size_t)nblk * (band + 1); }
+__host__ __device__ __forceinline__ unsigned* ch_sr_flags(unsigned* flags, int nblk, int band) { return flags + 2 + 3 * (size_t)nblk + (size_t)nblk * (band + 1); }
+
+#define CH_RED_MAX 160
+__host__ __device__ __forceinline__ int ch_reducers(int n_pairs) {
+    const int items = (n_pairs * SRED_SLICES + 7) & ~7;
+    return items < CH_RED_MAX ? items : CH_RED_MAX;
+}
+__device__ __forceinline__ void ch_reduce_role(const BaDev& d, unsigned* flags, int n_red, const SolveReduce& red) {
+    const int nblk = d.npad / NB;
+    unsigned* const SR = ch_sr_flags(flags, nblk, se_band(d));
+    unsigned* const SRC = SR + nblk;
+    const unsigned seq = d.solve_seq;
+    const int items = d.n_pairs * SRED_SLICES;
+    for (int it = blockIdx.x; it < items; it += n_red) {
+        const int pair = it / SRED_SLICES, slice = it - pair * SRED_SLICES;
+        schur_reduce_body<true>(d, red.lambda, red.pad_identity, pair, slice, d.n_pairs, red.copy);
+        asm volatile("s_waitcnt vmcnt(0)" ::: "memory");
+        __syncthreads();
+        if (threadIdx.x == 0) {
+            int a = 0;
+            while ((a + 1) * (a + 2) / 2 <= pair) a++;
+            auto count = [&](int R) {
+                const unsigned had = __hip_atomic_fetch_add(SRC + R, 1u, __ATOMIC_RELAXED, __HIP_MEMORY_SCOPE_AGENT);
+                if (had + 1 == sred_row_items(R, d.n_tiles, nblk)) {
+                    __hip_atomic_store(SRC + R, 0u, __ATOMIC_RELAXED, __HIP_MEMORY_SCOPE_AGENT);
+                    __hip_atomic_store(SR + R, seq << 1, __ATOMIC_RELAXED, __HIP_MEMORY_SCOPE_AGENT);
+#ifdef K7_TIMING
+                    d.dbg[7952 + R] = (long long)__builtin_amdgcn_s_memrealtime();
+#endif
+                }
+            };
+            const int lo = sred_row_lo(a), hi = sred_row_hi(a, nblk);
+            for (int R = lo; R <= hi; R++) count(R);
+            if (slice == SRED_SLICES - 1 && hi < nblk - 1) count(nblk - 1);
+        }
+    }
+}
 
 struct ChainArgs {
     double *S, *E, *L, *Dg, *y;
     unsigned* flags;
     int k0, k1, kr, n;
 };
-__global__ void __launch_bounds__(TPB, 2) ldlt_chain_kernel(BaDev d, ChainArgs a0, ChainArgs a1, int clubs, int cur, int do_bw) {
-    const int club = ((int)(blockIdx.x & 7) - d.chain_xcd) & 7;
+__global__ void __launch_bounds__(TPB, 2) ldlt_chain_kernel(BaDev d, ChainArgs a0, ChainArgs a1, int clubs, int cur, int do_bw, int n_red, SolveReduce red) {
+    TL_MARK(d, 9)
+    if ((int)blockIdx.x < n_red) {
+        ch_reduce_role(d, a0.flags, n_red, red);
+        return;
+    }
+    const int bid = (int)blockIdx.x - n_red;
+    const int club = ((bid & 7) - d.chain_xcd) & 7;
     if (club >= clubs) return;
     const ChainArgs& a = club == 0 ? a0 : a1;
     const int k0 = a.k0, k1 = a.k1, kr = a.kr;
-    const int role = blockIdx.x >> 3;
-    if (role == 0 && club == 0) { TL_MARK(d, 9) }
+    const int role = bid >> 3;
     extern __shared__ __attribute__((aligned(16))) double ch_lds[];
     ChainLds& s = *(ChainLds*)ch_lds;
     const int band = se_band(d), nblk = d.npad / NB;
@@ -91,6 +133,8 @@
     unsigned* const XCC = RF + nblk;
     unsigned* const XFb = XCC + nblk + 1;
     auto XF = [&](int r, int m) { return XFb + (size_t)r * (band + 1) + (m - max(0, r - band)); };
+    const bool red_in = n_red > 0;
+    const unsigned* const SR = ch_sr_flags(a.flags, nblk, band);
     double* __restrict__ S = a.S;
     double* __restrict__ E = a.E;
     double* __restrict__ Lf = a.L;
@@ -124,10 +168,18 @@
     if (role == 0) {
         const double e0 = m4 == 0 ? 1.0 : 0.0, e1 = m4 == 1 ? 1.0 : 0.0, e2 = m4 == 2 ? 1.0 : 0.0, e3 = m4 == 3 ? 1.0 : 0.0;
         v4f64 accK;
+#ifdef K7_TIMING
+        if (tid == 0) d.dbg[7950] = (long long)__builtin_amdgcn_s_memrealtime();
+#endif
+        if (red_in && lane == 0) (void)ch_wait(SR + k0, seq, err, d.spin_limit);
+#ifdef K7_TIMING
+        if (tid == 0) d.dbg[7951] = (long long)__builtin_amdgcn_s_memrealtime();
+#endif
 #pragma unroll
         for (int v = 0; v < 4; v++) {
             const int row = 16 * qi + m4 + 4 * v;
-            accK[v] = S[se_blk(k0, k0, band) + max(row, colq) * NB + min(row, colq)];
+            const double* p = S + se_blk(k0, k0, band) + max(row, colq) * NB + min(row, colq);
+            accK[v] = red_in ? ch_ld(p) : *p;
         }
         bool one_xcd = false;
         for (int k = k0; k < k1; k++) {
@@ -140,6 +192,7 @@
             const int r = k + 1;
             const bool have_row = r < kr;
             const size_t o_rk = have_row ? se_blk(r, k, band) : 0, o_rr = have_row ? se_blk(r, r, band) : 0;
+            const unsigned* const row_flag = r >= k0 + 2 ? RF + r : (red_in ? SR + r : nullptr);
             if (tid < 2) s.staged[tid] = 0;
             int stage_state = have_row ? 0 : 2;
             double stg[2][NB * NB / 64];
@@ -152,7 +205,7 @@
 #endif
 #define FACTOR_IDLE_HOOK(t_)                                                                                         \
     if (FL_STAGE_ON && stage_state < 2) {                                                                            \
-        if (stage_state == 0 && (r < k0 + 2 || (ch_flag(RF + r) >> 1) == seq)) {                                     \
+        if (stage_state == 0 && (row_flag == nullptr || (ch_flag(row_flag) >> 1) == seq)) {                          \
             _Pragma("unroll") for (int u = 0; u < NB * NB / 64; u++) stg[0][u] = ch_ld(S + o_rk + lane + 64 * u);    \
             _Pragma("unroll") for (int u = 0; u < NB * NB / 64; u++) stg[1][u] = ch_ld(S + o_rr + lane + 64 * u);    \
             stage_state = (t_) + 1 < niter ? 1 : 3;                                                                  \
@@ -201,7 +254,7 @@
             double aop[NB / 4];
             v4f64 accN;
             if (!(s.staged[0] && s.staged[1])) {
-                if (r >= k0 + 2 && lane == 0) ch_wait(RF + r, seq, err, d.spin_limit);
+                if (row_flag && lane == 0) ch_wait(row_flag, seq, err, d.spin_limit);
                 double t3[NB * NB / TPB], t4[NB * NB / TPB];
 #pragma unroll
                 for (int u = 0; u < NB * NB / TPB; u++) t3[u] = ch_ld(S + o_rk + tid + u * TPB);
@@ -277,7 +330,8 @@
     if (role == n_roles - 1) {
         double* const bb = ch_lds + (sizeof(ChainLds) + 7) / 8;
         const int b0 = k0 * NB;
-        for (int i = k0 * NB + tid; i < kr * NB; i += TPB) bb[i - b0] = E[i];
+        if (red_in) ch_wait_lanes(SR + min(k0 + lane, kr - 1), k0 + lane < kr, seq, err, d.spin_limit);
+        for (int i = k0 * NB + tid; i < kr * NB; i += TPB) bb[i - b0] = red_in ? ch_ld(E + i) : E[i];
         __syncthreads();
         const int q = tid & (NB - 1), part = tid >> 5;
         const int row = tid >> 3, g = tid & 7;
@@ -469,11 +523,12 @@
     if (r >= kr) return;
     const int j0 = max(k0, r - band), nt = r - j0 + 1;
     double* const tiles = ch_lds + (sizeof(ChainLds) + 7) / 8;
+    if (red_in && lane == 0) (void)ch_wait(SR + r, seq, err, d.spin_limit);
     for (int t = 0; t < nt; t++) {
         const size_t o = se_blk(r, j0 + t, band);
         double v4[NB * NB / TPB];
 #pragma unroll
-        for (int u = 0; u < NB * NB / TPB; u++) v4[u] = S[o + tid + u * TPB];
+        for (int u = 0; u < NB * NB / TPB; u++) v4[u] = red_in ? ch_ld(S + o + tid + u * TPB) : S[o + tid + u * TPB];
 #pragma unroll
         for (int u = 0; u < NB * NB / TPB; u++) {
             const int e = tid + u * TPB;
diff --git a/ptam_cg_amd/csrc/solve.hip b/ptam_cg_amd/csrc/solve.hip
--- a/ptam_cg_amd/csrc/solve.hip
+++ b/ptam_cg_amd/csrc/solve.hip
@@ -87,6 +87,7 @@
 }
 
 #include "ldlt_small.inc"
+#include "ba_schur_reduce.inc"
 #include "ldlt_chain.inc"
 
 template <bool BIG>
@@ -239,8 +240,28 @@
     return ChainArgs{d.SE, se_E(d), d.L, d.Dg, d.y, d.sflags, k0, k1, kr, d.n};
 }
 
-int ba_solve(ptam_ctx* ctx, BaDev& d, int cur) {
+static bool ch_backward_inside(int nblk, int band) {
+    static const bool sep_bw = getenv("PTAM_LDLT_SEPARATE_BACKWARD") != nullptr;
+    return !sep_bw && band <= CH_BW_MAXT && ch_lds_bytes_bw(band, nblk) <= CH_LDS_MAX;
+}
+bool ba_solve_one_chain(const BaDev& d) {
     const int nblk = d.npad / NB, band = se_band(d);
+    static const bool no_small = ptam_ab_env("PTAM_LDLT_NO_SMALL") != nullptr;
+    static const bool no_chain = getenv("PTAM_LDLT_NO_CHAIN") != nullptr;
+    if (!no_small && nblk <= SM_USE_NB) return false;
+    const size_t lds = ch_backward_inside(nblk, band) ? ch_lds_bytes_bw(band, nblk) : ch_lds_bytes(band);
+    return ldlt_twist_len(nblk, band) == 0 && !no_chain && !d.chain_off && d.sflags && nblk <= CH_MAX_NB && lds <= CH_LDS_MAX;
+}
+bool ba_solve_reduces(const BaDev& d, bool sharded) {
+    return !sharded && d.F > 0 && !ptam_ab_env("PTAM_SEPARATE_REDUCE") && ba_solve_one_chain(d);
+}
+
+int ba_solve(ptam_ctx* ctx, BaDev& d, int cur, const SolveReduce* red) {
+    const int nblk = d.npad / NB, band = se_band(d);
+    if (red && !ba_solve_one_chain(d)) {
+        ptam_set_error("ba_solve: asked to reduce the Schur partial tiles in a form that cannot");
+        return PTAM_E_STATE;
+    }
     static const bool no_small = ptam_ab_env("PTAM_LDLT_NO_SMALL") != nullptr;
     if (!no_small && nblk <= SM_USE_NB) {
         hipLaunchKernelGGL(ldlt_small_kernel, dim3(1), dim3(TPB), sizeof(SmallLds), ctx->stream, d, cur);
@@ -250,16 +271,16 @@
     auto nwg_of = [](int rem) { return 1 + rem + rem * (rem + 1) / 2; };
     const int t_end = ldlt_twist_len(nblk, band), b_start = nblk - t_end;
     {
-        static const bool no_chain = getenv("PTAM_LDLT_NO_CHAIN") != nullptr;
-        static const bool sep_bw = getenv("PTAM_LDLT_SEPARATE_BACKWARD") != nullptr;
-        const bool bw_in = !sep_bw && band <= CH_BW_MAXT && ch_lds_bytes_bw(band, nblk) <= CH_LDS_MAX;
+        const bool bw_in = ch_backward_inside(nblk, band);
         const size_t lds = bw_in ? ch_lds_bytes_bw(band, nblk) : ch_lds_bytes(band);
-        if (t_end == 0 && !no_chain && !d.chain_off && d.sflags && nblk <= CH_MAX_NB && lds <= CH_LDS_MAX) {
+        if (ba_solve_one_chain(d)) {
             d.solve_seq++;
             if (d.solve_seq >= (1u << 27)) d.solve_seq = 1;
             {
                 const ChainArgs a = chain_args_natural(d, 0, nblk, nblk);
-                hipLaunchKernelGGL(ldlt_chain_kernel, dim3(8 * ch_roles(nblk)), dim3(TPB), lds, ctx->stream, d, a, a, 1, cur, bw_in ? 1 : 0);
+                const int n_red = red ? ch_reducers(d.n_pairs) : 0;
+                hipLaunchKernelGGL(ldlt_chain_kernel, dim3(n_red + 8 * ch_roles(nblk)), dim3(TPB), lds, ctx->stream, d, a, a, 1, cur, bw_in ? 1 : 0, n_red,
+                                   red ? *red : SolveReduce{});
             }
             if (!bw_in) {
                 const size_t bw = (size_t)6 * d.npad * sizeof(double);
@@ -278,7 +299,7 @@
         hipLaunchKernelGGL(ldlt_mirror_in_kernel, dim3(kr2 * (band + 1)), dim3(TPB), 0, ctx->stream, d, kr2);
         const ChainArgs a0 = chain_args_natural(d, 0, t_end, kr2);
         const ChainArgs a1{d.SE2, d.SE2 + se_size(nblk, band), d.L2, d.Dg2, d.y2, d.sflags2, 0, t_end, kr2, d.npad};
-        hipLaunchKernelGGL(ldlt_chain_kernel, dim3(8 * ch_roles(kr2)), dim3(TPB), ch_lds_bytes(band), ctx->stream, d, a0, a1, 2, cur, 0);
+        hipLaunchKernelGGL(ldlt_chain_kernel, dim3(8 * ch_roles(kr2)), dim3(TPB), ch_lds_bytes(band), ctx->stream, d, a0, a1, 2, cur, 0, 0, SolveReduce{});
         hipLaunchKernelGGL(ldlt_mirror_out_kernel, dim3(kr2 * (band + 1)), dim3(TPB), 0, ctx->stream, d, t_end, kr2);
     }
     for (int st = 0; st < (two_persistent ? 0 : t_end); st++) {
@@ -295,7 +316,7 @@
             if (d.solve_seq >= (1u << 27)) d.solve_seq = 1;
             {
                 const ChainArgs a = chain_args_natural(d, t_end, b_start, b_start);
-                hipLaunchKernelGGL(ldlt_chain_kernel, dim3(8 * ch_roles(n_mid)), dim3(TPB), lds, ctx->stream, d, a, a, 1, cur, 0);
+                hipLaunchKernelGGL(ldlt_chain_kernel, dim3(8 * ch_roles(n_mid)), dim3(TPB), lds, ctx->stream, d, a, a, 1, cur, 0, 0, SolveReduce{});
             }
         } else {
             for (int k = t_end; k < b_start; k++) {
```

After: 5895. 7.5% lower.
